# robertknight/ocrs

Hardware: AMD Instinct MI355X
Metric: pages/sec end-to-end (1024x1024) (higher is better)
Workload: dtype f32

## Files before the change

include/ocrs_amd.h:

```cpp
#ifndef OCRS_AMD_H
#define OCRS_AMD_H

#include <stddef.h>
#include <stdint.h>

#if defined(__GNUC__)
#define OCRS_API __attribute__((visibility("default")))
#else
#define OCRS_API
#endif

#ifdef __cplusplus
extern "C" {
#endif

typedef enum ocrs_status {
    OCRS_OK = 0,
    OCRS_ERR_INVALID_ARGUMENT = 1,
    OCRS_ERR_MODEL_NOT_LOADED = 2,
    OCRS_ERR_MODEL_DIMS = 3,
    OCRS_ERR_RUN_FAILED = 4,
    OCRS_ERR_WRONG_OUTPUT = 5,
    OCRS_ERR_IMAGE_SOURCE = 6,
    OCRS_ERR_DEVICE = 7,
    OCRS_ERR_IO = 8,
    OCRS_ERR_CAPACITY = 9
} ocrs_status;

OCRS_API const char* ocrs_last_error(void);

#define OCRS_ABI_VERSION 6u
OCRS_API uint32_t ocrs_abi_version(void);

OCRS_API void ocrs_buffer_free(void* p);

OCRS_API ocrs_status ocrs_device_count(int* n);
OCRS_API ocrs_status ocrs_set_device(int device);
OCRS_API ocrs_status ocrs_get_device(int* device);

OCRS_API ocrs_status ocrs_ctc_beam_search(const float* logp, int t, int c, uint32_t width, int impl, uint32_t** labels,
                                          uint32_t** positions, size_t* n);
OCRS_API ocrs_status ocrs_ctc_beam_search_scored(const float* logp, int t, int c, uint32_t width, int impl, uint32_t** labels,
                                                 uint32_t** positions, size_t* n, double* score, float** step_logp);

OCRS_API ocrs_status ocrs_gru_tile_plan(const int32_t* lengths_desc, size_t n_lines, int hidden, int32_t* n_clusters, int32_t* waves,
                                        int16_t* tiles);

OCRS_API ocrs_status ocrs_coalescer_selftest(int n_threads, int requests_per_thread, int max_active, int max_pages,
                                             long window_us, int fail_every, uint64_t out[5]);

OCRS_API ocrs_status ocrs_stream_plan_selftest(int budget, const int32_t* ops, size_t n_ops, int32_t* out);

OCRS_API ocrs_status ocrs_set_option(const char* name, long value);
OCRS_API ocrs_status ocrs_option_name(int index, const char** name);

OCRS_API ocrs_status ocrs_device_pool_stats(int device, uint64_t out[12]);
OCRS_API ocrs_status ocrs_device_pool_configure(int device, uint64_t device_cached_cap_bytes, uint64_t pinned_cached_cap_bytes);
OCRS_API ocrs_status ocrs_device_pool_trim(int device);

typedef enum { OCRS_ISOLATION_AUTO = 0, OCRS_ISOLATION_NONE = 1 } ocrs_isolation;
OCRS_API ocrs_status ocrs_device_set_isolation(int device, ocrs_isolation policy);
OCRS_API ocrs_status ocrs_device_isolation(int device, int out[3]);

typedef struct ocrs_model ocrs_model;

OCRS_API ocrs_status ocrs_model_load_file(const char* path, ocrs_model** out);
OCRS_API ocrs_status ocrs_model_load_bytes(const void* data, size_t len, ocrs_model** out);
OCRS_API ocrs_status ocrs_model_load_file_on_device(const char* path, int device, ocrs_model** out);
OCRS_API ocrs_status ocrs_model_load_bytes_on_device(const void* data, size_t len, int device, ocrs_model** out);
OCRS_API ocrs_status ocrs_model_device(const ocrs_model* m, int* device);

typedef int (*ocrs_model_run_fn)(void* user, const float* input, const int64_t in_shape[4], float** output,
                                 int64_t out_shape[4], int* out_ndim);
OCRS_API ocrs_status ocrs_model_from_callback(const int64_t input_shape[4],
                                     ocrs_model_run_fn run, void* user, ocrs_model** out);

OCRS_API ocrs_status ocrs_model_input_shape(const ocrs_model* m, int64_t dims[4], uint8_t is_fixed[4]);

typedef struct ocrs_run_options {
    int timing;
} ocrs_run_options;

OCRS_API ocrs_status ocrs_model_run(const ocrs_model* m, const float* input, const int64_t in_shape[4],
                           const ocrs_run_options* opts, float** output, int64_t out_shape[4], int* out_ndim);

OCRS_API ocrs_status ocrs_model_flops(const ocrs_model* m, const int64_t in_shape[4], double* flops);

OCRS_API void ocrs_model_free(ocrs_model* m);

typedef struct ocrs_engine ocrs_engine;
typedef struct ocrs_page ocrs_page;

typedef enum ocrs_numerics { OCRS_NUMERICS_EXACT = 0, OCRS_NUMERICS_RELAXED = 1, OCRS_NUMERICS_REDUCED = 2 } ocrs_numerics;

typedef enum ocrs_decode_method {
    OCRS_DECODE_GREEDY = 0,
    OCRS_DECODE_BEAM_SEARCH = 1
} ocrs_decode_method;

typedef struct ocrs_engine_params {
    const ocrs_model* detection_model;
    const ocrs_model* recognition_model;
    int debug;
    ocrs_decode_method decode_method;
    uint32_t beam_width;
    const char* alphabet;
    const char* allowed_chars;
    ocrs_numerics numerics;
    int coalesce;
    int coalesce_pages;
    int coalesce_window_us;
    int layout_threads;
    int64_t rec_max_pixels;
} ocrs_engine_params;

OCRS_API ocrs_status ocrs_engine_new(const ocrs_engine_params* params, ocrs_engine** out);
OCRS_API void ocrs_engine_free(ocrs_engine* e);
OCRS_API ocrs_status ocrs_engine_device(const ocrs_engine* e, int* device);
OCRS_API ocrs_status ocrs_engine_set_option(ocrs_engine* e, const char* name, long value);
OCRS_API ocrs_status ocrs_engine_get_option(const ocrs_engine* e, const char* name, long* value);

typedef enum ocrs_dim_order { OCRS_HWC = 0, OCRS_CHW = 1 } ocrs_dim_order;
typedef enum ocrs_pixel_type { OCRS_U8 = 0, OCRS_F32 = 1 } ocrs_pixel_type;

OCRS_API ocrs_status ocrs_image_source_check_bytes(size_t len, uint32_t width, uint32_t height, uint32_t* channels);

OCRS_API ocrs_status ocrs_engine_prepare_input(const ocrs_engine* e, const void* pixels, ocrs_pixel_type type,
                                      ocrs_dim_order order, int height, int width, int channels,
                                      ocrs_page** out);
OCRS_API ocrs_status ocrs_engine_prepare_input_batch(const ocrs_engine* e, const void* const* pixels, size_t n,
                                                     ocrs_pixel_type type, ocrs_dim_order order, int height, int width,
                                                     int channels, ocrs_page** out);
OCRS_API ocrs_status ocrs_engine_prepare_input_device(const ocrs_engine* e, const void* d_pixels, ocrs_pixel_type type,
                                             ocrs_dim_order order, int height, int width, int channels,
                                             ocrs_page** out);
OCRS_API void ocrs_page_free(ocrs_page* p);
OCRS_API ocrs_status ocrs_page_dims(const ocrs_page* p, int* height, int* width);
OCRS_API ocrs_status ocrs_page_image(const ocrs_page* p, float* out_hw);
OCRS_API ocrs_status ocrs_engine_page_from_grey(const ocrs_engine* e, const float* grey_hw, int height, int width, ocrs_page** out);

OCRS_API ocrs_status ocrs_engine_detect_words(const ocrs_engine* e, const ocrs_page* page, float** rects, size_t* n);
OCRS_API ocrs_status ocrs_engine_detect_words_batch(const ocrs_engine* e, const ocrs_page* const* pages, size_t n_pages,
                                           float** rects, size_t* offsets);

OCRS_API ocrs_status ocrs_engine_detect_words_scored(const ocrs_engine* e, const ocrs_page* page, float** rects, size_t* n,
                                                     float** score, uint32_t** pixels);
OCRS_API ocrs_status ocrs_engine_detect_words_batch_scored(const ocrs_engine* e, const ocrs_page* const* pages, size_t n_pages,
                                                           float** rects, size_t* offsets, float** score, uint32_t** pixels);

OCRS_API ocrs_status ocrs_engine_detect_text_pixels(const ocrs_engine* e, const ocrs_page* page, float* out_hw);

#define OCRS_TILE_OVERLAP_DEFAULT 100
OCRS_API ocrs_status ocrs_detection_tile_plan(int page_h, int page_w, int model_h, int model_w, int overlap, size_t* ny, size_t* nx,
                                              int32_t** origin_y, int32_t** bound_y, int32_t** origin_x, int32_t** bound_x);
OCRS_API ocrs_status ocrs_engine_detect_words_tiled(const ocrs_engine* e, const ocrs_page* page, int overlap, float** rects, size_t* n,
                                                    float** score, uint32_t** pixels);
OCRS_API ocrs_status ocrs_engine_detect_words_batch_tiled(const ocrs_engine* e, const ocrs_page* const* pages, size_t n_pages, int overlap,
                                                          float** rects, size_t* offsets, float** score, uint32_t** pixels);
OCRS_API ocrs_status ocrs_engine_detect_text_pixels_tiled(const ocrs_engine* e, const ocrs_page* page, int overlap, float* out_hw);

typedef enum ocrs_resample_filter { OCRS_RESAMPLE_AUTO = 0, OCRS_RESAMPLE_BILINEAR = 1, OCRS_RESAMPLE_AREA = 2 } ocrs_resample_filter;
OCRS_API ocrs_status ocrs_engine_resize_page(const ocrs_engine* e, const ocrs_page* page, int out_h, int out_w, int filter, ocrs_page** out);
OCRS_API ocrs_status ocrs_engine_resize_pages(const ocrs_engine* e, const ocrs_page* const* pages, size_t n, const int* out_hw,
                                              const int* filters, ocrs_page** out);
OCRS_API ocrs_status ocrs_work_size(int page_h, int page_w, double scale, int* h, int* w);
OCRS_API ocrs_status ocrs_rescale_rects(float* rects6, size_t n, int from_h, int from_w, int to_h, int to_w);
OCRS_API ocrs_status ocrs_engine_detect_words_at(const ocrs_engine* e, const ocrs_page* page, int work_h, int work_w, int filter, int tiled,
                                                 int overlap, float** rects, size_t* n, float** score, uint32_t** pixels);
OCRS_API ocrs_status ocrs_engine_detect_words_batch_at(const ocrs_engine* e, const ocrs_page* const* pages, size_t n_pages,
                                                       const int* work_hw, int filter, int tiled, int overlap, float** rects,
                                                       size_t* offsets, float** score, uint32_t** pixels);

typedef enum ocrs_polarity { OCRS_POLARITY_AUTO = 0, OCRS_POLARITY_KEEP = 1, OCRS_POLARITY_INVERT = 2 } ocrs_polarity;
typedef struct ocrs_normalize_params {
    int32_t tile;
    int32_t polarity;
    int32_t flatten;
    int32_t levels;
} ocrs_normalize_params;
typedef struct ocrs_normalize_info {
    int32_t dark;
    int32_t white;
    int32_t lo, hi;
    int64_t vote;
    uint64_t counted;
} ocrs_normalize_info;
OCRS_API ocrs_status ocrs_normalize_params_default(ocrs_normalize_params* out);
OCRS_API ocrs_status ocrs_normalize_params_check(const ocrs_normalize_params* params);
OCRS_API ocrs_status ocrs_engine_normalize_page(const ocrs_engine* e, const ocrs_page* page, const ocrs_normalize_params* params,
                                                ocrs_page** out_page, ocrs_normalize_info* out_info);
OCRS_API ocrs_status ocrs_engine_normalize_pages(const ocrs_engine* e, const ocrs_page* const* pages, size_t n,
                                                 const ocrs_normalize_params* params, ocrs_page** out_pages, ocrs_normalize_info* out_info);

typedef struct ocrs_skew_params {
    double max_deg;
    double coarse_step_deg;
    double fine_step_deg;
    int32_t work_max_side;
    int32_t reserved;
} ocrs_skew_params;
typedef struct ocrs_skew_info {
    double angle_deg;
    uint64_t best_score;
    uint64_t second_score;
// ... 235 lines not shown
```

ocrs_amd/_lib.py:

```python
import ctypes as C
import os

_HERE = os.path.dirname(os.path.abspath(__file__))
LIB_PATH = os.environ.get("OCRS_AMD_LIB") or os.path.join(_HERE, "libocrs_amd.so")

OCRS_OK = 0
STATUS_NAMES = {
    0: "OK", 1: "INVALID_ARGUMENT", 2: "MODEL_NOT_LOADED", 3: "MODEL_DIMS", 4: "RUN_FAILED", 5: "WRONG_OUTPUT",
    6: "IMAGE_SOURCE", 7: "DEVICE", 8: "IO", 9: "CAPACITY",
}

RUN_FN = C.CFUNCTYPE(C.c_int, C.c_void_p, C.POINTER(C.c_float), C.POINTER(C.c_int64), C.POINTER(C.POINTER(C.c_float)),
                     C.POINTER(C.c_int64), C.POINTER(C.c_int))


class EngineParams(C.Structure):
    _fields_ = [("detection_model", C.c_void_p), ("recognition_model", C.c_void_p), ("debug", C.c_int),
                ("decode_method", C.c_int), ("beam_width", C.c_uint32), ("alphabet", C.c_char_p),
                ("allowed_chars", C.c_char_p), ("numerics", C.c_int), ("coalesce", C.c_int), ("coalesce_pages", C.c_int),
                ("coalesce_window_us", C.c_int), ("layout_threads", C.c_int), ("rec_max_pixels", C.c_int64)]


class GroupParams(C.Structure):
    _fields_ = [("detection_model", C.c_void_p), ("detection_model_len", C.c_size_t), ("recognition_model", C.c_void_p),
                ("recognition_model_len", C.c_size_t), ("devices", C.POINTER(C.c_int)), ("n_devices", C.c_size_t),
                ("debug", C.c_int), ("decode_method", C.c_int), ("beam_width", C.c_uint32), ("alphabet", C.c_char_p),
                ("allowed_chars", C.c_char_p), ("gather", C.c_int), ("numerics", C.c_int), ("coalesce", C.c_int),
                ("coalesce_pages", C.c_int), ("coalesce_window_us", C.c_int), ("layout_threads", C.c_int), ("rec_max_pixels", C.c_int64),
                ("min_block", C.c_int), ("shared_block", C.c_int)]


class RunOptions(C.Structure):
    _fields_ = [("timing", C.c_int)]


class TextCharC(C.Structure):
    _fields_ = [("ch", C.c_uint32), ("top", C.c_int32), ("left", C.c_int32), ("bottom", C.c_int32),
                ("right", C.c_int32)]


class OcrsError(RuntimeError):
    def __init__(self, status, message):
        super().__init__(message)
        self.status = status
        self.status_name = STATUS_NAMES.get(status, str(status))


DECLARED_SYMBOLS = [
    "ocrs_last_error", "ocrs_buffer_free", "ocrs_device_count", "ocrs_set_device", "ocrs_set_option", "ocrs_ctc_beam_search", "ocrs_model_load_file",
    "ocrs_model_load_bytes", "ocrs_model_from_callback", "ocrs_model_input_shape", "ocrs_model_run",
    "ocrs_model_flops", "ocrs_model_free", "ocrs_engine_new", "ocrs_engine_free", "ocrs_image_source_check_bytes",
    "ocrs_engine_prepare_input", "ocrs_engine_prepare_input_device", "ocrs_page_free", "ocrs_page_dims",
    "ocrs_page_image", "ocrs_engine_detect_words", "ocrs_engine_detect_words_batch",
    "ocrs_engine_detect_text_pixels", "ocrs_engine_detection_threshold", "ocrs_engine_find_text_lines",
    "ocrs_engine_find_text_lines_batch",
    "ocrs_engine_recognize_text", "ocrs_engine_recognize_text_batch", "ocrs_engine_recognize_tokens",
    "ocrs_engine_prepare_recognition_input", "ocrs_text_item_rotated_rect", "ocrs_rotated_rect_corners", "ocrs_engine_get_text", "ocrs_device_malloc", "ocrs_device_free",
    "ocrs_device_upload", "ocrs_device_synchronize", "ocrs_device_measure_peaks", "ocrs_engine_enable_timing", "ocrs_stage_count",
    "ocrs_stage_name", "ocrs_engine_stage_times", "ocrs_kernel_class_count", "ocrs_kernel_class_name",
    "ocrs_engine_kernel_stats", "ocrs_engine_set_kernel_timing_mask", "ocrs_gru_tile_plan", "ocrs_host_malloc", "ocrs_host_free", "ocrs_engine_prepare_input_batch",
    "ocrs_get_device", "ocrs_model_load_file_on_device", "ocrs_model_load_bytes_on_device", "ocrs_model_device", "ocrs_engine_device",
    "ocrs_engine_group_new", "ocrs_engine_group_free", "ocrs_engine_group_size", "ocrs_engine_group_member", "ocrs_group_deal",
    "ocrs_group_prepare_input_batch", "ocrs_group_prepare_input_device_batch", "ocrs_group_detect_words_batch",
    "ocrs_group_recognize_text_batch", "ocrs_group_gather", "ocrs_group_final_gather", "ocrs_group_worker_threads", "ocrs_group_last_gather", "ocrs_device_malloc_on", "ocrs_engine_coalesce_stats", "ocrs_coalescer_selftest", "ocrs_stream_plan_selftest", "ocrs_engine_kernel_mfma_flops", "ocrs_engine_prepare_input_jpeg", "ocrs_jpeg_decode_rgb", "ocrs_jpeg_info", "ocrs_jpeg_coefficients",
    "ocrs_group_member_stats", "ocrs_numa_parse_cpulist", "ocrs_numa_bind_selftest", "ocrs_engine_recognize_logits", "ocrs_engine_set_option", "ocrs_engine_get_option", "ocrs_option_name", "ocrs_device_pool_stats", "ocrs_device_pool_configure", "ocrs_device_pool_trim",
    "ocrs_device_set_isolation", "ocrs_device_isolation", "ocrs_group_set_replay", "ocrs_abi_version",
    "ocrs_engine_recognize_text_scored", "ocrs_engine_recognize_text_batch_scored", "ocrs_ctc_beam_search_scored",
    "ocrs_engine_run_recognition_ops",
    "ocrs_engine_detect_words_scored", "ocrs_engine_detect_words_batch_scored", "ocrs_group_detect_words_batch_scored",
    "ocrs_engine_find_text_lines_indexed", "ocrs_engine_find_text_lines_batch_indexed",
    "ocrs_detection_tile_plan", "ocrs_engine_detect_words_tiled", "ocrs_engine_detect_words_batch_tiled",
    "ocrs_engine_detect_text_pixels_tiled", "ocrs_group_detect_words_batch_tiled",
    "ocrs_line_frame", "ocrs_line_char_boxes", "ocrs_engine_prepare_recognition_input_rectified",
    "ocrs_engine_recognize_text_rectified", "ocrs_engine_recognize_text_batch_rectified",
    "ocrs_group_recognize_text_batch_rectified", "ocrs_engine_recognize_tokens_rectified",
    "ocrs_engine_rotate_page", "ocrs_engine_rotate_pages", "ocrs_unrotate_rects", "ocrs_unrotate_chars",
    "ocrs_orientation_vote", "ocrs_engine_detect_orientation", "ocrs_engine_page_from_grey",
    "ocrs_engine_resize_page", "ocrs_engine_resize_pages", "ocrs_work_size", "ocrs_rescale_rects",
    "ocrs_engine_detect_words_at", "ocrs_engine_detect_words_batch_at",
    "ocrs_normalize_params_default", "ocrs_normalize_params_check", "ocrs_engine_normalize_page", "ocrs_engine_normalize_pages",
    "ocrs_skew_params_default", "ocrs_skew_params_check", "ocrs_skew_table", "ocrs_engine_skew_scores", "ocrs_engine_estimate_skew",
    "ocrs_engine_warp_page", "ocrs_engine_warp_pages", "ocrs_deskew_map", "ocrs_unwarp_rects", "ocrs_unwarp_chars",
    "ocrs_outline_params_default", "ocrs_outline_params_check", "ocrs_engine_edge_peaks", "ocrs_outline_choose", "ocrs_engine_find_outline",
    "ocrs_quad_map", "ocrs_engine_project_page", "ocrs_engine_project_pages", "ocrs_unproject_rects", "ocrs_unproject_chars",
]

ABI_VERSION = 6
TILE_OVERLAP_DEFAULT = 100
RESAMPLE_FILTERS = {"auto": 0, "bilinear": 1, "area": 2}
POLARITIES = {"auto": 0, "keep": 1, "invert": 2}


class NormalizeParams(C.Structure):
    _fields_ = [("tile", C.c_int32), ("polarity", C.c_int32), ("flatten", C.c_int32), ("levels", C.c_int32)]


class NormalizeInfo(C.Structure):
    _fields_ = [("dark", C.c_int32), ("white", C.c_int32), ("lo", C.c_int32), ("hi", C.c_int32), ("vote", C.c_int64),
                ("counted", C.c_uint64)]

    def as_dict(self):
        return {"dark": int(self.dark), "vote": int(self.vote), "white": int(self.white), "lo": int(self.lo), "hi": int(self.hi),
                "counted": int(self.counted)}


class SkewParams(C.Structure):
    _fields_ = [("max_deg", C.c_double), ("coarse_step_deg", C.c_double), ("fine_step_deg", C.c_double), ("work_max_side", C.c_int32),
                ("reserved", C.c_int32)]


class SkewInfo(C.Structure):
    _fields_ = [("angle_deg", C.c_double), ("best_score", C.c_uint64), ("second_score", C.c_uint64), ("fine_score", C.c_uint64),
                ("work_h", C.c_int32), ("work_w", C.c_int32), ("coarse_index", C.c_int32), ("fine_index", C.c_int32)]


class OutlineParams(C.Structure):
    _fields_ = [("max_deg", C.c_double), ("step_deg", C.c_double), ("min_cover", C.c_double), ("min_span", C.c_double), ("min_area", C.c_double),
                ("work_max_side", C.c_int32), ("min_step", C.c_int32)]


class OutlineInfo(C.Structure):
    _fields_ = [("found", C.c_int32), ("polarity", C.c_int32), ("corners", C.c_float * 8), ("counts", C.c_uint32 * 4), ("angles", C.c_int32 * 4),
                ("work_h", C.c_int32), ("work_w", C.c_int32)]


_lib = None


def lib():
    global _lib
    if _lib is None:
        if not os.path.exists(LIB_PATH):
            raise OcrsError(7, "libocrs_amd.so is not built: run `python -m ocrs_amd.build` "
                               "(there is no CPU fallback for the HIP engine)")
        L = C.CDLL(LIB_PATH)
        L.ocrs_abi_version.restype = C.c_uint32
        if L.ocrs_abi_version() != ABI_VERSION:
            raise OcrsError(7, "libocrs_amd.so has ABI version %d, this binding was written for %d: rebuild (python -m ocrs_amd.build)"
                            % (L.ocrs_abi_version(), ABI_VERSION))
        L.ocrs_last_error.restype = C.c_char_p
        L.ocrs_engine_detection_threshold.restype = C.c_float
        L.ocrs_engine_detection_threshold.argtypes = [C.c_void_p]
        L.ocrs_stage_name.restype = C.c_char_p
        L.ocrs_kernel_class_name.restype = C.c_char_p
        L.ocrs_buffer_free.argtypes = [C.c_void_p]
        for name in ("ocrs_model_free", "ocrs_engine_free", "ocrs_page_free", "ocrs_engine_group_free"):
            getattr(L, name).argtypes = [C.c_void_p]
            getattr(L, name).restype = None
        _lib = L
    return _lib


def check(status):
    if status != OCRS_OK:
        msg = lib().ocrs_last_error()
        raise OcrsError(status, msg.decode("utf-8", "replace") if msg else STATUS_NAMES.get(status, "error"))


def device_count():
    n = C.c_int(0)
    check(lib().ocrs_device_count(C.byref(n)))
    return n.value


def measure_peaks():
    a, b = C.c_double(0), C.c_double(0)
    check(lib().ocrs_device_measure_peaks(C.byref(a), C.byref(b)))
    return a.value, b.value


def set_option(name, value):
    check(lib().ocrs_set_option(name.encode(), C.c_long(int(value))))


def option_names():
    out, i = [], 0
    while True:
        n = C.c_char_p()
        check(lib().ocrs_option_name(i, C.byref(n)))
        if not n.value:
            return out
        out.append(n.value.decode())
        i += 1


POOL_FIELDS = ("device_live", "device_cached", "device_cap", "device_peak_live", "device_driver_allocs", "device_driver_frees",
               "pinned_live", "pinned_cached", "pinned_cap", "pinned_peak_live", "pinned_driver_allocs", "pinned_driver_frees")


def pool_stats(device=-1):
    v = (C.c_uint64 * 12)()
    check(lib().ocrs_device_pool_stats(int(device), v))
    return dict(zip(POOL_FIELDS, (int(x) for x in v)))


def pool_trim(device=-1):
    check(lib().ocrs_device_pool_trim(int(device)))


def pool_configure(device=-1, device_cached_cap=0, pinned_cached_cap=0):
    check(lib().ocrs_device_pool_configure(int(device), C.c_uint64(int(device_cached_cap)), C.c_uint64(int(pinned_cached_cap))))


ISOLATION = {"auto": 0, "none": 1}


def set_isolation(policy="auto", device=-1):
    check(lib().ocrs_device_set_isolation(int(device), int(ISOLATION[policy])))


def isolation(device=-1):
    v = (C.c_int * 3)()
    check(lib().ocrs_device_isolation(int(device), v))
    return {"mode": ("free", "serial")[v[0]], "relaxed_engines": int(v[1]), "cus": int(v[2])}


def ctc_beam_search(logp, width, impl=0):
# ... 64 lines not shown
```

ocrs_amd/csrc/abi.cpp:

```cpp
#include <cstdio>
#include <fstream>
#include <thread>

#include <atomic>
#include "abi_util.hpp"
#include "coalesce_selftest.hpp"
#include "engine.hpp"
#include "host_pool.hpp"
#include "jpeg.hpp"
#include "kernels.hpp"
#include "page_ops.hpp"

using namespace ocrs;
using namespace ocrs::geom;

using namespace ocrs::abi;

extern "C" {

const char* ocrs_last_error(void) { return last_error().c_str(); }

void ocrs_buffer_free(void* p) { free(p); }

ocrs_status ocrs_device_count(int* n) {
    return guarded([&] {
        int c = 0;
        hipError_t e = hipGetDeviceCount(&c);
        if (e != hipSuccess) c = 0;
        *n = c;
    });
}

ocrs_status ocrs_set_device(int device) {
    return guarded([&] { select_device(device); });
}

ocrs_status ocrs_get_device(int* device) {
    return guarded([&] {
        if (!device) fail(OCRS_ERR_INVALID_ARGUMENT, "null argument");
        *device = default_device();
    });
}

ocrs_status ocrs_gru_tile_plan(const int32_t* lengths_desc, size_t n_lines, int hidden, int32_t* n_clusters, int32_t* waves,
                               int16_t* tiles) {
    return guarded([&] {
        if (!lengths_desc || !n_clusters || !waves || !tiles || n_lines == 0 || n_lines > (size_t)1 << 20)
            fail(OCRS_ERR_INVALID_ARGUMENT, "bad argument");
        for (size_t i = 0; i < n_lines; i++)
            if (lengths_desc[i] < 1 || (i > 0 && lengths_desc[i] > lengths_desc[i - 1]))
                fail(OCRS_ERR_INVALID_ARGUMENT, "lengths must be positive and descending");
        int ncl = 0;
        if (!k::gru_tile_plan(lengths_desc, (int)n_lines, hidden, &ncl, waves, tiles))
            fail(OCRS_ERR_CAPACITY, "no persistent-kernel plan for this shape (the engine then runs the recurrence as one fused launch per time step)");
        *n_clusters = ncl;
    });
}

ocrs_status ocrs_coalescer_selftest(int n_threads, int requests_per_thread, int max_active, int max_pages, long window_us,
                                    int fail_every, uint64_t out[5]) {
    return guarded([&] {
        if (!out || n_threads < 1 || requests_per_thread < 1 || max_pages < 1) fail(OCRS_ERR_INVALID_ARGUMENT, "bad argument");
        coalescer_selftest(n_threads, requests_per_thread, max_active, max_pages, window_us, fail_every, out);
    });
}

ocrs_status ocrs_stream_plan_selftest(int budget, const int32_t* ops, size_t n_ops, int32_t* out) {
    return guarded([&] {
        if (!out || (n_ops > 0 && !ops) || !LanePlan::valid_budget(budget)) fail(OCRS_ERR_INVALID_ARGUMENT, "bad argument");
        LanePlan plan(budget);
        for (size_t i = 0; i < n_ops; i++) {
            const int32_t op = ops[2 * i], arg = ops[2 * i + 1];
            switch (op) {
                case 0: out[i] = plan.acquire(arg); break;
                case 1: plan.release(arg); out[i] = plan.outstanding(); break;
                case 2: out[i] = plan.set_budget(arg) ? 1 : 0; break;
                case 3: out[i] = plan.load(arg); break;
                case 4: out[i] = plan.budget(); break;
                case 5: out[i] = plan.light_lanes(); break;
                default: fail(OCRS_ERR_INVALID_ARGUMENT, "unknown op %d", (int)op);
            }
        }
    });
}

namespace {

void beam_search_hook(const float* logp, int t, int c, uint32_t width, int impl, std::vector<uint32_t>* l,
                      std::vector<uint32_t>* p, double* score, std::vector<float>* step_logp) {
    if (impl == 2 && t > 0) {
        DeviceScope bind(-1);
        if (!k::ctc_beam_supported(c, (int)width)) fail(OCRS_ERR_CAPACITY, "beam search on the GPU supports up to 128 classes and width 128");
        Workspace ws;
        std::vector<int32_t> meta(1 + t + 1);
        meta[0] = t;
        for (int i = 0; i <= t; i++) meta[1 + i] = i;
        int32_t* d_meta = ws.alloc_n<int32_t>(meta.size());
        float* d_logp = ws.alloc_n<float>((size_t)t * c);
        ws.upload(d_meta, meta.data(), meta.size() * sizeof(int32_t));
        ws.upload(d_logp, logp, (size_t)t * c * sizeof(float));
        const size_t arena = k::ctc_beam_arena_entries(t, (int)width);
        int2* d_nodes = ws.alloc_n<int2>(arena);
        int2* d_posn = ws.alloc_n<int2>(arena);
        uint32_t* d_ol = ws.alloc_n<uint32_t>(t);
        uint32_t* d_op = ws.alloc_n<uint32_t>(t);
        int32_t* d_cnt = ws.alloc_n<int32_t>(1);
        double* d_score = score ? ws.alloc_n<double>(1) : nullptr;
        float* d_slp = score ? ws.alloc_n<float>(t) : nullptr;
        k::ctc_beam_packed(d_logp, d_meta, d_meta + 1, 1, t, c, (int)width, nullptr, d_nodes, d_posn, d_ol, d_op, d_cnt, ws.s(),
                           d_score, d_slp);
        std::vector<uint32_t> hl(t), hp(t);
        std::vector<float> hs(score ? t : 0);
        int32_t cnt = 0;
        ws.download(hl.data(), d_ol, (size_t)t * 4);
        ws.download(hp.data(), d_op, (size_t)t * 4);
        ws.download(&cnt, d_cnt, 4);
        if (score) {
            ws.download(score, d_score, sizeof(double));
            ws.download(hs.data(), d_slp, (size_t)t * sizeof(float));
        }
        ws.sync();
        OCRS_HIP(hipGetLastError());
        l->assign(hl.begin(), hl.begin() + cnt);
        p->assign(hp.begin(), hp.begin() + cnt);
        if (score) step_logp->assign(hs.begin(), hs.begin() + cnt);
    } else {
        double bs = 0.0;
        const std::vector<CtcStep> st = t == 0 ? std::vector<CtcStep>()
                                              : (impl == 1 ? ctc_beam_search_reference(logp, t, c, c, width, &bs)
                                                           : ctc_beam_search(logp, t, c, c, width, &bs));
        l->resize(st.size()); p->resize(st.size());
        for (size_t i = 0; i < st.size(); i++) { (*l)[i] = st[i].label; (*p)[i] = st[i].pos; }
        if (score) score_line(logp, t, c, c, nullptr, st, &bs, step_logp, score);
    }
}

}

ocrs_status ocrs_ctc_beam_search(const float* logp, int t, int c, uint32_t width, int impl, uint32_t** labels,
                                 uint32_t** positions, size_t* n) {
    return guarded([&] {
        if (!logp || !labels || !positions || !n || t < 0 || c < 1) fail(OCRS_ERR_INVALID_ARGUMENT, "bad argument");
        std::vector<uint32_t> l, p;
        beam_search_hook(logp, t, c, width, impl, &l, &p, nullptr, nullptr);
        *labels = dup_buffer(l);
        *positions = dup_buffer(p);
        *n = l.size();
    });
}

ocrs_status ocrs_ctc_beam_search_scored(const float* logp, int t, int c, uint32_t width, int impl, uint32_t** labels,
                                        uint32_t** positions, size_t* n, double* score, float** step_logp) {
    return guarded([&] {
        if (!logp || !labels || !positions || !n || !score || !step_logp || t < 0 || c < 1)
            fail(OCRS_ERR_INVALID_ARGUMENT, "bad argument");
        std::vector<uint32_t> l, p;
        std::vector<float> s;
        double sc = 0.0;
        beam_search_hook(logp, t, c, width, impl, &l, &p, &sc, &s);
        *labels = dup_buffer(l);
        *positions = dup_buffer(p);
        *step_logp = dup_buffer(s);
        *n = l.size();
        *score = sc;
    });
}

uint32_t ocrs_abi_version(void) { return OCRS_ABI_VERSION; }

static void check_option_set(int r, const char* name, long value) {
    if (r == 1) fail(OCRS_ERR_INVALID_ARGUMENT, "unknown option '%s'", name ? name : "(null)");
    if (r == 2) fail(OCRS_ERR_INVALID_ARGUMENT, "option '%s': value %ld is out of range", name, value);
    if (r == 3) fail(OCRS_ERR_INVALID_ARGUMENT, "option '%s' cannot change while a request is in flight on a device", name);
    if (r == 4) fail(OCRS_ERR_INVALID_ARGUMENT, "option '%s' belongs to the devices, not to an engine: set it with ocrs_set_option", name);
}

ocrs_status ocrs_set_option(const char* name, long value) {
    return guarded([&] { check_option_set(set_option(name, value), name, value); });
}

ocrs_status ocrs_engine_set_option(ocrs_engine* e, const char* name, long value) {
    return guarded([&] {
        if (!e) fail(OCRS_ERR_INVALID_ARGUMENT, "null argument");
        check_option_set(set_option(e->tuning, name, value), name, value);
    });
}

ocrs_status ocrs_engine_get_option(const ocrs_engine* e, const char* name, long* value) {
    return guarded([&] {
        if (!e || !value) fail(OCRS_ERR_INVALID_ARGUMENT, "null argument");
        if (!get_option(e->tuning, name, value)) fail(OCRS_ERR_INVALID_ARGUMENT, "unknown option '%s'", name ? name : "(null)");
    });
}

ocrs_status ocrs_option_name(int index, const char** name) {
    return guarded([&] {
        if (!name) fail(OCRS_ERR_INVALID_ARGUMENT, "null argument");
        *name = option_name(index);
    });
}

ocrs_status ocrs_device_pool_stats(int device, uint64_t out[12]) {
    return guarded([&] {
        if (!out) fail(OCRS_ERR_INVALID_ARGUMENT, "null argument");
        DeviceContext& c = device_context(device < 0 ? default_device() : device);
        const PoolStats d = c.pool.stats(), h = c.host_pool.stats();
        const uint64_t v[12] = {d.live, d.cached, d.cap, d.peak_live, d.driver_allocs, d.driver_frees,
                                h.live, h.cached, h.cap, h.peak_live, h.driver_allocs, h.driver_frees};
        for (int i = 0; i < 12; i++) out[i] = v[i];
    });
}

ocrs_status ocrs_device_pool_trim(int device) {
    return guarded([&] {
        DeviceContext& c = device_context(device < 0 ? default_device() : device);
        DeviceScope bind(c.device);
        {
            std::lock_guard<std::mutex> heavy(c.heavy_phase);
            OCRS_HIP(hipStreamSynchronize(c.heavy_stream()));
            c.heavy_arena.clear();
        }
        c.pool.trim();
    });
}

ocrs_status ocrs_device_set_isolation(int device, ocrs_isolation policy) {
    return guarded([&] {
        if (policy != OCRS_ISOLATION_AUTO && policy != OCRS_ISOLATION_NONE) fail(OCRS_ERR_INVALID_ARGUMENT, "unknown isolation policy %d", (int)policy);
        DeviceContext& c = device_context(device < 0 ? default_device() : device);
        DeviceScope bind(c.device);
        c.set_isolation(policy == OCRS_ISOLATION_NONE ? DeviceContext::ISO_NONE : DeviceContext::ISO_AUTO);
    });
}

// ... 878 lines not shown
```

ocrs_amd/csrc/common.cpp:

```cpp
#include "common.hpp"

#include <chrono>
#include <climits>
#include <cstdint>
#include <cstdlib>
#include <cstring>

#include <algorithm>
#include <atomic>
#include <condition_variable>
#include <deque>
#include <system_error>

namespace ocrs {

static thread_local std::string g_last_error;

void set_last_error(const std::string& msg) { g_last_error = msg; }
const std::string& last_error() { return g_last_error; }

namespace {
std::atomic<int> g_default_device{0};
thread_local DeviceContext* t_ctx = nullptr;
constexpr int kMaxDevices = 64;
// ... 323 lines not shown
hipStream_t DeviceContext::recurrent_stream(int mode) {
    if (mode == MODE_SERIAL) return heavy_stream();
    std::lock_guard<std::mutex> g(lazy_mu_);
    create_lanes_locked(planned_light_lanes());
    return recurrent_;
}

hipStream_t DeviceContext::light_lane(int lane) {
    std::lock_guard<std::mutex> g(lazy_mu_);
    create_lanes_locked(std::max(lane + 1, plan.light_lanes()));
    return light_[lane];
}

bool DeviceContext::calls_in_flight() {
    std::lock_guard<std::mutex> lk(iso_mu_);
    return leases_ > 0;
}

static thread_local int t_lease_depth[kMaxDevices] = {0};

template <class F> void DeviceContext::switch_isolation(F&& change) {
    if (t_lease_depth[device] > 0) fail(OCRS_ERR_INVALID_ARGUMENT, "the isolation regime of device %d cannot change from inside one of its requests", device);
    std::unique_lock<std::mutex> lk(iso_mu_);
    iso_cv_.wait(lk, [&] { return !switching_; });
    const Mode before = mode_locked();
    switching_ = true;
    struct Done { DeviceContext* c; ~Done() { c->switching_ = false; c->iso_cv_.notify_all(); } } done{this};
    const Isolation p0 = policy_;
    const int r0 = relaxed_;
    change();
    if (mode_locked() == before) return;
    const Isolation p1 = policy_;
    const int r1 = relaxed_;
    policy_ = p0; relaxed_ = r0;
    iso_cv_.wait(lk, [&] { return leases_ == 0; });
    {
        DeviceScope bind(device);
        if (hipDeviceSynchronize() != hipSuccess) (void)hipGetLastError();
    }
    policy_ = p1; relaxed_ = r1;
}

DeviceContext::Mode DeviceContext::lease_begin() {
    std::unique_lock<std::mutex> lk(iso_mu_);
    if (t_lease_depth[device] == 0) iso_cv_.wait(lk, [&] { return !switching_; });
    t_lease_depth[device]++;
    leases_++;
    return mode_locked();
}

void DeviceContext::lease_end() {
    std::lock_guard<std::mutex> lk(iso_mu_);
    t_lease_depth[device]--;
    if (--leases_ == 0) iso_cv_.notify_all();
}

void DeviceContext::add_relaxed_engine(int delta) {
    switch_isolation([&] { relaxed_ += delta; });
}

void DeviceContext::set_isolation(Isolation policy) {
    switch_isolation([&] { policy_ = policy; });
}

DeviceContext::Mode DeviceContext::current_mode() {
    std::lock_guard<std::mutex> lk(iso_mu_);
    return mode_locked();
}

int DeviceContext::relaxed_engine_count() {
    std::lock_guard<std::mutex> lk(iso_mu_);
    return relaxed_;
}

int DeviceContext::cu_count() {
    std::lock_guard<std::mutex> g(lazy_mu_);
    if (!cus_) {
        hipDeviceProp_t prop;
        OCRS_HIP(hipGetDeviceProperties(&prop, device));
        cus_ = prop.multiProcessorCount;
    }
    return cus_;
}

namespace {
struct OptDef { const char* name; const char* env; long def; };
const OptDef kOptDefs[OPT_COUNT] = {
    {"gru_mode", "OCRS_GRU_MODE", GRU_PERSISTENT},
    {"gru_gates", "OCRS_GRU_GATES", 1},
    {"gru_local", "OCRS_GRU_LOCAL", 1},
    {"det_fuse", "OCRS_DET_FUSE", 1},
    {"det_stream", "OCRS_DET_STREAM", 1},
    {"det_rows", "OCRS_DET_ROWS", 1},
    {"ccl_quad", "OCRS_CCL_QUAD", 1},
    {"conv12_fuse", "OCRS_CONV12_FUSE", 1},
    {"conv_flat", "OCRS_CONV_FLAT", 1},
    {"beam_gpu", "OCRS_BEAM_GPU", 1},
    {"det_tile_batch", "OCRS_DET_TILE_BATCH", 16},
    {"stream_budget", "OCRS_STREAM_BUDGET", LanePlan::kDefaultBudget},
    {"numerics", nullptr, 0},
    {"coalesce", nullptr, 2},
    {"coalesce_pages", nullptr, 16},
    {"coalesce_window_us", nullptr, 300},
    {"layout_threads", nullptr, 0},
    {"rec_max_pixels", nullptr, 0},
};
struct OptRange { long lo, hi; long also[4]; };
const OptRange kOptRanges[OPT_COUNT] = {
    {0, 1, {}}, {0, 1, {}}, {0, 1, {}}, {0, 2, {}}, {0, 1, {8, 14, 32}}, {0, 1, {8, 14, 20, 32}}, {0, 1, {}}, {0, 1, {}}, {0, 1, {}}, {0, 1, {}},
    {1, 1024, {}}, {LanePlan::kMinBudget, LanePlan::kMaxBudget, {}},
    {0, 2, {}}, {0, 64, {}}, {1, 4096, {}}, {0, 10000000, {}}, {0, 4096, {}}, {0, INT64_MAX, {}},
};
bool in_range(int i, long v) {
    const OptRange& r = kOptRanges[i];
    if (i == OPT_STREAM_BUDGET) return LanePlan::valid_budget(v);
    if (v >= r.lo && v <= r.hi) return true;
    for (long a : r.also) if (a && v == a) return true;
    return false;
}
const char* const kRetired[] = {"det_heavy", "det_tail", "gru_waves", "gru_background", "gru_scatter", "gru_gates_pack", "conv_occupancy",
                                "gx_heavy", "gemm_nfast", "conv_a_lds", "gru_heavy", "heavy_priority", "det_mfma"};
std::atomic<long> g_opts[OPT_COUNT];
std::once_flag g_opts_once;
void init_options() {
    for (int i = 0; i < OPT_COUNT; i++) {
        const char* e = kOptDefs[i].env ? getenv(kOptDefs[i].env) : nullptr;
        const long v = e && *e ? strtol(e, nullptr, 10) : kOptDefs[i].def;
        g_opts[i].store(in_range(i, v) ? v : kOptDefs[i].def);
    }
}
int find_option(const char* name, int count = OPT_PUBLIC_COUNT) {
    for (int i = 0; i < count; i++)
        if (name && i != OPT_NUMERICS && strcmp(name, kOptDefs[i].name) == 0) return i;
    return -1;
}
thread_local const Tuning* t_tuning = nullptr;
}

TuningScope::TuningScope(const Tuning* t) : prev_(t_tuning) { t_tuning = t; }
TuningScope::~TuningScope() { t_tuning = prev_; }
const Tuning* current_tuning() { return t_tuning; }

long process_option(Option o) {
    std::call_once(g_opts_once, init_options);
    return g_opts[o].load(std::memory_order_relaxed);
}

long option_long(Option o) {
    if (t_tuning) return __atomic_load_n(&t_tuning->v[o], __ATOMIC_RELAXED);
    std::call_once(g_opts_once, init_options);
    return g_opts[o].load(std::memory_order_relaxed);
}
int option(Option o) { return (int)option_long(o); }

Tuning default_tuning() {
    std::call_once(g_opts_once, init_options);
    Tuning t;
    for (int i = 0; i < OPT_COUNT; i++) t.v[i] = g_opts[i].load(std::memory_order_relaxed);
    return t;
}

const char* option_name(int i) { return i >= 0 && i < OPT_PUBLIC_COUNT ? kOptDefs[i].name : nullptr; }

int set_option(const char* name, long value) {
    std::call_once(g_opts_once, init_options);
    const int i = find_option(name);
    if (i < 0) {
        for (const char* r : kRetired) if (name && strcmp(name, r) == 0) return 0;
        return 1;
    }
    if (!in_range(i, value)) return 2;
    if (i == OPT_STREAM_BUDGET && value != g_opts[i].load() && any_device_has_calls_in_flight()) return 3;
    g_opts[i].store(value);
    return 0;
}

int set_option(Tuning& t, const char* name, long value) {
    const int i = find_option(name, OPT_COUNT);
    if (i < 0) return 1;
    if (i == OPT_STREAM_BUDGET) return 4;
    if (!in_range(i, value)) return 2;
    __atomic_store_n(&t.v[i], value, __ATOMIC_RELAXED);
    return 0;
}

bool get_option(const Tuning& t, const char* name, long* value) {
    const int i = name && strcmp(name, "numerics") == 0 ? (int)OPT_NUMERICS : find_option(name, OPT_COUNT);
    if (i < 0) return false;
    *value = __atomic_load_n(&t.v[i], __ATOMIC_RELAXED);
    return true;
}

static hipEvent_t take_lease_event(DeviceContext* c) {
    {
        std::lock_guard<std::mutex> g(c->stream_mu);
        if (!c->lease_events.empty()) {
            hipEvent_t e = c->lease_events.back();
            c->lease_events.pop_back();
            return e;
        }
    }
    hipEvent_t e = nullptr;
    OCRS_HIP(hipEventCreateWithFlags(&e, hipEventBlockingSync | hipEventDisableTiming));
    return e;
}

StreamLease::StreamLease(bool high_priority, int avoid_lane) : ctx_(&ctx()), high_(high_priority) {
    high_ = true;
    mode_ = ctx_->lease_begin();
    try {
        done_ = take_lease_event(ctx_);
        if (mode_ == DeviceContext::MODE_SERIAL) {
            s_ = ctx_->heavy_stream();
            shared_ = true;
            return;
        }
        (void)ctx_->planned_light_lanes();
        lane_ = ctx_->plan.acquire(avoid_lane);
        counted_ = true;
        if (lane_ >= 0) {
            s_ = ctx_->light_lane(lane_);
            return;
        }
        {
            std::lock_guard<std::mutex> g(ctx_->stream_mu);
            auto& v = ctx_->streams;
            if (!v.empty()) {
                s_ = v.back();
                v.pop_back();
                return;
            }
        }
        int least = 0, greatest = 0;
        OCRS_HIP(hipDeviceGetStreamPriorityRange(&least, &greatest));
        OCRS_HIP(hipStreamCreateWithPriority(&s_, hipStreamNonBlocking, greatest));
    } catch (...) {
        if (counted_) ctx_->plan.release(lane_);
        if (done_) {
            std::lock_guard<std::mutex> g(ctx_->stream_mu);
            ctx_->lease_events.push_back(done_);
        }
        ctx_->lease_end();
        throw;
    }
}

StreamLease::~StreamLease() {
    {
        std::lock_guard<std::mutex> g(ctx_->stream_mu);
        ctx_->lease_events.push_back(done_);
        if (!shared_ && lane_ < 0) ctx_->streams.push_back(s_);
    }
    if (counted_) ctx_->plan.release(lane_);
    ctx_->lease_end();
}

std::vector<StageTimers::Pending>& StageTimers::pending() {
    static thread_local std::vector<Pending> p;
    return p;
}
std::map<int, std::vector<hipEvent_t>>& StageTimers::thread_events() {
    static thread_local std::map<int, std::vector<hipEvent_t>> f;
    return f;
}
std::vector<hipEvent_t>& StageTimers::free_events() { return thread_events()[ctx().device]; }

hipEvent_t StageTimers::get_event() {
    auto& fe = free_events();
    if (!fe.empty()) {
        hipEvent_t e = fe.back();
        fe.pop_back();
        return e;
    }
    hipEvent_t e;
    OCRS_HIP(hipEventCreate(&e));
    return e;
}

int StageTimers::begin(int stage, hipStream_t s, uint64_t n_launches) {
    if (!enabled) return -1;
    Pending p{stage, get_event(), get_event(), n_launches, false, 0.0, 0.0, 0.0};
    OCRS_HIP(hipEventRecord(p.a, s));
    pending().push_back(p);
    return (int)pending().size() - 1;
}

int StageTimers::kbegin(int cls, hipStream_t s, double flops, double bytes, double mfma_flops) {
    if (!enabled || !kernels_enabled || !((kernel_mask >> cls) & 1u)) return -1;
    if (mfma_flops < 0.0) mfma_flops = cls <= KC_GEMM_LINEAR ? flops : 0.0;
    Pending p{cls, get_event(), get_event(), 1, true, flops, bytes, mfma_flops};
    OCRS_HIP(hipEventRecord(p.a, s));
    pending().push_back(p);
    return (int)pending().size() - 1;
}

void StageTimers::end(int token, hipStream_t s) {
    if (token < 0) return;
    auto& pd = pending();
    if ((size_t)token < pd.size()) (void)hipEventRecord(pd[token].b, s);
}

void StageTimers::collect() {
    auto& pd = pending();
    if (pd.empty()) return;
    double lms[ST_COUNT] = {0}, lkms[KC_COUNT] = {0}, lkf[KC_COUNT] = {0}, lkb[KC_COUNT] = {0}, lkm[KC_COUNT] = {0};
    uint64_t ln[ST_COUNT] = {0}, lkn[KC_COUNT] = {0};
    for (auto& p : pd) {
        float t = 0.f;
        if (hipEventSynchronize(p.b) == hipSuccess && hipEventElapsedTime(&t, p.a, p.b) == hipSuccess) {
            if (p.kernel) { lkms[p.stage] += t; lkn[p.stage] += 1; lkf[p.stage] += p.flops; lkb[p.stage] += p.bytes; lkm[p.stage] += p.mfma; }
            else { lms[p.stage] += t; ln[p.stage] += p.n; }
        }
        free_events().push_back(p.a);
        free_events().push_back(p.b);
    }
    pd.clear();
    std::lock_guard<std::mutex> g(mu);
    for (int i = 0; i < ST_COUNT; i++) { ms[i] += lms[i]; launches[i] += ln[i]; }
    for (int i = 0; i < KC_COUNT; i++) { kms[i] += lkms[i]; klaunches[i] += lkn[i]; kflops[i] += lkf[i]; kbytes[i] += lkb[i]; kmfma[i] += lkm[i]; }
}

void StageTimers::release_thread_events() {
    for (auto& p : pending()) { (void)hipEventDestroy(p.a); (void)hipEventDestroy(p.b); }
    pending().clear();
    for (auto& kv : thread_events()) {
        for (hipEvent_t e : kv.second) (void)hipEventDestroy(e);
        kv.second.clear();
    }
}

void StageTimers::reset() {
    std::lock_guard<std::mutex> g(mu);
    for (int i = 0; i < ST_COUNT; i++) { ms[i] = 0; launches[i] = 0; }
    for (int i = 0; i < KC_COUNT; i++) { kms[i] = 0; klaunches[i] = 0; kflops[i] = 0; kbytes[i] = 0; kmfma[i] = 0; }
}

}
```

ocrs_amd/csrc/common.hpp:

```cpp
#pragma once
#include <atomic>
#include <hip/hip_runtime.h>

#include <cstdarg>
#include <cstdint>
#include <cstdio>
#include <cstdlib>
#include <chrono>
#include <condition_variable>
#include <cstring>
#include <map>
#include <mutex>
#include <stdexcept>
#include <string>
#include <thread>
#include <vector>

#include "../../include/ocrs_amd.h"
#include "stream_plan.hpp"

namespace ocrs {

struct Error : std::runtime_error {
    ocrs_status status;
    Error(ocrs_status s, const std::string& msg) : std::runtime_error(msg), status(s) {}
};

[[noreturn]] inline void fail(ocrs_status s, const char* fmt, ...) {
    char buf[512];
    va_list ap;
    va_start(ap, fmt);
    vsnprintf(buf, sizeof buf, fmt, ap);
    va_end(ap);
    throw Error(s, buf);
}

#define OCRS_HIP(expr)                                                                              \
    do {                                                                                            \
        hipError_t _e = (expr);                                                                     \
        if (_e != hipSuccess)                                                                       \
            ::ocrs::fail(OCRS_ERR_DEVICE, "HIP error %s at %s:%d (%s)", hipGetErrorString(_e), __FILE__, \
                         __LINE__, #expr);                                                          \
    } while (0)

void set_last_error(const std::string& msg);


struct PoolStats { uint64_t live = 0, cached = 0, cap = 0, peak_live = 0, driver_allocs = 0, driver_frees = 0; };
class DevicePool {
  public:
    explicit DevicePool(int device) : device_(device) {}
    ~DevicePool();
    void* alloc(size_t bytes);
    void release(void* p);
    void trim();
    void set_cap(uint64_t bytes);
    PoolStats stats();
    int device() const { return device_; }

  private:
    uint64_t cap_locked();
    const int device_;
    std::mutex mu_;
    std::multimap<size_t, void*> free_;
    std::map<void*, size_t> live_;
    uint64_t cached_ = 0, live_bytes_ = 0, peak_live_ = 0, cap_ = 0, allocs_ = 0;
    std::atomic<uint64_t> frees_{0};
};

class HostPool {
  public:
    void* alloc(size_t bytes);
    void release(void* p);
    void set_cap(uint64_t bytes);
    PoolStats stats();

  private:
    std::mutex mu_;
    std::multimap<size_t, void*> free_;
    std::map<void*, size_t> live_;
    uint64_t cached_ = 0, live_bytes_ = 0, peak_live_ = 0, cap_ = uint64_t(1) << 30, allocs_ = 0;
    std::atomic<uint64_t> frees_{0};
};

struct DeviceContext {
    const int device;
    DevicePool pool;
    HostPool host_pool;
    std::mutex heavy_phase, rec_phase;
    hipStream_t heavy_stream();
    hipStream_t recurrent_stream(int mode = 0);
    enum Isolation { ISO_AUTO = 0, ISO_NONE = 1 };
    enum Mode { MODE_FREE = 0, MODE_SERIAL = 1 };
    Mode lease_begin();
    void lease_end();
    void add_relaxed_engine(int delta);
    void set_isolation(Isolation policy);
    Mode current_mode();
    int relaxed_engine_count();
    int cu_count();
    std::vector<struct DevBuf> heavy_arena;
    std::mutex stream_mu;
    LanePlan plan;
    std::vector<hipStream_t> streams;
    std::vector<hipEvent_t> lease_events;
    hipStream_t light_lane(int lane);
    int planned_light_lanes();
    bool calls_in_flight();

    explicit DeviceContext(int d) : device(d), pool(d) {}

  private:
    Mode mode_locked() const { return policy_ == ISO_NONE || relaxed_ <= 0 ? MODE_FREE : MODE_SERIAL; }
    template <class F> void switch_isolation(F&& change);
    std::mutex lazy_mu_;
    hipStream_t heavy_ = nullptr, recurrent_ = nullptr;
    std::vector<hipStream_t> light_;
    void create_lanes_locked(int n_light);
    int cus_ = 0;
    std::mutex iso_mu_;
    std::condition_variable iso_cv_;
    int leases_ = 0, relaxed_ = 0;
    bool switching_ = false;
    Isolation policy_ = ISO_AUTO;
    friend class StreamLease;
};

DeviceContext& device_context(int device);
int default_device();
void select_device(int device);
DeviceContext& ctx();

class DeviceScope {
  public:
    explicit DeviceScope(int device);
    ~DeviceScope();
    DeviceScope(const DeviceScope&) = delete;
    DeviceScope& operator=(const DeviceScope&) = delete;

  private:
    DeviceContext* prev_;
    int restore_ = -1;
};

inline DevicePool& pool() { return ctx().pool; }
inline HostPool& host_pool() { return ctx().host_pool; }
inline hipStream_t heavy_stream() { return ctx().heavy_stream(); }

enum Option { OPT_GRU_MODE = 0, OPT_GRU_GATES, OPT_GRU_LOCAL, OPT_DET_FUSE, OPT_DET_STREAM, OPT_DET_ROWS, OPT_CCL_QUAD,
              OPT_CONV12_FUSE, OPT_CONV_FLAT, OPT_BEAM_GPU, OPT_DET_TILE_BATCH, OPT_STREAM_BUDGET, OPT_PUBLIC_COUNT,
              OPT_NUMERICS = OPT_PUBLIC_COUNT,
              OPT_COALESCE, OPT_COALESCE_PAGES, OPT_COALESCE_WINDOW_US,
              OPT_LAYOUT_THREADS, OPT_REC_MAX_PIXELS,
              OPT_COUNT };
struct Tuning { long v[OPT_COUNT]; };
Tuning default_tuning();
int set_option(const char* name, long value);
int set_option(Tuning& t, const char* name, long value);
bool get_option(const Tuning& t, const char* name, long* value);
const char* option_name(int i);
class TuningScope {
  public:
    explicit TuningScope(const Tuning* t);
    ~TuningScope();
    TuningScope(const TuningScope&) = delete;
    TuningScope& operator=(const TuningScope&) = delete;
  private:
    const Tuning* prev_;
};
const Tuning* current_tuning();
enum { GRU_PERSISTENT = 0, GRU_STEP = 1 };
int option(Option o);
long process_option(Option o);

inline void allow_dynamic_lds(const void* kernel, std::atomic<uint64_t>& done) {
    int dev = 0;
    (void)hipGetDevice(&dev);
    const uint64_t bit = 1ull << (dev & 63);
    if (done.load(std::memory_order_relaxed) & bit) return;
    (void)hipFuncSetAttribute(kernel, hipFuncAttributeMaxDynamicSharedMemorySize, 160 * 1024);
    done.fetch_or(bit, std::memory_order_relaxed);
}
long option_long(Option o);
inline int gru_mode() { return option(OPT_GRU_MODE); }

struct DevBuf {
    void* p = nullptr;
    size_t bytes = 0;
    DevicePool* owner = nullptr;
    DevBuf() = default;
    explicit DevBuf(size_t n) : bytes(n), owner(n ? &pool() : nullptr) { p = n ? owner->alloc(n) : nullptr; }
    DevBuf(const DevBuf&) = delete;
    DevBuf& operator=(const DevBuf&) = delete;
    DevBuf(DevBuf&& o) noexcept : p(o.p), bytes(o.bytes), owner(o.owner) { o.p = nullptr; o.bytes = 0; o.owner = nullptr; }
    DevBuf& operator=(DevBuf&& o) noexcept {
        if (this != &o) { reset(); p = o.p; bytes = o.bytes; owner = o.owner; o.p = nullptr; o.bytes = 0; o.owner = nullptr; }
        return *this;
    }
    ~DevBuf() { reset(); }
    void reset() { if (p && owner) owner->release(p); p = nullptr; bytes = 0; owner = nullptr; }
    int device() const { return owner ? owner->device() : -1; }
    template <class T> T* as() const { return static_cast<T*>(p); }
};

struct PinnedBuf {
    void* p = nullptr;
    size_t bytes = 0;
    PinnedBuf() = default;
    explicit PinnedBuf(size_t n) : bytes(n) { if (n) OCRS_HIP(hipHostMalloc(&p, n, hipHostMallocPortable)); }
    PinnedBuf(const PinnedBuf&) = delete;
    PinnedBuf& operator=(const PinnedBuf&) = delete;
    ~PinnedBuf() { if (p) (void)hipHostFree(p); }
    template <class T> T* as() const { return static_cast<T*>(p); }
};

inline hipError_t wait_event(hipEvent_t ev) noexcept {
    for (int i = 0;; i++) {
        const hipError_t e = hipEventQuery(ev);
        if (e != hipErrorNotReady) return e;
        if (i < 64) std::this_thread::yield();
        else std::this_thread::sleep_for(std::chrono::microseconds(i < 256 ? 20 : 100));
    }
}

class StreamLease {
  public:
    explicit StreamLease(bool high_priority = false, int avoid_lane = LanePlan::kPrivate);
    ~StreamLease();
    hipStream_t get() const { return s_; }
    int lane() const { return lane_; }
    bool may_park_waits() const { return lane_ < 0 || ctx_->plan.outstanding() <= 1; }
    hipError_t wait_done() const noexcept {
        const hipError_t e = hipEventRecord(done_, s_);
        return e != hipSuccess ? e : wait_event(done_);
    }
    void sync() const { OCRS_HIP(wait_done()); }
    hipError_t sync_noexcept() const noexcept { return wait_done(); }
    DeviceContext::Mode mode() const { return mode_; }
    bool serial() const { return mode_ == DeviceContext::MODE_SERIAL; }
    hipStream_t conv_stream() const { return ctx_->heavy_stream(); }
    hipStream_t recurrent_stream() const { return ctx_->recurrent_stream((int)mode_); }

  private:
    DeviceContext* ctx_;
    DeviceContext::Mode mode_ = DeviceContext::MODE_FREE;
    bool shared_ = false;
    bool counted_ = false;
    int lane_ = LanePlan::kPrivate;
    hipStream_t s_ = nullptr;
    hipEvent_t done_ = nullptr;
    bool high_;
};

enum Stage {
    ST_PREPARE = 0,
    ST_RESIZE_IN,
    ST_DET_CNN,
    ST_RESIZE_THRESH,
    ST_CCL,
    ST_CONTOUR_RECTS,
    ST_LINE_CROP,
    ST_REC_CONV,
    ST_REC_GRU,
    ST_REC_HEAD,
    ST_CTC,
    ST_COUNT
};
extern const char* const kStageNames[ST_COUNT];

enum KernelClass {
    KC_GEMM_CONV3X3 = 0, KC_GEMM_POINTWISE, KC_GEMM_CONVT, KC_GEMM_GRU_INPUT, KC_GEMM_GRU_HIDDEN, KC_GEMM_LINEAR,
    KC_DWCONV3X3, KC_CONV_DIRECT, KC_POOL, KC_PADCAT, KC_CONV1X1_SIGMOID, KC_GRU_GATES, KC_LOGSOFTMAX_ARGMAX,
    KC_OTHER, KC_DET_BLOCK, KC_DET_STREAM_WAVE, KC_DET_STREAM_ROWS, KC_COUNT
};
extern const char* const kKernelClassNames[KC_COUNT];

struct StageTimers {
    bool enabled = false;
    bool kernels_enabled = false;
    uint32_t kernel_mask = 0xffffffffu;
    std::mutex mu;
    double ms[ST_COUNT] = {0};
    uint64_t launches[ST_COUNT] = {0};
    double kms[KC_COUNT] = {0};
    uint64_t klaunches[KC_COUNT] = {0};
    double kflops[KC_COUNT] = {0};
    double kbytes[KC_COUNT] = {0};
    double kmfma[KC_COUNT] = {0};
    struct Pending { int stage; hipEvent_t a, b; uint64_t n; bool kernel; double flops, bytes, mfma; };
    static std::vector<Pending>& pending();
    int begin(int stage, hipStream_t s, uint64_t n_launches);
    int kbegin(int cls, hipStream_t s, double flops, double bytes, double mfma_flops = -1.0);
    void end(int token, hipStream_t s);
    void collect();
    void reset();
    static void release_thread_events();
  private:
    static std::vector<hipEvent_t>& free_events();
    static std::map<int, std::vector<hipEvent_t>>& thread_events();
    hipEvent_t get_event();
};

inline int ceil_div(int64_t a, int64_t b) { return (int)((a + b - 1) / b); }

struct StageScope {
    StageTimers* t; int token; hipStream_t s;
    StageScope(StageTimers* timers, int stage, hipStream_t stream, uint64_t n_launches = 1)
        : t(timers), token(timers ? timers->begin(stage, stream, n_launches) : -1), s(stream) {}
// ... 66 lines not shown
```

ocrs_amd/csrc/kernels.hpp:

```cpp
#pragma once
#include <vector>
#include <hip/hip_runtime.h>

#include <cstdint>

namespace ocrs {
namespace jpeg { struct Coefficients; }
namespace k {

void prepare_image(const void* d_pixels, bool is_u8, bool chans_last, int h, int w, int chans, float* d_out,
                   hipStream_t s);
struct PrepareTable {
    enum { kPages = 32 };
    const void* src[kPages];
    float* dst[kPages];
};
void prepare_image_batch(const void* const* d_pixels, float* const* d_out, int n, bool is_u8, bool chans_last, int h, int w,
                         int chans, hipStream_t s);
void resize_pages_to_model(const float* const* d_src_ptrs, int n, int sh, int sw, int vh, int vw, float* d_dst,
                           int dh, int dw, hipStream_t s);
bool resize_threshold(const float* d_prob, int n, int mh, int mw, int sh, int sw, float thr, uint8_t* d_mask,
                      float* d_map, int h, int w, hipStream_t s, int32_t* d_labels = nullptr, int32_t* d_zero_a = nullptr,
                      int32_t* d_zero_b = nullptr);
void threshold_only(const float* d_prob, float thr, uint8_t* d_mask, int64_t count, hipStream_t s);

struct CclBuffers {
    int32_t* labels;
    int32_t* row_counts;
    int32_t* row_offsets;
    int32_t* n_roots;
    int32_t* roots;
    int32_t* lengths;
    int32_t* offsets;
    int32_t* overflow;
    uint32_t* pts;
    uint32_t* tmp;
    uint8_t* keep;
    float* rects;
    uint8_t* valid;
    uint32_t* score_pixels;
    unsigned long long* score_sums;
};
void ccl_label(const uint8_t* d_mask, int n, int h, int w, const CclBuffers& b, int max_comp, hipStream_t s, bool prepared = false);
void contour_rects(const uint8_t* d_mask, int n, int h, int w, const CclBuffers& b, int max_comp, int64_t arena,
                   float expand, float min_area, float eps, hipStream_t s, bool prepared = false);

void component_scores(const uint8_t* d_mask, const float* d_map, int n, int h, int w, const CclBuffers& b, int max_comp,
                      hipStream_t s);

struct TileDesc {
    const float* page;
    uint8_t* mask;
    float* map;
    int32_t h, w;
    int32_t oy, ox;
    int32_t y0, y1, x0, x1;
};
void gather_tiles(const TileDesc* d_tiles, int n_tiles, float* d_dst, int mh, int mw, hipStream_t s);
void stitch_threshold(const TileDesc* d_tiles, int n_tiles, const float* d_prob, int mh, int mw, float thr, hipStream_t s);

struct GemmDesc {
    const float* A; int lda;
    const float* B; int ldb;
    const float* bias;
    float* C; int ldc;
    int M, N, K;
    int relu;
    int im2col; int H, W, Cin;
    int convt; int Cout;
    int batch; int64_t strideA, strideB, strideBias, strideC;
    int nfast = 0, nx = 0, ny = 0;
    const uint16_t* Bsplit = nullptr; int64_t strideBsplit = 0;
};
void gemm(const GemmDesc& d, hipStream_t s);
void conv_direct(const float* x, int n, int h, int w, int cin, const float* wt, const float* bias, int kh, int kw,
                 int cout, int relu, float* y, hipStream_t s);
void dwconv3x3(const float* x, int n, int h, int w, int c, const float* wt, const float* bias, int relu, float* y,
               hipStream_t s);
bool dwpw_fused_supported(int cin, int cout);
void dwpw_fused(const float* x, int n, int h, int w, int cin, const float* wdw, const float* bdw, int relu_dw, int cout,
                const float* wpw, const float* bpw, int relu_pw, float* y, hipStream_t s);
bool dwconv3x3_cat(const float* skip, int n, int h, int w, int cs, const float* up, int uh, int uw, int cu, const float* wt,
                   const float* bias, int relu, float* y, hipStream_t s);
struct DoubleConvArgs {
    const float* skip;
    const float* x1;
    const float *wt, *bt;
    const float *wd1, *bd1;
    const float *wp1, *bp1;
    const float *wd2, *bd2;
    const float *wp2, *bp2;
    const float *wf, *bf;
    float* y;
    float* ypool;
    int n, h, w, h1, w1;
    int relu_d1, relu_p1, relu_d2, relu_p2, sigmoid;
    int tiles_x, tiles_y;
    const float* tape = nullptr;
    int tape_len = 0;
    const float* rtape = nullptr;
    int rtape_len = 0;
};
struct StreamWeights {
    const float *wt, *bt, *wd1, *bd1, *wp1, *bp1, *wd2, *bd2, *wp2, *bp2, *wf, *bf;
};
bool double_conv_fused(const DoubleConvArgs& a, int cs, int cx, int cmid, int cout, bool pool, bool final_conv,
                       bool launch, hipStream_t s, bool* on_mfma = nullptr, int* path = nullptr);
bool double_conv_stream(const DoubleConvArgs& a, int cs, int cx, int cmid, int cout, bool pool, bool final_conv, bool launch, hipStream_t s,
                        const StreamWeights* hw = nullptr, std::vector<float>* tape_out = nullptr, int* tape_len = nullptr);
bool double_conv_rows(const DoubleConvArgs& a, int cs, int cx, int cmid, int cout, bool pool, bool final_conv, bool launch, hipStream_t s,
                      const StreamWeights* hw = nullptr, std::vector<float>* tape_out = nullptr, int* tape_len = nullptr);
bool double_conv_rows_takes(const DoubleConvArgs& a, int cx);
void maxpool(const float* x, int n, int h, int w, int c, int kh, int kw, float* y, hipStream_t s);
void avgpool(const float* x, int n, int h, int w, int c, int kh, int kw, float* y, hipStream_t s);
void padcat(const float* skip, int n, int sh, int sw, int cs, const float* x, int h, int w, int cx, float* y,
            hipStream_t s);
void sigmoid(const float* x, float* y, int64_t count, hipStream_t s);
void conv1x1_cout1(const float* x, int64_t pixels, int cin, const float* wt, const float* bias, int relu, int do_sigmoid,
                   float* y, hipStream_t s);
void to_seq(const float* x, int n, int w, int c, float* y, hipStream_t s);
void gru_gates(const float* gx, const float* gh, float* h, float* y, int T, int N, int H, int step, hipStream_t s);
bool log_softmax_argmax(const float* logits, int64_t rows, int c, const uint8_t* d_excluded ,
                        float* logp, int32_t* labels, hipStream_t s, float* maxlp = nullptr);
void to_seq_packed(const float* x, int n, int T, int c, const int32_t* d_pos, const int32_t* d_off, float* y,
                   hipStream_t s);
void gru_gates_packed(const float* gx, const float* gh, float* h, float* y, const int32_t* d_Tm, const int32_t* d_off,
                      int64_t R, int Mcap, int active, int H, int step, hipStream_t s);
bool gru_step_fused(const float* gx, const float* wh, const float* bh, const float* hT_in, float* hT_out, float* y,
                    const int32_t* d_Tm, const int32_t* d_off, int64_t R, int Mcap, int active, int H, int step,
                    hipStream_t s);
size_t gru_persistent_sync_words(int M);
size_t gru_persistent_exchange_bytes(const int32_t* h_Tm, int M, int H);
bool gru_persistent_supported(const int32_t* h_Tm, int M, int Tmax, int64_t R, int H);
bool gru_tile_plan(const int32_t* h_Tm, int M, int H, int* ncl, int* waves, int16_t* tiles );
hipError_t gru_persistent_prepare(float* hx, const int32_t* h_Tm, int M, int H, hipStream_t s);
bool gru_persistent(const float* gx, const float* wh, const float* bh, float* y, float* hx, const int32_t* d_Tm, const int32_t* d_off,
                    const int32_t* h_Tm, int64_t R, int M, int Tmax, int H, uint32_t* d_sync, hipStream_t s);
bool gru_general_tile_plan(const int32_t* h_Tm, int M, int Tmax, int H, int cap, int* ncl, int16_t* tiles , int kernel );
size_t gru_split_exchange_bytes(const int32_t* h_Tm, int M, int H, int np);
bool gru_split_supported(const int32_t* h_Tm, int M, int Tmax, int64_t R, int H, int np);
hipError_t gru_split_prepare(uint16_t* hx, const int32_t* h_Tm, int M, int H, int np, hipStream_t s);
bool gru_persistent_split(const float* gx, const float* wh, const float* bh, float* y, uint16_t* hx, const int32_t* d_Tm, const int32_t* d_off,
                          const int32_t* h_Tm, int64_t R, int M, int Tmax, int H, int np, uint32_t* d_sync, hipStream_t s);
void ctc_collapse_packed(const int32_t* labels, const int32_t* d_Tm, const int32_t* d_off, int M, int Tmax,
                         uint32_t* out_labels, uint32_t* out_pos, int32_t* out_count, hipStream_t s);
void ctc_collapse_scored_packed(const int32_t* labels, const float* maxlp, const int32_t* d_Tm, const int32_t* d_off, int M,
                                int Tmax, uint32_t* out_labels, uint32_t* out_pos, float* out_logp, int32_t* out_count,
                                double* out_score, hipStream_t s);
void argmax_rows(const float* x, int64_t rows, int c, const uint8_t* d_excluded, int32_t* labels, hipStream_t s);
bool ctc_beam_supported(int C, int width);
size_t ctc_beam_arena_entries(int Tmax, int width);
bool ctc_beam_packed(const float* logp, const int32_t* d_Tm, const int32_t* d_off, int M, int Tmax, int C, int width,
                     const uint8_t* d_excluded, int2* d_nodes, int2* d_posn, uint32_t* out_labels, uint32_t* out_pos,
                     int32_t* out_count, hipStream_t s, double* out_score = nullptr, float* out_logp = nullptr);
void ctc_collapse(const int32_t* labels, int T, int N, uint32_t* out_labels, uint32_t* out_pos, int32_t* out_count,
                  hipStream_t s);

struct RaggedView {
    int G;
    int H;
    const int32_t* W;
    const int32_t* n;
    const int64_t* poff;
    const int32_t* toff256;
    const int32_t* loff;
    int ntiles256;
    const int32_t* toff2d;
    int ntiles2d, tw;
    const int32_t* toff2d_flat;
    const int32_t* toff2d_flat2;
    int ntiles2d_flat, ntiles2d_flat2;
    const int32_t* toff2d_gap;
    int ntiles2d_gap;
    int64_t max_tile_px_;
    int min_w;
    int64_t pixels;
    int max_w;
};
void conv1_relu_pool_ragged(const float* x, const RaggedView& in, const float* wt, const float* bias, int cout,
                            float* y, const RaggedView& out, hipStream_t s);
void pool_ragged(const float* x, const RaggedView& in, int c, int kh, int kw, bool avg, float* y, const RaggedView& out,
                 hipStream_t s);
void to_seq_packed_ragged(const float* x, const RaggedView& in, int c, const int32_t* d_pos, const int32_t* d_off,
                          float* y, hipStream_t s);
void avgpool_to_seq_ragged(const float* x, const RaggedView& in, const RaggedView& seq, int c, const int32_t* d_pos,
                           const int32_t* d_off, float* y, hipStream_t s);
bool conv12_fused_ragged(const float* x, const RaggedView& in0, const RaggedView& mid, const float* w1, const float* b1,
                         int c1, const float* w2, const float* b2, int c2, float* y, const RaggedView& out, hipStream_t s,
                         const uint16_t* w2split = nullptr);
void conv12_split_weights(const float* w2_host , std::vector<uint16_t>* out);
bool conv3x3_ragged(const float* x, const RaggedView& rv, int cin, const float* wt, const float* bias, int cout, int relu,
                    int ph, int pw, float* y, const RaggedView& out, hipStream_t s, const uint16_t* wsplit = nullptr);
void split_weights(const float* w_host, int K, int N, int ldw, std::vector<uint16_t>* out);

struct LineDesc {
    int32_t page;
    int32_t poly_off;
    int32_t poly_n;
    int32_t top, left, bh, bw;
    int32_t resized_w;
    int32_t out_w;
    int64_t out_off;
};
void crop_lines(const float* const* d_pages, const int32_t* d_page_hw , const LineDesc* d_lines,
                const int32_t* d_poly , int n_lines, int out_h, float* d_out, hipStream_t s);

struct RectLineDesc {
    int32_t page;
    int32_t mode;
    int32_t range_off;
    int32_t range_n;
    int32_t resized_w;
    int32_t out_w;
    int64_t out_off;
    float x0, ax, bx, y0, ay, by;
};
void rectify_lines(const float* const* d_pages, const int32_t* d_page_hw , const RectLineDesc* d_lines,
                   const int32_t* d_ranges, int n_lines, int max_out_w, int out_h, float* d_out, hipStream_t s);

struct RotateDesc {
    const uint32_t* src;
    uint32_t* dst;
    int32_t h, w;
    int32_t k;
    int32_t block0;
    int32_t vec;
    int32_t pad_;
};
int64_t rotate_tiles(int h, int w);
void rotate_pages(const RotateDesc* d_descs, int n_pages, int total_tiles, hipStream_t s);

struct ResampleDesc {
    const float* src;
    float* dst;
    int32_t sh, sw, dh, dw;
    int32_t area;
    int32_t block0;
    uint32_t py, qy;
    uint32_t px, qx;
};
int64_t resample_blocks(int dh, int dw);
void resample_pages(const ResampleDesc* d_descs, int n_pages, int total_blocks, hipStream_t s);

struct NormInfo {
    int32_t dark;
    int32_t white;
    int32_t lo, hi;
    int64_t vote;
    uint64_t counted;
};
struct NormState {
    unsigned long long hist_v[256];
    unsigned long long hist_u[256];
    long long vote;
    NormInfo info;
};
struct NormDesc {
    const float* src;
    float* dst;
    NormState* state;
    uint32_t* tiles;
    uint8_t* grid;
    int32_t h, w;
    int32_t tshift;
    int32_t th, tw;
    int32_t block0;
    int32_t polarity;
    int32_t flatten, levels;
    int32_t vec;
};
void normalize_pages(const NormDesc* d_descs, int n_pages, int total_blocks, NormInfo* d_info, hipStream_t s);

struct SkewDesc {
    const float* src;
    uint32_t* prof;
    int32_t h, w;
    int32_t nb;
    int32_t block0;
};
int64_t skew_tiles(int h, int w);
void skew_scores(const SkewDesc* d_descs, int n_pages, int total_tiles, const int32_t* d_sc_table, int n_angles,
                 unsigned long long* d_scores, hipStream_t s);
struct WarpDesc {
    const float* src;
    float* dst;
    int32_t sh, sw, dh, dw;
    int32_t block0;
    int32_t vec;
    float m[6];
    float fill;
    int32_t pad_;
};
int64_t warp_blocks(int dh, int dw);
void warp_pages(const WarpDesc* d_descs, int n_pages, int total_blocks, hipStream_t s);

struct EdgeDesc {
    const float* src;
    uint32_t* prof;
    unsigned long long* peaks;
    int32_t h, w;
    int32_t nb;
    int32_t block0;
};
int64_t edge_tiles(int h, int w);
void edge_peaks(const EdgeDesc* d_descs, int n_pages, int total_tiles, const int32_t* d_sc_table, int n_angles, int min_step, hipStream_t s);
struct ProjDesc {
    const float* src;
    float* dst;
    int32_t sh, sw, dh, dw;
    int32_t block0;
    int32_t vec;
    float m[8];
    float fill;
    int32_t pad_;
};
int64_t project_blocks(int dh, int dw);
void project_pages(const ProjDesc* d_descs, int n_pages, int total_blocks, hipStream_t s);

void measure_peaks(double* mfma_tflops, double* copy_gbps);


size_t jpeg_sample_bytes(const jpeg::Coefficients& c);
void jpeg_decode(const jpeg::Coefficients& c, const uint64_t* d_mask, const uint32_t* d_offset, const int16_t* d_values,
                 const uint16_t* d_quant, uint8_t* d_samples, uint8_t* d_rgb, hipStream_t s);

}
}
```

ocrs_amd/csrc/kernels_rec.hip:

```cpp
#include <algorithm>

#include "common.hpp"
#include "kernels.hpp"
#include "split_mfma.hpp"

namespace ocrs {
namespace k {

typedef float f32x16 __attribute__((ext_vector_type(16)));
typedef unsigned u32x4 __attribute__((ext_vector_type(4)));
typedef float f32x4 __attribute__((ext_vector_type(4)));
typedef float f32x2 __attribute__((ext_vector_type(2)));
typedef unsigned u32x2 __attribute__((ext_vector_type(2)));
typedef __bf16 bf16x8 __attribute__((ext_vector_type(8)));
typedef __bf16 bf16x2 __attribute__((ext_vector_type(2)));

__device__ __forceinline__ int xcd_remap(int b, int nwg) {
    const int xcd = b & 7, q = nwg >> 3, r = nwg & 7;
    return (xcd < r ? xcd * (q + 1) : r * (q + 1) + (xcd - r) * q) + (b >> 3);
}

__device__ __forceinline__ int find_group(const int32_t* __restrict__ toff, int G, int tile) {
    int lo = 0, hi = G;
    while (hi - lo > 1) {
        int mid = (lo + hi) >> 1;
        if (toff[mid] <= tile) lo = mid; else hi = mid;
    }
    return lo;
}

__global__ void __launch_bounds__(256)
conv1_relu_pool_ragged_kernel(const float* __restrict__ x, RaggedView in, const float* __restrict__ wt,
                              const float* __restrict__ bias, int cout, float* __restrict__ y, RaggedView out) {
    __shared__ float sw[9 * 64 + 64];
    for (int i = threadIdx.x; i < 9 * cout; i += 256) sw[i] = wt[i];
    for (int i = threadIdx.x; i < cout; i += 256) sw[9 * 64 + i] = bias[i];
    __syncthreads();
    const int g = find_group(out.toff256, out.G, blockIdx.x);
    const int tile = blockIdx.x - out.toff256[g];
    const int ow = out.W[g], oh = out.H, iw = in.W[g], ih = in.H;
    const int64_t rows = (int64_t)out.n[g] * oh * ow;
    const float* __restrict__ xg = x + in.poff[g];
    float* __restrict__ yg = y + out.poff[g] * cout;
    const int cq = cout >> 2;
    const int step_px = 256 / cq;
    const int q = threadIdx.x % cq;
    int64_t r = (int64_t)tile * 256 + threadIdx.x / cq;
    int ox = (int)(r % ow);
    int64_t t0 = r / ow;
    int oy = (int)(t0 % oh);
    int64_t img = t0 / oh;
    float wq[9][4], bq[4];
#pragma unroll
    for (int t = 0; t < 9; t++)
#pragma unroll
        for (int c = 0; c < 4; c++) wq[t][c] = sw[t * cout + 4 * q + c];
#pragma unroll
    for (int c = 0; c < 4; c++) bq[c] = sw[9 * 64 + 4 * q + c];
    for (int it = 0; it < cq; it++, r += step_px) {
        if (r >= rows) break;
        if (it > 0) {
            ox += step_px;
            while (ox >= ow) { ox -= ow; if (++oy == oh) { oy = 0; img++; } }
        }
        const float* xi = xg + img * ih * iw;
        float p[4][4];
        const int iy0 = 2 * oy - 1, ix0 = 2 * ox - 1;
        if (iy0 >= 0 && iy0 + 3 < ih && ix0 >= 0 && ix0 + 3 < iw) {
            const float* pp = xi + (int64_t)iy0 * iw + ix0;
#pragma unroll
            for (int a = 0; a < 4; a++)
#pragma unroll
                for (int b = 0; b < 4; b++) p[a][b] = pp[a * iw + b];
        } else {
#pragma unroll
            for (int a = 0; a < 4; a++)
#pragma unroll
                for (int b = 0; b < 4; b++) {
                    const int iy = iy0 + a, ix = ix0 + b;
                    p[a][b] = ((unsigned)iy < (unsigned)ih && (unsigned)ix < (unsigned)iw) ? xi[(int64_t)iy * iw + ix] : 0.0f;
                }
        }
        float m[4];
#pragma unroll
        for (int py = 0; py < 2; py++)
#pragma unroll
            for (int px = 0; px < 2; px++) {
                float acc[4];
#pragma unroll
                for (int c = 0; c < 4; c++) acc[c] = bq[c];
#pragma unroll
                for (int ky = 0; ky < 3; ky++)
#pragma unroll
                    for (int kx = 0; kx < 3; kx++) {
                        const float xv = p[py + ky][px + kx];
#pragma unroll
                        for (int c = 0; c < 4; c++) acc[c] = fmaf(xv, wq[ky * 3 + kx][c], acc[c]);
                    }
#pragma unroll
                for (int c = 0; c < 4; c++) {
                    float v = acc[c] > 0.0f ? acc[c] : 0.0f;
                    if (py == 0 && px == 0) m[c] = v;
                    else m[c] = v > m[c] ? v : m[c];
                }
            }
        *reinterpret_cast<float4*>(yg + r * cout + 4 * q) = make_float4(m[0], m[1], m[2], m[3]);
    }
}

void conv1_relu_pool_ragged(const float* x, const RaggedView& in, const float* wt, const float* bias, int cout,
                            float* y, const RaggedView& out, hipStream_t s) {
    if (out.ntiles256 <= 0) return;
    hipLaunchKernelGGL(conv1_relu_pool_ragged_kernel, dim3(out.ntiles256), dim3(256), 0, s, x, in, wt, bias, cout, y, out);
}

template <bool AVG>
__global__ void __launch_bounds__(256)
pool_ragged_kernel(const float* __restrict__ x, RaggedView in, int c, int kh, int kw, float* __restrict__ y,
                   RaggedView out) {
    const int g = find_group(out.toff256, out.G, blockIdx.x);
    const int tile = blockIdx.x - out.toff256[g];
    const int ow = out.W[g], oh = out.H, iw = in.W[g], ih = in.H;
    const int64_t rows = (int64_t)out.n[g] * oh * ow;
    const float* __restrict__ xg = x + in.poff[g] * c;
    float* __restrict__ yg = y + out.poff[g] * c;
    const int cq = c >> 2;
    const float inv = 1.0f / (float)(kh * kw);
    for (int i = threadIdx.x; i < 256 * cq; i += 256) {
        const int64_t r = (int64_t)tile * 256 + i / cq;
        if (r >= rows) break;
        const int q = i % cq;
        const int ox = (int)(r % ow);
        const int oy = (int)((r / ow) % oh);
        const int64_t img = r / ((int64_t)ow * oh);
        const float* xp = xg + ((img * ih + (int64_t)oy * kh) * iw + (int64_t)ox * kw) * c + 4 * q;
        float4 acc = AVG ? make_float4(0.f, 0.f, 0.f, 0.f) : *reinterpret_cast<const float4*>(xp);
        for (int ky = 0; ky < kh; ky++)
            for (int kx = 0; kx < kw; kx++) {
                const float4 v = *reinterpret_cast<const float4*>(xp + ((int64_t)ky * iw + kx) * c);
                if (AVG) { acc.x = acc.x + v.x; acc.y = acc.y + v.y; acc.z = acc.z + v.z; acc.w = acc.w + v.w; }
                else {
                    acc.x = v.x > acc.x ? v.x : acc.x; acc.y = v.y > acc.y ? v.y : acc.y;
                    acc.z = v.z > acc.z ? v.z : acc.z; acc.w = v.w > acc.w ? v.w : acc.w;
                }
            }
        if (AVG) { acc.x = acc.x * inv; acc.y = acc.y * inv; acc.z = acc.z * inv; acc.w = acc.w * inv; }
        *reinterpret_cast<float4*>(yg + r * c + 4 * q) = acc;
    }
}

void pool_ragged(const float* x, const RaggedView& in, int c, int kh, int kw, bool avg, float* y, const RaggedView& out,
                 hipStream_t s) {
    if (out.ntiles256 <= 0) return;
    if (avg) hipLaunchKernelGGL((pool_ragged_kernel<true>), dim3(out.ntiles256), dim3(256), 0, s, x, in, c, kh, kw, y, out);
    else hipLaunchKernelGGL((pool_ragged_kernel<false>), dim3(out.ntiles256), dim3(256), 0, s, x, in, c, kh, kw, y, out);
}

__global__ void __launch_bounds__(256)
to_seq_packed_ragged_kernel(const float* __restrict__ x, RaggedView in, int c, const int32_t* __restrict__ pos,
                            const int32_t* __restrict__ off, float* __restrict__ y) {
    const int g = find_group(in.toff256, in.G, blockIdx.x);
    const int tile = blockIdx.x - in.toff256[g];
    const int T = in.W[g];
    const int64_t rows = (int64_t)in.n[g] * T;
    const float* __restrict__ xg = x + in.poff[g] * c;
    const int32_t* __restrict__ posg = pos + in.loff[g];
    const int cq = c >> 2;
    for (int i = threadIdx.x; i < 256 * cq; i += 256) {
        const int64_t r = (int64_t)tile * 256 + i / cq;
        if (r >= rows) break;
        const int q = i % cq;
        const int t = (int)(r % T);
        const int line = (int)(r / T);
        const float4 v = *reinterpret_cast<const float4*>(xg + r * c + 4 * q);
        *reinterpret_cast<float4*>(y + ((int64_t)off[t] + posg[line]) * c + 4 * q) = v;
    }
}

__global__ void __launch_bounds__(256)
avgpool_to_seq_ragged_kernel(const float* __restrict__ x, RaggedView in, RaggedView seq, int c,
                             const int32_t* __restrict__ pos, const int32_t* __restrict__ off, float* __restrict__ y) {
    const int g = find_group(seq.toff256, seq.G, blockIdx.x);
    const int tile = blockIdx.x - seq.toff256[g];
    const int T = seq.W[g], ih = in.H;
    const int64_t rows = (int64_t)seq.n[g] * T;
    const float* __restrict__ xg = x + in.poff[g] * c;
    const int32_t* __restrict__ posg = pos + seq.loff[g];
    const int cq = c >> 2;
    const float inv = 1.0f / (float)ih;
    for (int i = threadIdx.x; i < 256 * cq; i += 256) {
        const int64_t r = (int64_t)tile * 256 + i / cq;
        if (r >= rows) break;
        const int q = i % cq;
        const int t = (int)(r % T);
        const int64_t line = r / T;
        const float* xp = xg + (line * ih * T + t) * c + 4 * q;
        float4 acc = make_float4(0.f, 0.f, 0.f, 0.f);
        for (int ky = 0; ky < ih; ky++) {
            const float4 v = *reinterpret_cast<const float4*>(xp + (int64_t)ky * T * c);
            acc.x = acc.x + v.x; acc.y = acc.y + v.y; acc.z = acc.z + v.z; acc.w = acc.w + v.w;
        }
        acc.x = acc.x * inv; acc.y = acc.y * inv; acc.z = acc.z * inv; acc.w = acc.w * inv;
        *reinterpret_cast<float4*>(y + ((int64_t)off[t] + posg[line]) * c + 4 * q) = acc;
    }
}

void avgpool_to_seq_ragged(const float* x, const RaggedView& in, const RaggedView& seq, int c, const int32_t* d_pos,
                           const int32_t* d_off, float* y, hipStream_t s) {
    if (seq.ntiles256 <= 0) return;
    hipLaunchKernelGGL(avgpool_to_seq_ragged_kernel, dim3(seq.ntiles256), dim3(256), 0, s, x, in, seq, c, d_pos, d_off, y);
}

void to_seq_packed_ragged(const float* x, const RaggedView& in, int c, const int32_t* d_pos, const int32_t* d_off,
                          float* y, hipStream_t s) {
    if (in.ntiles256 <= 0) return;
    hipLaunchKernelGGL(to_seq_packed_ragged_kernel, dim3(in.ntiles256), dim3(256), 0, s, x, in, c, d_pos, d_off, y);
}

constexpr int RG_BM = 128, RG_BK = 16, RG_LDA = RG_BM + 1;
constexpr int CONV_WAVES = 4;
template <int BN, int TW, int PH, int PW, bool FLAT, int SPLIT = 0>
__global__ void __launch_bounds__(256, SPLIT == 3 ? 2 : SPLIT == 2 ? 3 : CONV_WAVES)
conv3x3_ragged_kernel(const float* __restrict__ X, RaggedView rv, int cin, const float* __restrict__ Bw,
                      const float* __restrict__ bias, int cout, int relu, float* __restrict__ Y,
                      const int64_t* __restrict__ out_poff) {
    extern __shared__ __attribute__((aligned(16))) float lds[];
    constexpr int NTW = BN / 64;
    constexpr int TH = RG_BM / TW;
    static_assert(TW == 32 || TW == 16, "patch width");
    static_assert(!SPLIT || (BN == 128 && RG_BK == 16), "split mode: 128-column blocks, 16-deep chunks");
    constexpr int NP = SPLIT ? SPLIT : 1;
    constexpr int SP_PLANE = split::PLANE;
    float* As = lds;
    float* Bs = lds + (SPLIT ? 2 * NP * SP_PLANE : 2 * RG_BK * RG_LDA);
    const int tid = threadIdx.x, lane = tid & 63, wave = tid >> 6;
    const int half = lane >> 5, l31 = lane & 31;
    const int wm = wave >> 1, wn = wave & 1;
    const int gtile = xcd_remap(blockIdx.x, gridDim.x);
    const int32_t* __restrict__ toff = FLAT ? (PW == 2 ? rv.toff2d_flat2 : rv.toff2d_flat) : rv.toff2d;
    const int g = find_group(toff, rv.G, gtile);
    const int tile = gtile - toff[g];
    const int H = rv.H, W = rv.W[g];
    const int tiles_h = H / TH;
    const int Wp = FLAT ? (PW == 2 ? (W + 1) & ~1 : W) : W;
    const int nimg = FLAT ? rv.n[g] : 1;
    int rb, img, x0, span = 1;
    if (FLAT) {
        rb = tile % tiles_h;
        const int c0 = (tile / tiles_h) * TW;
        img = c0 / Wp;
        x0 = c0 - img * Wp;
        span = min(nimg - img, (x0 + TW - 1) / Wp + 1);
    } else {
        const int tiles_w = (W + TW - 1) / TW;
        const int cb = tile % tiles_w;
        const int t2 = tile / tiles_w;
        rb = t2 % tiles_h;
        img = t2 / tiles_h;
        x0 = cb * TW;
    }
    const int y0 = rb * TH;
    const int n0 = blockIdx.y * BN;
    const float* __restrict__ A = X + (rv.poff[g] + (int64_t)img * H * W) * cin;
    const int K = 9 * cin;

    constexpr int AQ = RG_BK / 4;
    constexpr int AROWS = 256 / AQ;
    constexpr int AV = RG_BM / AROWS;
    const int ar = tid / AQ, akq = tid % AQ;
    int aoff[AV];
    unsigned amask[AV];
#pragma unroll
    for (int j = 0; j < AV; j++) {
        const int m = ar + AROWS * j;
        const int py = y0 + m / TW;
        int px = x0 + m % TW, ir = 0;
        if (FLAT) {
#pragma unroll
            for (int q = 0; q < 3; q++) { const bool nx = px >= Wp; px -= nx ? Wp : 0; ir += nx; }
        }
        unsigned mk = 0;
        if (px < W && ir < span) {
#pragma unroll
            for (int t9 = 0; t9 < 9; t9++) {
                const int iy = py + t9 / 3 - 1, ix = px + t9 % 3 - 1;
                if ((unsigned)iy < (unsigned)H && (unsigned)ix < (unsigned)W) mk |= 1u << t9;
            }
        }
        amask[j] = mk;
        aoff[j] = ((min(ir, span - 1) * H + py) * W + min(px, W - 1)) * cin + akq * 4;
    }
    constexpr int BV = RG_BK * BN / 4 / 256;
    f32x4 pa0[AV], pa1[AV];
    const uint64_t a_addr = reinterpret_cast<uint64_t>(A);
    const float* a_uniform = reinterpret_cast<const float*>(((uint64_t)(uint32_t)__builtin_amdgcn_readfirstlane((int)(a_addr >> 32)) << 32) |
                                                            (uint32_t)__builtin_amdgcn_readfirstlane((int)a_addr));
    const __amdgpu_buffer_rsrc_t a_rsrc = __builtin_amdgcn_make_buffer_rsrc(
        const_cast<float*>(a_uniform),  0,
        __builtin_amdgcn_readfirstlane((int)((int64_t)span * H * W * cin * sizeof(float))), 0x00020000);
    constexpr int OOB = 0x40000000;
    auto load_a_into = [&](int k0, f32x4 (&d0)[AV], f32x4 (&d1)[AV]) {
        const int tap = k0 / cin;
        const int ci0 = k0 - tap * cin;
        const int ky = tap / 3, kx = tap - ky * 3;
        const int delta = ((ky - 1) * W + (kx - 1)) * cin + ci0;
#pragma unroll
        for (int j = 0; j < AV; j++) {
            const int voff = ((amask[j] >> tap) & 1u) ? (aoff[j] + delta) * 4 : OOB;
            const u32x4 v0 = __builtin_amdgcn_raw_buffer_load_b128(a_rsrc, voff, 0, 0);
            const u32x4 v1 = __builtin_amdgcn_raw_buffer_load_b128(a_rsrc, voff + RG_BK * 4, 0, 0);
            d0[j] = __builtin_bit_cast(f32x4, v0);
            d1[j] = __builtin_bit_cast(f32x4, v1);
        }
    };
    auto load_a_pair = [&](int k0) { load_a_into(k0, pa0, pa1); };
    int boff[BV];
#pragma unroll
    for (int j = 0; j < BV; j++) {
        const int idx = tid + 256 * j;
        const int kk = idx / (BN / 4), nn = (idx % (BN / 4)) * 4;
        boff[j] = kk * cout + min(n0 + nn, cout - 4);
    }
    auto load_b = [&](int k0, int buf) {
        if constexpr (SPLIT != 0) {
            split::load_weights<NP>(Bw + ((int64_t)blockIdx.y * (K / RG_BK) + k0 / RG_BK) * split::image_floats,
                                    Bs + buf * NP * SP_PLANE, wave, lane);
            return;
        }
        const float* __restrict__ bk = Bw + (int64_t)k0 * cout;
        float* bdst = Bs + buf * RG_BK * BN + wave * 256;
#pragma unroll
        for (int j = 0; j < BV; j++)
            __builtin_amdgcn_global_load_lds((const __attribute__((address_space(1))) void*)(bk + boff[j]),
                                             (__attribute__((address_space(3))) void*)(bdst + 1024 * j), 16, 0, 0);
    };
    auto commit = [&](int buf, const f32x4 (&pa)[AV]) {
        if constexpr (SPLIT != 0) {
            char* base = reinterpret_cast<char*>(As + buf * NP * SP_PLANE);
#pragma unroll
            for (int j = 0; j < AV; j++) split::commit4<NP>(base, ar + AROWS * j, akq, pa[j][0], pa[j][1], pa[j][2], pa[j][3]);
            return;
        }
        float* a = As + buf * RG_BK * RG_LDA;
#pragma unroll
        for (int j = 0; j < AV; j++) {
            const int r = ar + AROWS * j;
            a[(akq * 4 + 0) * RG_LDA + r] = pa[j].x;
            a[(akq * 4 + 1) * RG_LDA + r] = pa[j].y;
            a[(akq * 4 + 2) * RG_LDA + r] = pa[j].z;
            a[(akq * 4 + 3) * RG_LDA + r] = pa[j].w;
        }
    };

    f32x16 acc[2][NTW];
#pragma unroll
    for (int t = 0; t < NTW; t++) {
        const int col = n0 + wn * (BN / 2) + t * 32 + l31;
        const float bv = col < cout ? bias[col] : 0.0f;
#pragma unroll
        for (int r = 0; r < 16; r++) { acc[0][t][r] = bv; acc[1][t][r] = bv; }
    }
    auto compute = [&](int buf, int bbuf = -1) {
        if constexpr (SPLIT != 0) {
            split::mma_chunk<NP>(reinterpret_cast<const char*>(As + buf * NP * SP_PLANE),
                                 reinterpret_cast<const char*>(Bs + (bbuf < 0 ? buf : bbuf) * NP * SP_PLANE), wm, wn, l31, half, acc);
            return;
        }
        const float* a = As + buf * RG_BK * RG_LDA + wm * 64 + l31;
        const float* b = Bs + buf * RG_BK * BN + wn * (BN / 2) + l31;
#pragma unroll
        for (int kp = 0; kp < RG_BK / 2; kp++) {
            const int kr = 2 * kp + half;
            const float a0 = a[kr * RG_LDA], a1 = a[kr * RG_LDA + 32];
#pragma unroll
            for (int t = 0; t < NTW; t++) {
                const float bt = b[kr * BN + t * 32];
                acc[0][t] = __builtin_amdgcn_mfma_f32_32x32x2f32(a0, bt, acc[0][t], 0, 0, 0);
                acc[1][t] = __builtin_amdgcn_mfma_f32_32x32x2f32(a1, bt, acc[1][t], 0, 0, 0);
            }
        }
    };
    const int nchunks = K / RG_BK;
    if constexpr (SPLIT != 0) {
        static_assert(AV == 2, "split::pipeline counts four activation loads per chunk pair");
        split::pipeline<NP>(nchunks,
                            [&](int k0, f32x4 (&d0)[AV], f32x4 (&d1)[AV]) { load_a_into(k0, d0, d1); },
                            [&](int k0, int ring) { load_b(k0, ring); },
                            [&](int abuf, const f32x4 (&d)[AV]) { commit(abuf, d); },
                            [&](int abuf, int ring) { compute(abuf, ring); });
    } else {
    load_a_pair(0);
    load_b(0, 0);
    commit(0, pa0);
    __syncthreads();
    for (int c = 0; c < nchunks; c += 2) {
        load_b((c + 1) * RG_BK, 1);
        compute(0);
        commit(1, pa1);
        __syncthreads();
        const bool more = c + 2 < nchunks;
        if (more) {
            load_a_pair((c + 2) * RG_BK);
            load_b((c + 2) * RG_BK, 0);
        }
        compute(1);
        if (more) commit(0, pa0);
        __syncthreads();
    }
    }

    const int Ho = H / PH, Wo = W / PW;
    float* __restrict__ C = Y + (out_poff[g] + (int64_t)img * Ho * Wo) * cout;
    auto act = [&](float v) { return relu ? (v > 0.0f ? v : 0.0f) : v; };
    if (PH == 1 && PW == 1 && n0 + BN <= cout && (cout & 3) == 0 && (((uintptr_t)Y) & 15) == 0) {
        constexpr int WN = BN / 2, LPR = WN / 4, RPI = 64 / LPR, NIT = 32 / RPI;
        static_assert(SPLIT != 0 || 4 * 32 * WN <= 2 * RG_BK * RG_LDA + 2 * RG_BK * BN, "staging must fit the operand tiles");
        float* stage = lds + wave * (32 * WN);
        const int srow = lane / LPR, sc4 = (lane % LPR) * 4;
        int soff[NIT];
#pragma unroll
        for (int it = 0; it < NIT; it++) {
            const int q = it * RPI + srow;
            int x = x0 + (TW == 32 ? q : (q & 15)), ir = 0;
            if (FLAT) {
#pragma unroll
                for (int k = 0; k < 3; k++) { const bool nx = x >= Wp; x -= nx ? Wp : 0; ir += nx; }
            }
            soff[it] = (x < W && (!FLAT || ir < span)) ? ((FLAT ? ir * Ho * Wo : 0) + x) * cout + n0 + wn * WN + sc4 : -1;
        }
#pragma unroll
        for (int i = 0; i < 2; i++) {
#pragma unroll
            for (int t = 0; t < NTW; t++)
#pragma unroll
                for (int r = 0; r < 16; r++)
                    stage[((r & 3) + 8 * (r >> 2) + 4 * half) * WN + t * 32 + l31] = act(acc[i][t][r]);
            asm volatile("s_waitcnt lgkmcnt(0)" ::: "memory");
#pragma unroll
            for (int it = 0; it < NIT; it++) {
                const int q = it * RPI + srow;
                if (soff[it] < 0) continue;
                const int ty = TW == 32 ? 2 * wm + i : 4 * wm + 2 * i + (q >> 4);
                *reinterpret_cast<f32x4*>(&C[soff[it] + (y0 + ty) * Wo * cout]) = *reinterpret_cast<const f32x4*>(&stage[q * WN + sc4]);
            }
            asm volatile("s_waitcnt lgkmcnt(0)" ::: "memory");
        }
        return;
    }
    constexpr int NX = TW == 16 ? 8 : 16;
    int xo_off[FLAT ? NX : 1];
    if (FLAT) {
#pragma unroll
        for (int jx = 0; jx < NX; jx++) {
            if (PW == 2 && (jx & 1)) { xo_off[jx] = -1; continue; }
            const int q = (jx & 3) + 8 * (jx >> 2) + 4 * half;
            int x = x0 + (TW == 32 ? q : (q & 15)), ir = 0;
#pragma unroll
            for (int k = 0; k < 3; k++) { const bool nx = x >= Wp; x -= nx ? Wp : 0; ir += nx; }
            xo_off[jx] = (x + (PW - 1) < W && ir < span) ? (ir * Ho * Wo + x / PW) * cout : -1;
        }
    }
#pragma unroll
    for (int t = 0; t < NTW; t++) {
        const int col = n0 + wn * (BN / 2) + t * 32 + l31;
        if (col >= cout) continue;
#pragma unroll
        for (int i = 0; i < 2; i++) {
            if (PH == 2 && TW == 32 && i == 1) continue;
#pragma unroll
            for (int r = 0; r < 16; r++) {
                if (PH == 2 && TW == 16 && (r & 8)) continue;
                if (PW == 2 && (r & 1)) continue;
                const int q = (r & 3) + 8 * (r >> 2) + 4 * half;
                const int ty = TW == 32 ? 2 * wm + i : 4 * wm + 2 * i + (r >> 3);
                const int tx = TW == 32 ? q : (q & 15);
                const int x = x0 + tx;
                if (FLAT ? xo_off[TW == 16 ? (r & 7) : r] < 0 : x + (PW - 1) >= W) continue;
                constexpr int VI = (PH == 2 && TW == 32) ? 1 : 0;
                constexpr int VR = (PH == 2 && TW == 16) ? 8 : 0;
                float m = act(acc[i][t][r]);
                if (PW == 2) { const float v = act(acc[i][t][(r + 1) & 15]); m = v > m ? v : m; }
                if (PH == 2) {
                    { const float v = act(acc[(i + VI) & 1][t][(r + VR) & 15]); m = v > m ? v : m; }
                    if (PW == 2) { const float v = act(acc[(i + VI) & 1][t][(r + VR + 1) & 15]); m = v > m ? v : m; }
                }
                const int yo = (y0 + ty) / PH;
                if (FLAT) C[xo_off[TW == 16 ? (r & 7) : r] + yo * Wo * cout + col] = m;
                else C[((int64_t)yo * Wo + x / PW) * cout + col] = m;
            }
        }
    }
}

constexpr int F12_MID = 32, F12_COUT = 64, F12_TW = 16, F12_TH = 8, F12_HW = F12_TW + 2, F12_HH = F12_TH + 2;
constexpr int F12_NPOS = F12_HH * F12_HW;
constexpr int F12_LD = F12_MID + 1;
constexpr int F12_BK = 16;
constexpr size_t F12_LDS = (size_t)(F12_NPOS * F12_LD + 2 * F12_BK * F12_COUT) * sizeof(float);

__global__ void __launch_bounds__(256, CONV_WAVES)
conv12_fused_kernel(const float* __restrict__ X0, RaggedView in0, RaggedView mid, const float* __restrict__ w1,
                    const float* __restrict__ b1, const float* __restrict__ Bw, const float* __restrict__ bias,
                    float* __restrict__ Y, const int64_t* __restrict__ out_poff) {
    extern __shared__ __attribute__((aligned(16))) float lds[];
    constexpr int BN = F12_COUT, TW = F12_TW, TH = F12_TH, LD = F12_LD;
    float* T = lds;
    float* Bs = lds + F12_NPOS * LD;
    const int tid = threadIdx.x, lane = tid & 63, wave = tid >> 6;
    const int half = lane >> 5, l31 = lane & 31;
    const int wm = wave >> 1, wn = wave & 1;
    const int gtile = xcd_remap(blockIdx.x, gridDim.x);
    const int g = find_group(mid.toff2d_gap, mid.G, gtile);
    const int tile = gtile - mid.toff2d_gap[g];
    const int H = mid.H, W = mid.W[g];
    const int H0 = in0.H, W0 = in0.W[g];
    const int tiles_h = H / TH;
    const int Wg = (W + 2) & ~1;
    const int nimg = mid.n[g];
    const int rb = tile % tiles_h;
    const int c0 = (tile / tiles_h) * TW;
    const int img = c0 / Wg;
    const int x0 = c0 - img * Wg;
    const int span = min(nimg - img, (x0 + TW - 1) / Wg + 1);
    const int y0 = rb * TH;

    constexpr int BV = F12_BK * BN / 4 / 256;
    const int boff = (tid / (BN / 4)) * BN + (tid % (BN / 4)) * 4;
    auto load_b = [&](int k0, int buf) {
#pragma unroll
        for (int j = 0; j < BV; j++)
            __builtin_amdgcn_global_load_lds((const __attribute__((address_space(1))) void*)(Bw + (int64_t)(k0 + 16 * j) * BN + boff),
                                             (__attribute__((address_space(3))) void*)(Bs + buf * F12_BK * BN + wave * 256 + 1024 * j), 16, 0, 0);
    };
    load_b(0, 0);

    {
        const int q = tid & 7;
        f32x2 wq[9][2], bq[2];
#pragma unroll
        for (int t = 0; t < 9; t++)
#pragma unroll
            for (int c = 0; c < 2; c++) wq[t][c] = f32x2{w1[t * F12_MID + 4 * q + 2 * c], w1[t * F12_MID + 4 * q + 2 * c + 1]};
#pragma unroll
        for (int c = 0; c < 2; c++) bq[c] = f32x2{b1[4 * q + 2 * c], b1[4 * q + 2 * c + 1]};
        const float* __restrict__ xg = X0 + in0.poff[g];
        for (int p = tid >> 3; p < F12_NPOS; p += 32) {
            const int hy = p / F12_HW, hx = p - hy * F12_HW;
            const int y = y0 - 1 + hy;
            int x = x0 - 1 + hx, ir = 0;
#pragma unroll
            for (int k = 0; k < 3; k++) { const bool nx = x >= Wg; x -= nx ? Wg : 0; ir += nx; }
            f32x2 m[2] = {f32x2{0.0f, 0.0f}, f32x2{0.0f, 0.0f}};
            if ((unsigned)y < (unsigned)H && x >= 0 && x < W && ir < span) {
                const float* xi = xg + (int64_t)(img + ir) * H0 * W0;
                float pt[4][4];
                const int iy0 = 2 * y - 1, ix0 = 2 * x - 1;
                if (iy0 >= 0 && iy0 + 3 < H0 && ix0 >= 0 && ix0 + 3 < W0) {
                    const float* pp = xi + (int64_t)iy0 * W0 + ix0;
#pragma unroll
                    for (int a = 0; a < 4; a++)
#pragma unroll
                        for (int b = 0; b < 4; b++) pt[a][b] = pp[a * W0 + b];
                } else {
#pragma unroll
                    for (int a = 0; a < 4; a++)
#pragma unroll
                        for (int b = 0; b < 4; b++) {
                            const int iy = iy0 + a, ix = ix0 + b;
                            pt[a][b] = ((unsigned)iy < (unsigned)H0 && (unsigned)ix < (unsigned)W0) ? xi[(int64_t)iy * W0 + ix] : 0.0f;
                        }
                }
#pragma unroll
                for (int py = 0; py < 2; py++)
#pragma unroll
                    for (int px = 0; px < 2; px++) {
                        f32x2 acc[2] = {bq[0], bq[1]};
#pragma unroll
                        for (int ky = 0; ky < 3; ky++)
#pragma unroll
                            for (int kx = 0; kx < 3; kx++) {
                                const float xs = pt[py + ky][px + kx];
                                const f32x2 xv = f32x2{xs, xs};
#pragma unroll
                                for (int c = 0; c < 2; c++) acc[c] = __builtin_elementwise_fma(xv, wq[ky * 3 + kx][c], acc[c]);
                            }
#pragma unroll
                        for (int c = 0; c < 2; c++) m[c] = (py == 0 && px == 0) ? acc[c] : __builtin_elementwise_max(acc[c], m[c]);
                    }
#pragma unroll
                for (int c = 0; c < 2; c++) {
                    m[c].x = m[c].x > 0.0f ? m[c].x : 0.0f;
                    m[c].y = m[c].y > 0.0f ? m[c].y : 0.0f;
                }
            }
            float* t = T + p * LD + 4 * q;
            t[0] = m[0].x; t[1] = m[0].y; t[2] = m[1].x; t[3] = m[1].y;
        }
    }

    f32x16 acc[2];
    {
        const int col = wn * 32 + l31;
        const float bv = bias[col];
#pragma unroll
        for (int r = 0; r < 16; r++) { acc[0][r] = bv; acc[1][r] = bv; }
    }
    int abase[2];
#pragma unroll
    for (int i = 0; i < 2; i++) {
        const int m = wm * 64 + i * 32 + l31;
        abase[i] = ((m / TW) * F12_HW + (m % TW)) * LD + half;
    }
    __syncthreads();
// ... 151 lines not shown
            *reinterpret_cast<u32x2*>(T + off) = ph;
            *reinterpret_cast<u32x2*>(T + F12S_TILE + off) = pm;
            if (NP == 3) {
                u32x2 pl = {cut(r0 - lo_f(pm[0]), r1 - hi_f(pm[0])), cut(r2 - lo_f(pm[1]), r3 - hi_f(pm[1]))};
                *reinterpret_cast<u32x2*>(T + 2 * F12S_TILE + off) = pl;
            }
        }
    }

    f32x16 acc[2];
    {
        const float bv = bias[wn * 32 + l31];
#pragma unroll
        for (int r = 0; r < 16; r++) { acc[0][r] = bv; acc[1][r] = bv; }
    }
    const int mx = l31 & 15;
    int pos0[2];
#pragma unroll
    for (int i = 0; i < 2; i++) {
        const int m = wm * 64 + i * 32 + l31;
        pos0[i] = (m / TW) * F12S_RS + mx;
    }
    const int nb = wn * 32 + l31;
    const int boff = nb * 64, bsw = (nb >> 2) & 3;
    asm volatile("" ::: "memory");
    __builtin_amdgcn_s_waitcnt(0x0070);
    __builtin_amdgcn_s_barrier();
    asm volatile("" ::: "memory");
#pragma unroll
    for (int tap = 0; tap < 9; tap++) {
        if (tap + 2 < 9) load_b(tap + 2);
        const int ky = tap / 3, kx = tap % 3;
        const int asw = ((mx + kx) >> 2) & 3;
        const char* bb = Bs + (tap % 3) * NP * F12S_BTAP + boff;
#pragma unroll
        for (int s2 = 0; s2 < 2; s2++) {
            const int qa = (((2 * s2 + half) ^ asw) & 3) << 4, qb = (((2 * s2 + half) ^ bsw) & 3) << 4;
            bf16x8 af[2][3], bfr[3];
#pragma unroll
            for (int i = 0; i < 2; i++)
#pragma unroll
                for (int p = 0; p < NP; p++) af[i][p] = *reinterpret_cast<const bf16x8*>(T + p * F12S_TILE + (pos0[i] + ky * F12S_RS + kx) * 64 + qa);
#pragma unroll
            for (int p = 0; p < NP; p++) bfr[p] = *reinterpret_cast<const bf16x8*>(bb + p * F12S_BTAP + qb);
#define OCRS_TERM12(PA, PB)                                                                                   \
            OCRS_SPLIT_MMA(af[0][PA], bfr[PB], acc[0]);                                                       \
            OCRS_SPLIT_MMA(af[1][PA], bfr[PB], acc[1]);
            if (NP == 3) { OCRS_TERM12(NP - 1, 0) OCRS_TERM12(0, NP - 1) OCRS_TERM12(1, 1) }
            OCRS_TERM12(1, 0) OCRS_TERM12(0, 1) OCRS_TERM12(0, 0)
#undef OCRS_TERM12
        }
        asm volatile("" ::: "memory");
        if (tap + 2 < 9) __builtin_amdgcn_s_waitcnt(0x0070 | NP);
        else __builtin_amdgcn_s_waitcnt(0x0070);
        __builtin_amdgcn_s_barrier();
        asm volatile("" ::: "memory");
    }

    const int Ho = H / 2, Wo = W / 2;
    float* __restrict__ C = Y + (out_poff[g] + (int64_t)img * Ho * Wo) * BN;
    auto act = [&](float v) { return v > 0.0f ? v : 0.0f; };
    const int col = wn * 32 + l31;
    int xo_off[8];
#pragma unroll
    for (int jx = 0; jx < 8; jx++) {
        if (jx & 1) { xo_off[jx] = -1; continue; }
        int x = x0 + (jx & 3) + 8 * (jx >> 2) + 4 * half, ir = 0;
#pragma unroll
        for (int k = 0; k < 3; k++) { const bool nx = x >= Wg; x -= nx ? Wg : 0; ir += nx; }
        xo_off[jx] = (x + 1 < W && ir < span) ? (ir * Ho * Wo + x / 2) * BN : -1;
    }
#pragma unroll
    for (int i = 0; i < 2; i++)
#pragma unroll
        for (int r = 0; r < 8; r += 2) {
            if (xo_off[r & 7] < 0) continue;
            const float m = act(__builtin_fmaxf(__builtin_fmaxf(acc[i][r], acc[i][r + 1]), __builtin_fmaxf(acc[i][r + 8], acc[i][r + 9])));
            const int yo = (y0 + 4 * wm + 2 * i) / 2;
            C[xo_off[r & 7] + yo * Wo * BN + col] = m;
        }
}

void conv12_split_weights(const float* w, std::vector<uint16_t>* out) {
    out->assign((size_t)9 * 3 * F12_COUT * 32, 0);
    auto bits = [](float f) { uint32_t u; memcpy(&u, &f, 4); return u; };
    auto from = [](uint32_t u) { float f; memcpy(&f, &u, 4); return f; };
    auto rne = [&](float f) { const uint32_t u = bits(f); return (u + 0x7FFFu + ((u >> 16) & 1u)) >> 16; };
    for (int tap = 0; tap < 9; tap++)
        for (int n = 0; n < F12_COUT; n++)
            for (int k = 0; k < 32; k++) {
                const float x = w[(size_t)(tap * 32 + k) * F12_COUT + n];
                const uint32_t hb = rne(x);
                const float r1 = x - from(hb << 16);
                const uint32_t mb = rne(r1);
                const uint32_t lb = rne(r1 - from(mb << 16));
                const size_t e = (size_t)n * 32 + (size_t)((((k >> 3) ^ (n >> 2)) & 3) * 8) + (k & 7);
                uint16_t* img = out->data() + (size_t)tap * 3 * F12_COUT * 32;
                img[e] = (uint16_t)hb;
                img[F12_COUT * 32 + e] = (uint16_t)mb;
                img[2 * F12_COUT * 32 + e] = (uint16_t)lb;
            }
}

bool conv12_fused_ragged(const float* x, const RaggedView& in0, const RaggedView& mid, const float* w1, const float* b1,
                         int c1, const float* w2, const float* b2, int c2, float* y, const RaggedView& out, hipStream_t s,
                         const uint16_t* w2split) {
    if (option(OPT_CONV12_FUSE) == 0) return false;
    if (c1 != F12_MID || c2 != F12_COUT || mid.H % F12_TH != 0 || in0.H != 2 * mid.H || out.H * 2 != mid.H) return false;
    if (mid.min_w < 11 || mid.ntiles2d_gap <= 0) return false;
    if (mid.max_tile_px_ * 4 * (int64_t)sizeof(float) >= (int64_t)1 << 30 ||
        mid.max_tile_px_ * F12_COUT * (int64_t)sizeof(float) >= (int64_t)1 << 30) return false;
    if (!x) return true;
    const int numerics = option(OPT_NUMERICS);
    if (numerics != 0 && w2split) {
        static std::atomic<uint64_t> ok3{0}, ok2{0};
        if (numerics == 2) {
            allow_dynamic_lds(reinterpret_cast<const void*>(&conv12_fused_split_kernel<2>), ok2);
            hipLaunchKernelGGL((conv12_fused_split_kernel<2>), dim3(mid.ntiles2d_gap), dim3(256), f12s_lds(2), s, x, in0, mid, w1, b1, w2split, b2, y, out.poff);
        } else {
            allow_dynamic_lds(reinterpret_cast<const void*>(&conv12_fused_split_kernel<3>), ok3);
            hipLaunchKernelGGL((conv12_fused_split_kernel<3>), dim3(mid.ntiles2d_gap), dim3(256), f12s_lds(3), s, x, in0, mid, w1, b1, w2split, b2, y, out.poff);
        }
        return true;
    }
    hipLaunchKernelGGL(conv12_fused_kernel, dim3(mid.ntiles2d_gap), dim3(256), F12_LDS, s, x, in0, mid, w1, b1, w2, b2, y, out.poff);
    return true;
}

void split_weights(const float* w, int K, int N, int ldw, std::vector<uint16_t>* out) {
    const int nblk = N / 128, nch = K / 16;
    out->assign((size_t)nblk * nch * 3 * 128 * 16, 0);
    auto bits = [](float f) { uint32_t u; memcpy(&u, &f, 4); return u; };
    auto from = [](uint32_t u) { float f; memcpy(&f, &u, 4); return f; };
    auto rne = [&](float f) { const uint32_t u = bits(f); return (u + 0x7FFFu + ((u >> 16) & 1u)) >> 16; };
    for (int nb = 0; nb < nblk; nb++)
        for (int c = 0; c < nch; c++) {
            uint16_t* img = out->data() + ((size_t)nb * nch + c) * 3 * 128 * 16;
            for (int n = 0; n < 128; n++)
                for (int kl = 0; kl < 16; kl++) {
                    const float x = w[(size_t)(c * 16 + kl) * ldw + nb * 128 + n];
                    const uint32_t hb = rne(x);
                    const float r1 = x - from(hb << 16);
                    const uint32_t mb = rne(r1);
                    const uint32_t lb = rne(r1 - from(mb << 16));
                    const int half = kl >> 3, j = kl & 7;
                    const size_t e = (size_t)n * 16 + (size_t)(((half ^ (n >> 3)) & 1) * 8) + j;
                    img[e] = (uint16_t)hb;
                    img[128 * 16 + e] = (uint16_t)mb;
                    img[2 * 128 * 16 + e] = (uint16_t)lb;
                }
        }
}

bool conv3x3_ragged(const float* x, const RaggedView& rv, int cin, const float* wt, const float* bias, int cout, int relu,
                    int ph, int pw, float* y, const RaggedView& out, hipStream_t s, const uint16_t* wsplit) {
    if ((cin % (2 * RG_BK)) != 0 || (cout % 4) != 0 || cout < 64) return false;
    if (!((ph == 1 && pw == 1) || (ph == 2 && (pw == 1 || pw == 2)))) return false;
    if ((ph == 2 || pw == 2) && !relu) return false;
    if (rv.tw != 32 && rv.tw != 16) return false;
    if (rv.H % (RG_BM / rv.tw) != 0) return false;
    const bool flat = option(OPT_CONV_FLAT) != 0 && rv.min_w >= 11 &&
                      rv.max_tile_px_ * std::max(cin, cout) * (int64_t)sizeof(float) < (int64_t)1 << 30;
    if (!flat && (int64_t)rv.H * rv.max_w * cin * (int64_t)sizeof(float) >= (int64_t)1 << 30) return false;
    const int ntiles = flat ? (pw == 2 ? rv.ntiles2d_flat2 : rv.ntiles2d_flat) : rv.ntiles2d;
    if (ntiles <= 0) return true;
    const bool n64 = cout <= 64;
    const int numerics = option(OPT_NUMERICS);
    const bool split = wsplit && !n64 && (cout % 128) == 0 && (cin % 64) == 0 && numerics != 0;
    const size_t lds = split ? split::lds_bytes(numerics == 2 ? 2 : 3)
                             : (size_t)(2 * RG_BK * RG_LDA + 2 * RG_BK * (n64 ? 64 : 128)) * sizeof(float);
    const dim3 grid(ntiles, (cout + (n64 ? 63 : 127)) / (n64 ? 64 : 128));
#define OCRS_LAUNCH_SPLIT(TW_, PH_, PW_, FLAT_, NP_, SLOT_)                                                              \
    if (flat == FLAT_ && (numerics == 2 ? 2 : 3) == NP_) {                                                              \
        allow_dynamic_lds(reinterpret_cast<const void*>(&conv3x3_ragged_kernel<128, TW_, PH_, PW_, FLAT_, NP_>), ok_[SLOT_]);   \
        hipLaunchKernelGGL((conv3x3_ragged_kernel<128, TW_, PH_, PW_, FLAT_, NP_>), grid, dim3(256), lds, s, x, rv, cin, ws_, bias, \
                           cout, relu, y, out.poff);                                                                    \
    }
#define OCRS_LAUNCH_CONV(BN_, TW_, PH_, PW_)                                                                            \
    do {                                                                                                                \
        if (split && BN_ == 128) {                                                                                      \
            const float* ws_ = reinterpret_cast<const float*>(wsplit);                                                  \
            static std::atomic<uint64_t> ok_[4] = {};                                                                    \
            OCRS_LAUNCH_SPLIT(TW_, PH_, PW_, true, 3, 0) OCRS_LAUNCH_SPLIT(TW_, PH_, PW_, false, 3, 1)                     \
            OCRS_LAUNCH_SPLIT(TW_, PH_, PW_, true, 2, 2) OCRS_LAUNCH_SPLIT(TW_, PH_, PW_, false, 2, 3)                     \
        } else if (flat) hipLaunchKernelGGL((conv3x3_ragged_kernel<BN_, TW_, PH_, PW_, true>), grid, dim3(256), lds, s, x, rv, \
                                     cin, wt, bias, cout, relu, y, out.poff);                                           \
        else hipLaunchKernelGGL((conv3x3_ragged_kernel<BN_, TW_, PH_, PW_, false>), grid, dim3(256), lds, s, x, rv,     \
                                cin, wt, bias, cout, relu, y, out.poff);                                                \
    } while (0)
#define OCRS_DISPATCH_POOL(BN_, TW_)                              \
    do {                                                          \
        if (ph == 1) OCRS_LAUNCH_CONV(BN_, TW_, 1, 1);            \
        else if (pw == 1) OCRS_LAUNCH_CONV(BN_, TW_, 2, 1);       \
        else OCRS_LAUNCH_CONV(BN_, TW_, 2, 2);                    \
    } while (0)
    if (n64) {
        if (rv.tw == 32) OCRS_DISPATCH_POOL(64, 32); else OCRS_DISPATCH_POOL(64, 16);
    } else {
        if (rv.tw == 32) OCRS_DISPATCH_POOL(128, 32); else OCRS_DISPATCH_POOL(128, 16);
    }
#undef OCRS_DISPATCH_POOL
#undef OCRS_LAUNCH_CONV
#undef OCRS_LAUNCH_SPLIT
    return true;
}

}
}
```

ocrs_amd/csrc/model.hpp:

```cpp
#pragma once
#include <functional>
#include <memory>
#include <string>
#include <vector>

#include "common.hpp"

namespace ocrs {

enum OpType : uint32_t {
    OP_CONV = 0, OP_DWCONV3, OP_MAXPOOL, OP_AVGPOOL, OP_CONVT2, OP_PADCAT, OP_SIGMOID, OP_TOSEQ, OP_GRU, OP_LINEAR,
    OP_LOGSOFTMAX, OP_COUNT
};

struct GraphOp {
    uint32_t type;
    int32_t in0, in1, out;
    int32_t relu, kh, kw, cin, cout, hidden;
    const float* w[8] = {nullptr};
    size_t wcount[8] = {0};
    const float* aux0 = nullptr;
    const float* aux1 = nullptr;
    const float* aux2 = nullptr;
    const float* aux3 = nullptr;
    const uint16_t* wsplit = nullptr;
    bool fused_into_prev = false;
    bool fuse_next_pw = false;
    bool done_by_prev = false;
    bool cat_into_next = false;
    bool reads_cat = false;
    int dc_block = -1;
};

struct DcBlock {
    int first = -1, last = -1;
    int convt = -1, cat = -1, dw1 = -1, pw1 = -1, dw2 = -1, pw2 = -1, pool = -1, fin = -1, sig = -1;
    int cs = 0, cx = 0, cmid = 0, cout = 0;
    const float* tape = nullptr;
    int tape_len = 0;
    const float* rtape = nullptr;
    int rtape_len = 0;
};

struct TensorShape {
    int n = 0, h = 0, w = 0, c = 0;
    bool seq = false;
    int64_t count() const { return (int64_t)n * h * w * c; }
};

struct ModelBase {
    virtual ~ModelBase() = default;
    int device = -1;
    int64_t input_shape[4] = {-1, -1, -1, -1};
    virtual bool is_callback() const = 0;
};

struct CallbackModel : ModelBase {
    ocrs_model_run_fn fn = nullptr;
    void* user = nullptr;
    bool is_callback() const override { return true; }
    void run(const float* input, const int64_t in_shape[4], std::vector<float>& out, int64_t out_shape[4],
             int* out_ndim) const;
};

struct HipModel : ModelBase {
    uint32_t kind = 0;
    std::vector<GraphOp> ops;
    std::vector<DcBlock> dc_blocks;
    uint32_t n_slots = 0, out_slot = 0;
    DevBuf weights;
    std::vector<DevBuf> tapes;
    bool is_callback() const override { return false; }

    static std::unique_ptr<HipModel> load(const void* data, size_t len, int device = -1);

    TensorShape infer(int n, int h, int w, std::vector<TensorShape>* slots = nullptr) const;
    double flops(int n, int h, int w) const;

    float* run_device(Workspace& ws, const float* d_in, int n, int h, int w, TensorShape* out_shape,
                      StageTimers* timers, const uint8_t* d_excluded = nullptr, int32_t* d_labels = nullptr,
                      bool want_logp = true, bool print_timing = false, int stop_before = -1,
                      hipStream_t exec = nullptr ) const;

    int packed_split() const;
    struct PackedGroup {
        const float* d_batch;
        int n, w;
        const int32_t* d_pos;
    };
    struct PackedPlan {
        int M = 0, Tmax = 0;
        int64_t R = 0;
        const int32_t* d_Tm = nullptr;
        const int32_t* d_off = nullptr;
        std::vector<int> active;
        std::vector<int32_t> h_Tm;
        std::vector<int32_t> h_off;
        uint32_t* h_status = nullptr;
    };
    struct OpRange {
        int first = 0, last = 0;
        bool gx_only = false;
        const float* seq_in = nullptr;
        int in_c = 0;
        const float* out = nullptr;
        int out_c = 0;
    };
    static const int32_t* make_packed_plan(Workspace& ws, const std::vector<int32_t>& T, PackedPlan* plan, std::vector<size_t>* order);
    int run_recognition_packed(Workspace& ws, const std::vector<PackedGroup>& groups, const PackedPlan& plan, int h,
                               StageTimers* timers, const uint8_t* d_excluded, int32_t* d_labels,
                               float** d_logp = nullptr, float* d_maxlp = nullptr, OpRange* range = nullptr) const;
    float* run_prefix_ragged(Workspace& ws, hipStream_t exec, const std::vector<PackedGroup>& groups,
                             const PackedPlan& plan, int h, int ts, StageTimers* timers, int* feat_c,
                             const std::function<void()>& before_launch = nullptr, const OpRange* range = nullptr,
                             hipEvent_t* stack_done = nullptr) const;
};

}

struct ocrs_model {
    std::unique_ptr<ocrs::ModelBase> impl;
};
```

ocrs_amd/csrc/model_load.cpp:

```cpp
#include "model_exec.hpp"

namespace ocrs {

namespace {
#pragma pack(push, 1)
struct FileHeader {
    char magic[8];
    uint32_t version, kind;
    int64_t input_shape[4];
    uint32_t n_ops, n_slots, out_slot, reserved;
    uint64_t blob_floats;
};
struct FileOp {
    uint32_t type;
    int32_t in0, in1, out, relu, kh, kw, cin, cout, hidden;
    uint32_t n_w, reserved;
    struct { uint64_t off, cnt; } w[8];
};
#pragma pack(pop)
static_assert(sizeof(FileHeader) == 72, "header layout");
static_assert(sizeof(FileOp) == 176, "op layout");

struct ParsedFile {
    FileHeader hd;
    std::vector<FileOp> fops;
    const float* blob = nullptr;
    std::vector<float> slab;
};
struct Fix { size_t op; int which; size_t off; };

void pad16(std::vector<float>& slab) { while (slab.size() % 4) slab.push_back(0.f); }

void check_op_record(const FileHeader& hd, const FileOp& f, uint32_t i) {
    if (f.type >= OP_COUNT || f.n_w > 8) fail(OCRS_ERR_IO, "bad op record %u", i);
    for (uint32_t j = 0; j < f.n_w; j++)
        if (f.w[j].off > hd.blob_floats || f.w[j].cnt > hd.blob_floats - f.w[j].off)
            fail(OCRS_ERR_IO, "weight reference out of range in op %u", i);
    const int64_t ns = hd.n_slots;
    const bool two_in = f.type == OP_PADCAT;
    if (f.in0 < 0 || f.in0 >= ns || f.out <= 0 || f.out >= ns || (two_in ? (f.in1 < 0 || f.in1 >= ns) : false) ||
        (!two_in && f.in1 >= ns))
        fail(OCRS_ERR_IO, "slot index out of range in op %u", i);
    auto want = [&](uint32_t j, int64_t cnt) {
        if (j >= f.n_w || cnt < 0 || (int64_t)f.w[j].cnt != cnt)
            fail(OCRS_ERR_IO, "op %u (%s): weight tensor %u has %llu floats, the op's shape needs %lld", i,
                 kOpNames[f.type], j, j < f.n_w ? (unsigned long long)f.w[j].cnt : 0ull, (long long)cnt);
    };
    auto pos = [&](int64_t v, const char* what) {
        if (v <= 0 || v > (1 << 20)) fail(OCRS_ERR_IO, "op %u (%s): bad %s %lld", i, kOpNames[f.type], what, (long long)v);
    };
    switch (f.type) {
        case OP_CONV: pos(f.kh, "kh"); pos(f.kw, "kw"); pos(f.cin, "cin"); pos(f.cout, "cout");
            want(0, (int64_t)f.kh * f.kw * f.cin * f.cout); want(1, f.cout); break;
        case OP_DWCONV3: pos(f.cin, "channels"); want(0, 9LL * f.cin); want(1, f.cin); break;
        case OP_MAXPOOL: case OP_AVGPOOL: pos(f.kh, "kh"); pos(f.kw, "kw"); break;
        case OP_CONVT2: pos(f.cin, "cin"); pos(f.cout, "cout"); want(0, 4LL * f.cin * f.cout); want(1, f.cout); break;
        case OP_GRU: pos(f.cin, "input size"); pos(f.hidden, "hidden size");
            if (f.n_w != 8) fail(OCRS_ERR_IO, "GRU op %u needs 8 weight tensors", i);
            for (uint32_t d = 0; d < 2; d++) {
                want(4 * d + 0, 3LL * f.cin * f.hidden); want(4 * d + 1, 3LL * f.hidden);
                want(4 * d + 2, 3LL * f.hidden * f.hidden); want(4 * d + 3, 3LL * f.hidden);
            }
            break;
        case OP_LINEAR: pos(f.cin, "cin"); pos(f.cout, "cout"); want(0, (int64_t)f.cin * f.cout); want(1, f.cout); break;
        default: break;
    }
}

void check_channels(const FileHeader& hd, const std::vector<FileOp>& fops) {
    std::vector<int64_t> chans(hd.n_slots, -1);
    chans[0] = 1;
    for (uint32_t i = 0; i < hd.n_ops; i++) {
        const FileOp& f = fops[i];
        auto in = [&](int32_t sl) {
            if (chans[sl] < 0)
                fail(OCRS_ERR_IO, "op %u (%s): input slot %d is not written by an earlier op", i, kOpNames[f.type], sl);
            return chans[sl];
        };
        const int64_t c0 = in(f.in0);
        auto need = [&](int64_t want, const char* what) {
            if (c0 != want)
                fail(OCRS_ERR_IO, "op %u (%s): %s is %lld but input slot %d carries %lld channels", i, kOpNames[f.type], what,
                     (long long)want, f.in0, (long long)c0);
        };
        int64_t co = c0;
        switch (f.type) {
            case OP_CONV: case OP_CONVT2: case OP_LINEAR: need(f.cin, "cin"); co = f.cout; break;
            case OP_DWCONV3: need(f.cin, "channels"); break;
            case OP_GRU: need(f.cin, "input size"); co = 2LL * f.hidden; break;
            case OP_PADCAT: co = c0 + in(f.in1); break;
            default: break;
        }
        if (co > (1 << 24)) fail(OCRS_ERR_IO, "op %u (%s): %lld output channels", i, kOpNames[f.type], (long long)co);
        chans[f.out] = co;
    }
    if (chans[hd.out_slot] < 0) fail(OCRS_ERR_IO, "the output slot %u is not written by any op", hd.out_slot);
}

ParsedFile parse_and_validate(const void* data, size_t len) {
    ParsedFile pf;
    FileHeader& hd = pf.hd;
    if (len < sizeof(FileHeader)) fail(OCRS_ERR_IO, "model file too short");
    memcpy(&hd, data, sizeof hd);
    if (memcmp(hd.magic, "OCRSMDL1", 8) != 0 || hd.version != 1) fail(OCRS_ERR_IO, "not an OCRSMDL1 model file");
    if (hd.n_ops > (1u << 20) || hd.n_slots == 0 || hd.n_slots > (1u << 20) || hd.out_slot >= hd.n_slots)
        fail(OCRS_ERR_IO, "model file header out of range (%u ops, %u slots, output slot %u)", hd.n_ops, hd.n_slots, hd.out_slot);
    const size_t table = sizeof(FileHeader) + (size_t)hd.n_ops * sizeof(FileOp);
    if (len < table || hd.blob_floats > (len - table) / sizeof(float)) fail(OCRS_ERR_IO, "model file truncated");
    pf.blob = reinterpret_cast<const float*>(static_cast<const char*>(data) + table);
    pf.fops.resize(hd.n_ops);
    for (uint32_t i = 0; i < hd.n_ops; i++) {
        memcpy(&pf.fops[i], static_cast<const char*>(data) + sizeof(FileHeader) + (size_t)i * sizeof(FileOp), sizeof(FileOp));
        check_op_record(hd, pf.fops[i], i);
    }
    check_channels(hd, pf.fops);
    pf.slab.assign(pf.blob, pf.blob + hd.blob_floats);
    pad16(pf.slab);
    return pf;
}

GraphOp graph_op(const FileOp& f) {
    GraphOp op{};
    op.type = f.type; op.in0 = f.in0; op.in1 = f.in1; op.out = f.out;
    op.relu = f.relu; op.kh = f.kh; op.kw = f.kw; op.cin = f.cin; op.cout = f.cout; op.hidden = f.hidden;
    for (uint32_t j = 0; j < f.n_w; j++) op.wcount[j] = f.w[j].cnt;
    return op;
}

std::vector<Fix> append_derived(ParsedFile& pf) {
    std::vector<Fix> fixes;
    std::vector<float>& slab = pf.slab;
    for (size_t i = 0; i < pf.fops.size(); i++) {
        const FileOp& f = pf.fops[i];
        if (f.type == OP_CONVT2) {
            const float* w = pf.blob + f.w[0].off;
            const float* b = pf.blob + f.w[1].off;
            fixes.push_back({i, 0, slab.size()});
            for (int ci = 0; ci < f.cin; ci++)
                for (int q = 0; q < 4; q++)
                    for (int co = 0; co < f.cout; co++) slab.push_back(w[((size_t)q * f.cin + ci) * f.cout + co]);
            pad16(slab);
            fixes.push_back({i, 1, slab.size()});
            for (int q = 0; q < 4; q++)
                for (int co = 0; co < f.cout; co++) slab.push_back(b[co]);
            pad16(slab);
        } else if (f.type == OP_GRU) {
            for (int part = 0; part < 4; part++) {
                fixes.push_back({i, part, slab.size()});
                for (int d = 0; d < 2; d++) {
                    const float* src = pf.blob + f.w[4 * d + part].off;
                    slab.insert(slab.end(), src, src + f.w[4 * d + part].cnt);
                }
                pad16(slab);
            }
        }
    }
    return fixes;
}

template <class T>
const T* upload_tape(HipModel& m, const std::vector<T>& host) {
    m.tapes.emplace_back(host.size() * sizeof(T));
    OCRS_HIP(hipMemcpy(m.tapes.back().p, host.data(), host.size() * sizeof(T), hipMemcpyHostToDevice));
    return m.tapes.back().as<T>();
}

void upload_slab(HipModel& m, const ParsedFile& pf, const std::vector<Fix>& fixes) {
    m.weights = DevBuf(pf.slab.size() * sizeof(float));
    OCRS_HIP(hipMemcpy(m.weights.p, pf.slab.data(), pf.slab.size() * sizeof(float), hipMemcpyHostToDevice));
    const float* base = m.weights.as<float>();
    for (size_t i = 0; i < m.ops.size(); i++)
        for (uint32_t j = 0; j < pf.fops[i].n_w; j++) m.ops[i].w[j] = base + pf.fops[i].w[j].off;
    for (const Fix& fx : fixes) {
        GraphOp& op = m.ops[fx.op];
        const float** aux[4] = {&op.aux0, &op.aux1, &op.aux2, &op.aux3};
        *aux[fx.which] = base + fx.off;
    }
}

void upload_split_images(HipModel& m, const ParsedFile& pf, const std::vector<Fix>& fixes) {
    const float* slab = pf.slab.data();
    for (size_t i = 0; i < m.ops.size(); i++) {
        GraphOp& op = m.ops[i];
        if (m.kind != 1 || op.type != OP_CONV || op.kh != 3 || op.kw != 3) continue;
        std::vector<uint16_t> img;
        if ((op.cin % 32) == 0 && (op.cout % 128) == 0)
            k::split_weights(slab + pf.fops[i].w[0].off, 9 * op.cin, op.cout, op.cout, &img);
        else if (op.cin == 32 && op.cout == 64)
            k::conv12_split_weights(slab + pf.fops[i].w[0].off, &img);
        else
            continue;
        op.wsplit = upload_tape(m, img);
    }
    for (const Fix& fx : fixes) {
        GraphOp& op = m.ops[fx.op];
        if (fx.which != 0 || op.type != OP_GRU || (op.cin % 64) != 0 || ((3 * op.hidden) % 128) != 0) continue;
        std::vector<uint16_t> both;
        for (int dir = 0; dir < 2; dir++) {
            std::vector<uint16_t> img;
            k::split_weights(slab + fx.off + (size_t)dir * op.cin * 3 * op.hidden, op.cin, 3 * op.hidden, 3 * op.hidden, &img);
            both.insert(both.end(), img.begin(), img.end());
        }
        op.wsplit = upload_tape(m, both);
    }
}

void mark_fusions(HipModel& m) {
    std::vector<GraphOp>& ops = m.ops;
    auto only_reader_is_next = [&](size_t i) {
        const int slot = ops[i].out;
        if ((uint32_t)slot == m.out_slot) return false;
        for (size_t j = i + 2; j < ops.size(); j++)
            if (ops[j].in0 == slot || ops[j].in1 == slot) return false;
        return true;
    };
    for (size_t i = 0; i + 1 < ops.size(); i++) {
        GraphOp& a = ops[i];
        GraphOp& b = ops[i + 1];
        if (b.in0 != a.out) continue;
        const bool pw11 = b.type == OP_CONV && b.kh == 1 && b.kw == 1;
        if (a.type == OP_CONV && a.cout == 1 && a.kh == 1 && a.kw == 1 && b.type == OP_SIGMOID && only_reader_is_next(i))
            b.fused_into_prev = true;
        if (a.type == OP_DWCONV3 && pw11 && b.cin == a.cin && k::dwpw_fused_supported(a.cin, b.cout) && only_reader_is_next(i)) {
            a.fuse_next_pw = true; b.done_by_prev = true;
        }
        if (a.type == OP_PADCAT && b.type == OP_DWCONV3 && only_reader_is_next(i)) {
            a.cat_into_next = true; b.reads_cat = true;
        }
    }
}

void upload_block_tapes(HipModel& m, const ParsedFile& pf, DcBlock& b) {
    auto host = [&](int op, int j) -> const float* { return op >= 0 ? pf.slab.data() + pf.fops[op].w[j].off : nullptr; };
    k::StreamWeights hw{host(b.convt, 0), host(b.convt, 1), host(b.dw1, 0), host(b.dw1, 1), host(b.pw1, 0), host(b.pw1, 1),
                        host(b.dw2, 0), host(b.dw2, 1), host(b.pw2, 0), host(b.pw2, 1), host(b.fin, 0), host(b.fin, 1)};
    k::DoubleConvArgs none{};
    std::vector<float> tape;
    int tape_len = 0;
    if (k::double_conv_stream(none, b.cs, b.cx, b.cmid, b.cout, b.pool >= 0, b.fin >= 0, false, nullptr, &hw, &tape, &tape_len)) {
        b.tape = upload_tape(m, tape);
        b.tape_len = tape_len;
    }
    if (k::double_conv_rows(none, b.cs, b.cx, b.cmid, b.cout, b.pool >= 0, b.fin >= 0, false, nullptr, &hw, &tape, &tape_len)) {
        b.rtape = upload_tape(m, tape);
        b.rtape_len = tape_len;
    }
}

void find_double_conv_blocks(HipModel& m, const ParsedFile& pf) {
    auto& ops = m.ops;
    const int n = (int)ops.size();
    auto uses = [&](int slot) {
        int u = 0;
        for (const GraphOp& o : ops) u += (o.in0 == slot) + (o.in1 == slot);
        return u + ((uint32_t)slot == m.out_slot ? 1 : 0);
    };
    auto pw11 = [](const GraphOp& o) { return o.type == OP_CONV && o.kh == 1 && o.kw == 1; };
    for (int i = 0; i + 3 < n; i++) {
        DcBlock b;
        int j = i;
        if (ops[j].type == OP_CONVT2 && j + 1 < n && ops[j + 1].type == OP_PADCAT && ops[j + 1].in1 == ops[j].out &&
            uses(ops[j].out) == 1 && uses(ops[j + 1].out) == 1) {
            b.convt = j; b.cat = j + 1;
            j += 2;
        }
        if (j + 3 >= n) continue;
        const GraphOp &d1 = ops[j], &p1 = ops[j + 1], &d2 = ops[j + 2], &p2 = ops[j + 3];
        if (d1.type != OP_DWCONV3 || !pw11(p1) || d2.type != OP_DWCONV3 || !pw11(p2)) continue;
        if (b.cat >= 0 && d1.in0 != ops[b.cat].out) continue;
        if (p1.in0 != d1.out || d2.in0 != p1.out || p2.in0 != d2.out) continue;
        if (uses(d1.out) != 1 || uses(p1.out) != 1 || uses(d2.out) != 1) continue;
        if (p1.cin != d1.cin || d2.cin != p1.cout || p2.cin != d2.cin) continue;
        b.dw1 = j; b.pw1 = j + 1; b.dw2 = j + 2; b.pw2 = j + 3;
        b.first = i; b.last = j + 3;
        b.cmid = p1.cout; b.cout = p2.cout;
        if (b.convt >= 0) {
            b.cx = ops[b.convt].cin;
            b.cs = d1.cin - ops[b.convt].cout;
            if (b.cs != ops[b.convt].cout) continue;
        } else {
            b.cs = d1.cin;
        }
        const int k = j + 4;
        if (k < n && ops[k].type == OP_MAXPOOL && ops[k].kh == 2 && ops[k].kw == 2 && ops[k].in0 == p2.out && b.convt < 0) {
            b.pool = k; b.last = k;
        } else if (k < n && pw11(ops[k]) && ops[k].cout == 1 && !ops[k].relu && ops[k].in0 == p2.out && uses(p2.out) == 1 && b.convt >= 0) {
            b.fin = k; b.last = k;
            if (k + 1 < n && ops[k + 1].type == OP_SIGMOID && ops[k + 1].fused_into_prev) { b.sig = k + 1; b.last = k + 1; }
            else if (uses(ops[k].out) == 0) continue;
        }
        k::DoubleConvArgs none{};
        if (!k::double_conv_fused(none, b.cs, b.cx, b.cmid, b.cout, b.pool >= 0, b.fin >= 0, false, nullptr)) continue;
        upload_block_tapes(m, pf, b);
        ops[i].dc_block = (int)m.dc_blocks.size();
        m.dc_blocks.push_back(b);
        i = b.last;
    }
}
}

void CallbackModel::run(const float* input, const int64_t in_shape[4], std::vector<float>& out,
                        int64_t out_shape[4], int* out_ndim) const {
    float* o = nullptr;
    int64_t os[4] = {0, 0, 0, 0};
    int nd = 0;
    int rc = fn(user, input, in_shape, &o, os, &nd);
    if (rc != 0 || !o || nd < 1 || nd > 4) {
        if (o) free(o);
        fail(OCRS_ERR_RUN_FAILED, "model run failed: callback returned %d", rc);
    }
    int64_t cnt = 1;
    for (int i = 0; i < nd; i++) cnt *= os[i];
    out.assign(o, o + cnt);
    free(o);
    for (int i = 0; i < 4; i++) out_shape[i] = i < nd ? os[i] : 1;
    *out_ndim = nd;
}

std::unique_ptr<HipModel> HipModel::load(const void* data, size_t len, int device) {
    ParsedFile pf = parse_and_validate(data, len);
    const std::vector<Fix> fixes = append_derived(pf);
    auto m = std::make_unique<HipModel>();
    m->kind = pf.hd.kind;
    for (int i = 0; i < 4; i++) m->input_shape[i] = pf.hd.input_shape[i];
    m->n_slots = pf.hd.n_slots;
    m->out_slot = pf.hd.out_slot;
    for (const FileOp& f : pf.fops) m->ops.push_back(graph_op(f));
    DeviceScope bind(device);
    m->device = ctx().device;
    upload_slab(*m, pf, fixes);
    upload_split_images(*m, pf, fixes);
    mark_fusions(*m);
    find_double_conv_blocks(*m, pf);
    return m;
}

TensorShape HipModel::infer(int n, int h, int w, std::vector<TensorShape>* slots_out) const {
    std::vector<TensorShape> s(n_slots);
    s[0] = TensorShape{n, h, w, 1, false};
    for (const GraphOp& op : ops) {
        const TensorShape a = s[op.in0];
        TensorShape o = a;
        switch (op.type) {
            case OP_CONV: o.c = op.cout; break;
            case OP_MAXPOOL:
            case OP_AVGPOOL: o.h = a.h / op.kh; o.w = a.w / op.kw; break;
            case OP_CONVT2: o.h = 2 * a.h; o.w = 2 * a.w; o.c = op.cout; break;
            case OP_PADCAT: o.c = a.c + s[op.in1].c; break;
            case OP_DWCONV3: case OP_SIGMOID: case OP_LOGSOFTMAX: break;
            case OP_TOSEQ: o = TensorShape{a.w, a.n, 1, a.c, true}; break;
            case OP_GRU: o.c = 2 * op.hidden; break;
            case OP_LINEAR: o.c = op.cout; break;
            default: fail(OCRS_ERR_IO, "bad op type %u", op.type);
        }
        s[op.out] = o;
    }
    TensorShape out = s[out_slot];
    if (slots_out) *slots_out = std::move(s);
    return out;
}

double HipModel::flops(int n, int h, int w) const {
    std::vector<TensorShape> s;
    infer(n, h, w, &s);
    double total = 0;
    for (const GraphOp& op : ops) {
        const TensorShape a = s[op.in0];
        const double px = (double)a.n * a.h * a.w;
        switch (op.type) {
            case OP_CONV: total += 2.0 * px * op.cout * op.cin * op.kh * op.kw; break;
            case OP_DWCONV3: total += 2.0 * px * a.c * 9; break;
            case OP_CONVT2: total += 2.0 * px * op.cin * op.cout * 4; break;
            case OP_GRU: total += 2.0 * 2.0 * px * 3 * op.hidden * (op.cin + op.hidden); break;
            case OP_LINEAR: total += 2.0 * px * op.cin * op.cout; break;
            default: break;
        }
    }
    return total;
}

}
```

ocrs_amd/csrc/model_packed.cpp:

```cpp
#include <functional>
#include <mutex>

#include "model_exec.hpp"
#include "ragged_plan.hpp"

namespace ocrs {

namespace {
bool ragged_stack_supported(const std::vector<GraphOp>& ops, int ts, int h) {
    for (int i = 0; i < ts; i++) {
        const GraphOp& op = ops[i];
        if (op.in0 != (i == 0 ? 0 : ops[i - 1].out)) return false;
        if (op.type == OP_CONV) {
            if (op.kh != 3 || op.kw != 3 || !op.relu) return false;
            if (op.cin == 1) {
                if (i + 1 >= ts || ops[i + 1].type != OP_MAXPOOL || ops[i + 1].kh != 2 || ops[i + 1].kw != 2) return false;
                if (op.cout > 64 || op.cout < 4 || (op.cout & (op.cout - 1)) != 0) return false;
            } else if ((op.cin % 32) != 0 || op.cout < 64 || (op.cout % 4) != 0) {
                return false;
            }
        } else if (op.type != OP_MAXPOOL && op.type != OP_AVGPOOL) {
            return false;
        }
    }
    for (int i = 0; i < ts; i++) {
        if (ops[i].type == OP_CONV && ops[i].cin != 1 && (h % 4) != 0) return false;
        if (ops[i].type == OP_MAXPOOL || ops[i].type == OP_AVGPOOL) h /= ops[i].kh;
    }
    return true;
}

struct StackBuffers {
    Workspace& ws;
    const bool shared_arena;
    std::vector<std::pair<float*, size_t>> spare;
    std::vector<char> arena_taken;
    float* held = nullptr;
    size_t held_bytes = 0;

    float* get(size_t floats) {
        const size_t bytes = floats * sizeof(float);
        for (size_t i = 0; i < spare.size(); i++)
            if (spare[i].second >= bytes) { float* p = spare[i].first; spare.erase(spare.begin() + i); return p; }
        if (!shared_arena) return static_cast<float*>(ws.alloc(bytes));
        auto& arena = ctx().heavy_arena;
        arena_taken.resize(arena.size(), 0);
        size_t best = arena.size();
        for (size_t i = 0; i < arena.size(); i++)
            if (!arena_taken[i] && arena[i].bytes >= bytes && (best == arena.size() || arena[i].bytes < arena[best].bytes)) best = i;
        if (best == arena.size()) {
            arena.emplace_back(bytes + bytes / 8);
            arena_taken.push_back(0);
        }
        arena_taken[best] = 1;
        return arena[best].as<float>();
    }
    void rotate(float* y, size_t floats) {
        if (held) spare.emplace_back(held, held_bytes);
        held = y; held_bytes = floats * sizeof(float);
    }
};

struct RaggedStack {
    const HipModel& m;
    const RaggedPlan& geo;
    StageTimers* timers;
    hipStream_t st;
    const int ts, first, last;
    StackBuffers bufs;
    const float* cur;
    int curC = 1;

    template <class Launch>
    void timed(int cls, double flops, double bytes, Launch&& launch) { timed_launch(timers, st, cls, flops, bytes, launch); }
    bool launches(int i, int j) const {
        if (i < first && j >= first)
            fail(OCRS_ERR_INVALID_ARGUMENT, "op range: op %d lies inside the fused launch of ops %d..%d (a range starts at %d)", first, i, j, i);
        if (i <= last && j > last)
            fail(OCRS_ERR_INVALID_ARGUMENT, "op range: op %d lies inside the fused launch of ops %d..%d (a range ends at %d)", last, i, j, j);
        return i >= first;
    }
    float* output(const k::RaggedView& vout, int c) { return bufs.get((size_t)vout.pixels * c); }
    void produced(float* y, const k::RaggedView& vout, int c) {
        bufs.rotate(y, (size_t)vout.pixels * c);
        cur = y;
    }

    int step(int i) {
        const auto& ops = m.ops;
        const GraphOp& op = ops[i];
        const k::RaggedView vin = geo.view(i);
        if (op.type == OP_CONV && op.cin == 1) {
            if (i + 3 < ts && ops[i + 2].type == OP_CONV && ops[i + 2].cin == op.cout && ops[i + 2].relu &&
                ops[i + 3].type == OP_MAXPOOL && ops[i + 3].kh == 2 && ops[i + 3].kw == 2) {
                const GraphOp& op2 = ops[i + 2];
                const k::RaggedView vmid = geo.view(i + 2), vout = geo.view(i + 4);
                if (k::conv12_fused_ragged(nullptr, vin, vmid, nullptr, nullptr, op.cout, nullptr, nullptr, op2.cout, nullptr, vout, st)) {
                    if (launches(i, i + 3)) {
                        float* y = output(vout, op2.cout);
                        timed(KC_GEMM_CONV3X3, 2.0 * vmid.pixels * 9.0 * op2.cin * op2.cout,
                              4.0 * (vin.pixels + vout.pixels * op2.cout) + 4.0 * op2.wcount[0],
                              [&] { k::conv12_fused_ragged(cur, vin, vmid, op.w[0], op.w[1], op.cout, op2.w[0], op2.w[1], op2.cout, y, vout, st, op2.wsplit); });
                        produced(y, vout, op2.cout);
                    }
                    curC = op2.cout;
                    return i + 3;
                }
            }
            const k::RaggedView vout = geo.view(i + 2);
            if (launches(i, i + 1)) {
                float* y = output(vout, op.cout);
                timed(KC_CONV_DIRECT, 2.0 * vin.pixels * 9 * op.cout, 4.0 * vin.pixels + 4.0 * vout.pixels * op.cout,
                      [&] { k::conv1_relu_pool_ragged(cur, vin, op.w[0], op.w[1], op.cout, y, vout, st); });
                produced(y, vout, op.cout);
            }
            curC = op.cout;
            return i + 1;
        }
        if (op.type == OP_CONV) {
            const bool fuse = i + 1 < ts && ops[i + 1].type == OP_MAXPOOL && ops[i + 1].kh == 2 &&
                              (ops[i + 1].kw == 1 || ops[i + 1].kw == 2) && vin.H % 2 == 0;
            const int ph = fuse ? 2 : 1, pw = fuse ? ops[i + 1].kw : 1;
            const k::RaggedView vout = geo.view(fuse ? i + 2 : i + 1);
            if (launches(i, fuse ? i + 1 : i)) {
                float* y = output(vout, op.cout);
                bool ok = false;
                timed(KC_GEMM_CONV3X3, 2.0 * vin.pixels * 9.0 * op.cin * op.cout,
                      4.0 * (vin.pixels * op.cin + vout.pixels * op.cout) + 4.0 * op.wcount[0],
                      [&] { ok = k::conv3x3_ragged(cur, vin, op.cin, op.w[0], op.w[1], op.cout, op.relu, ph, pw, y, vout, st, op.wsplit); });
                if (!ok) fail(OCRS_ERR_RUN_FAILED, "model run failed: ragged conv %d->%d at height %d not supported", op.cin, op.cout, vin.H);
                produced(y, vout, op.cout);
            }
            curC = op.cout;
            return fuse ? i + 1 : i;
        }
        if (op.type == OP_AVGPOOL && i + 1 == ts && op.kw == 1 && op.kh == vin.H && (curC & 3) == 0) {
            launches(i, ts);
            return ts;
        }
        if (launches(i, i)) {
            const k::RaggedView vout = geo.view(i + 1);
            float* y = output(vout, curC);
            timed(KC_POOL, 0, 4.0 * curC * (vin.pixels + vout.pixels),
                  [&] { k::pool_ragged(cur, vin, curC, op.kh, op.kw, op.type == OP_AVGPOOL, y, vout, st); });
            produced(y, vout, curC);
        }
        return i;
    }

    float* finish(int at, Workspace& ws, const HipModel::PackedPlan& plan, const int32_t* d_pos) {
        if (at < ts) {
            float* X = ws.alloc_n<float>(bufs.held_bytes / sizeof(float));
            OCRS_HIP(hipMemcpyAsync(X, bufs.held, bufs.held_bytes, hipMemcpyDeviceToDevice, st));
            return X;
        }
        const auto& ops = m.ops;
        const k::RaggedView vf = geo.view(ts);
        if (vf.H != 1) fail(OCRS_ERR_RUN_FAILED, "model run failed: TOSEQ expects height 1, got %d", vf.H);
        float* X = ws.alloc_n<float>((size_t)plan.R * curC);
        const bool pool_here = ts >= 1 && ops[ts - 1].type == OP_AVGPOOL && ops[ts - 1].kw == 1 && (curC & 3) == 0 &&
                               ops[ts - 1].kh == geo.view(ts - 1).H;
        if (pool_here) {
            const k::RaggedView vp = geo.view(ts - 1);
            timed(KC_POOL, 0, 4.0 * curC * (vp.pixels + vf.pixels),
                  [&] { k::avgpool_to_seq_ragged(cur, vp, vf, curC, d_pos, plan.d_off, X, st); });
        } else {
            launches(ts, ts);
            timed(KC_OTHER, 0, 8.0 * vf.pixels * curC, [&] { k::to_seq_packed_ragged(cur, vf, curC, d_pos, plan.d_off, X, st); });
        }
        return X;
    }
};
}

float* HipModel::run_prefix_ragged(Workspace& ws, hipStream_t exec, const std::vector<PackedGroup>& groups,
                                   const PackedPlan& plan, int h, int ts, StageTimers* timers, int* feat_c,
                                   const std::function<void()>& before_launch, const OpRange* range,
                                   hipEvent_t* stack_done) const {
    const int G = (int)groups.size();
    if (G == 0 || ts <= 0 || !ragged_stack_supported(ops, ts, h)) return nullptr;
    for (int g = 0; g + 1 < G && !(range && range->first > 0); g++)
        if (groups[g].d_batch + (size_t)groups[g].n * h * groups[g].w != groups[g + 1].d_batch) return nullptr;

    RaggedPlan geo(ops, ts, h, groups);
    int64_t* d64 = ws.alloc_n<int64_t>(geo.meta64.size());
    int32_t* d32 = ws.alloc_n<int32_t>(geo.meta32.size());
    ws.upload(d64, geo.meta64.data(), geo.meta64.size() * sizeof(int64_t));
    ws.upload(d32, geo.meta32.data(), geo.meta32.size() * sizeof(int32_t));
    geo.d64 = d64;
    geo.d32 = d32;
    if (before_launch) before_launch();
    if (exec != ws.s()) {
        hipEvent_t ready = ws.make_event();
        OCRS_HIP(hipEventRecord(ready, ws.s()));
        OCRS_HIP(hipStreamWaitEvent(exec, ready, 0));
    }

    int tok = timers ? timers->begin(ST_REC_CONV, exec, 0) : -1;
    const bool shared_arena = exec != ws.s() || (ws.stream.serial() && before_launch);
    RaggedStack stack{*this, geo, timers, exec, ts, range ? range->first : 0, range ? range->last : ts,
                      StackBuffers{ws, shared_arena}, groups[0].d_batch};
    int at = ts;
    for (int i = 0; i < ts; i++) {
        i = stack.step(i);
        if (i >= stack.last) { at = i; break; }
    }
    float* X = stack.finish(at, ws, plan, groups[0].d_pos);
    if (tok >= 0) timers->end(tok, exec);
    if (exec != ws.s()) {
        hipEvent_t done = ws.make_event();
        OCRS_HIP(hipEventRecord(done, exec));
        if (stack_done && !ws.stream.may_park_waits()) *stack_done = done;
        else OCRS_HIP(hipStreamWaitEvent(ws.s(), done, 0));
    }
    *feat_c = stack.curC;
    return X;
}

const int32_t* HipModel::make_packed_plan(Workspace& ws, const std::vector<int32_t>& T, PackedPlan* plan,
                                          std::vector<size_t>* order) {
    order->clear();
    for (size_t i = 0; i < T.size(); i++)
        if (T[i] > 0) order->push_back(i);
    std::stable_sort(order->begin(), order->end(), [&](size_t a, size_t b) { return T[a] > T[b]; });
    const int M = (int)order->size();
    if (M == 0) return nullptr;
    plan->M = M;
    plan->Tmax = T[(*order)[0]];
    plan->active.assign(plan->Tmax, 0);
    std::vector<int32_t> hTm(M), hoff(plan->Tmax + 1, 0), hpos(T.size(), 0);
    for (int m = 0; m < M; m++) {
        hTm[m] = T[(*order)[m]];
        hpos[(*order)[m]] = m;
        for (int t = 0; t < hTm[m]; t++) plan->active[t]++;
    }
    for (int t = 0; t < plan->Tmax; t++) hoff[t + 1] = hoff[t] + plan->active[t];
    plan->R = hoff[plan->Tmax];
    std::vector<int32_t> meta(hTm);
    meta.insert(meta.end(), hoff.begin(), hoff.end());
    meta.insert(meta.end(), hpos.begin(), hpos.end());
    int32_t* d_meta = ws.alloc_n<int32_t>(meta.size());
    ws.upload(d_meta, meta.data(), meta.size() * sizeof(int32_t));
    plan->d_Tm = d_meta;
    plan->d_off = d_meta + M;
    plan->h_Tm = std::move(hTm);
    plan->h_off = std::move(hoff);
    return d_meta + M + plan->Tmax + 1;
}

int HipModel::packed_split() const {
    int ts = -1;
    for (size_t i = 0; i < ops.size(); i++)
        if (ops[i].type == OP_TOSEQ) { ts = (int)i; break; }
    if (ts < 0 || (size_t)ts + 3 > ops.size()) return -1;
    int prev_out = ops[ts].out;
    for (size_t i = ts + 1; i < ops.size(); i++) {
        const GraphOp& op = ops[i];
        const bool last = i + 1 == ops.size(), second_last = i + 2 == ops.size();
        if (op.in0 != prev_out) return -1;
        if (last) { if (op.type != OP_LOGSOFTMAX || (uint32_t)op.out != out_slot) return -1; }
        else if (second_last) { if (op.type != OP_LINEAR) return -1; }
        else if (op.type != OP_GRU) return -1;
        prev_out = op.out;
    }
    for (int i = 0; i < ts; i++)
        if (ops[i].type == OP_GRU || ops[i].type == OP_LINEAR || ops[i].type == OP_LOGSOFTMAX || ops[i].type == OP_TOSEQ)
            return -1;
    return ts;
}

namespace {
struct PackedRun {
    const HipModel& m;
    Workspace& ws;
    const HipModel::PackedPlan& plan;
    StageTimers* timers;
    HipModel::OpRange* range;
    hipStream_t st;
    const float* cur = nullptr;
    int curC = 0;
    int gru_layer = 0;
    float* gx_buf = nullptr; size_t gx_cap = 0;
// ... 213 lines not shown
```

ocrs_amd/csrc/ragged_plan.hpp:

```cpp
#pragma once
#include <algorithm>

#include "kernels.hpp"
#include "model.hpp"

namespace ocrs {

struct RaggedPlan {
    struct Table { size_t off = 0; int32_t total = 0; };
    struct Layer {
        int H = 0;
        std::vector<int32_t> W;
        size_t w = 0, p = 0;
        Table t256;
        Table t32, t16;
        Table f32[2], f16[2];
        Table gap;
        int64_t pixels = 0;
    };
    int G = 0;
    std::vector<int32_t> n;
    std::vector<Layer> layers;
    std::vector<int32_t> meta32;
    std::vector<int64_t> meta64;
    size_t loff_at = 0;
    const int32_t* d32 = nullptr;
    const int64_t* d64 = nullptr;

    RaggedPlan(const std::vector<GraphOp>& ops, int ts, int h, const std::vector<HipModel::PackedGroup>& groups)
        : G((int)groups.size()) {
        Layer in;
        in.H = h;
        for (const HipModel::PackedGroup& g : groups) { n.push_back(g.n); in.W.push_back(g.w); }
        layers.push_back(std::move(in));
        for (int i = 0; i < ts; i++) {
            Layer o = layers.back();
            if (ops[i].type == OP_MAXPOOL || ops[i].type == OP_AVGPOOL) {
                o.H /= ops[i].kh;
                for (auto& w : o.W) w /= ops[i].kw;
            }
            layers.push_back(std::move(o));
        }
        meta32 = n;
        loff_at = prefix([&](int g) { return n[g]; }).off;
        for (Layer& l : layers) tabulate(l);
    }

    k::RaggedView view(size_t li) const {
        const Layer& l = layers[li];
        k::RaggedView v{};
        v.G = G; v.H = l.H;
        v.W = d32 + l.w; v.n = d32; v.poff = d64 + l.p;
        v.toff256 = d32 + l.t256.off; v.loff = d32 + loff_at;
        v.ntiles256 = l.t256.total; v.pixels = l.pixels;
        const bool use16 = l.H % 8 == 0 && (l.H % 4 != 0 || l.t16.total < l.t32.total);
        const Table &t2d = use16 ? l.t16 : l.t32, *flat = use16 ? l.f16 : l.f32;
        v.tw = use16 ? 16 : 32;
        v.toff2d = d32 + t2d.off; v.ntiles2d = t2d.total;
        v.toff2d_flat = d32 + flat[0].off; v.ntiles2d_flat = flat[0].total;
        v.toff2d_flat2 = d32 + flat[1].off; v.ntiles2d_flat2 = flat[1].total;
        v.toff2d_gap = d32 + l.gap.off;
        v.ntiles2d_gap = l.H % 8 == 0 ? l.gap.total : 0;
        v.max_w = 0;
        v.max_tile_px_ = 0;
        v.min_w = INT32_MAX;
        for (int g = 0; g < G; g++) {
            const int64_t w = l.W[g], span = std::min<int64_t>(n[g], (v.tw - 1 + w - 1) / w + 1);
            v.max_tile_px_ = std::max(v.max_tile_px_, span * l.H * w);
            v.min_w = std::min(v.min_w, (int)w);
            v.max_w = std::max(v.max_w, (int)w);
        }
        return v;
    }

private:
    template <class Count>
    Table prefix(Count count) {
        Table t{meta32.size(), 0};
        meta32.push_back(0);
        for (int g = 0; g < G; g++) { t.total += (int32_t)count(g); meta32.push_back(t.total); }
        return t;
    }
    void tabulate(Layer& l) {
        const int H = l.H;
        const std::vector<int32_t>& W = l.W;
        l.w = meta32.size();
        meta32.insert(meta32.end(), W.begin(), W.end());
        l.t256 = prefix([&](int g) { return ((int64_t)n[g] * H * W[g] + 255) / 256; });
        l.t32 = prefix([&](int g) { return n[g] * (H / 4) * ((W[g] + 31) / 32); });
        l.t16 = prefix([&](int g) { return n[g] * (H / 8) * ((W[g] + 15) / 16); });
        l.gap = prefix([&](int g) { return (H / 8) * (((int64_t)n[g] * ((W[g] + 2) & ~1) + 15) / 16); });
        for (int e = 0; e < 2; e++) {
            auto cols = [&, e](int g) { return (int64_t)n[g] * (e ? (W[g] + 1) & ~1 : W[g]); };
            l.f32[e] = prefix([&](int g) { return (H / 4) * ((cols(g) + 31) / 32); });
            l.f16[e] = prefix([&](int g) { return (H / 8) * ((cols(g) + 15) / 16); });
        }
        l.p = meta64.size();
        meta64.push_back(0);
        for (int g = 0; g < G; g++) { l.pixels += (int64_t)n[g] * H * W[g]; meta64.push_back(l.pixels); }
    }
};

}
```

Measured before the change: 277.2.

## Add row-owning wave variant of ragged conv3x3 that skips zero-padding taps

Adds a ROWS template variant of the ragged 3x3 conv kernel in which each wave owns a 32-column slice across all four patch rows. This lets the K loop skip the MFMAs for the top or bottom row when those rows read only zero padding at image edges. The skip is enabled only when the weights are all finite and the result is exact (relu, or no -0 bias), which is checked at model load. It also rotates row-block order by column index and adds a new epilogue, and is on by default (conv_rows=2). The cost is a different wave-to-output mapping with more MFMA issue per wave and new code paths for pooled outputs.

```diff
diff --git a/include/ocrs_amd.h b/include/ocrs_amd.h
--- a/include/ocrs_amd.h
+++ b/include/ocrs_amd.h
@@ -50,6 +50,9 @@
                                              long window_us, int fail_every, uint64_t out[5]);
 
 OCRS_API ocrs_status ocrs_stream_plan_selftest(int budget, const int32_t* ops, size_t n_ops, int32_t* out);
+
+OCRS_API ocrs_status ocrs_conv_rows_selftest(const float* w, size_t n_w, const float* bias, size_t n_bias, int relu, int y0, int h,
+                                             int cin, int32_t out[6]);
 
 OCRS_API ocrs_status ocrs_set_option(const char* name, long value);
 OCRS_API ocrs_status ocrs_option_name(int index, const char** name);
diff --git a/ocrs_amd/_lib.py b/ocrs_amd/_lib.py
--- a/ocrs_amd/_lib.py
+++ b/ocrs_amd/_lib.py
@@ -62,7 +62,7 @@
     "ocrs_get_device", "ocrs_model_load_file_on_device", "ocrs_model_load_bytes_on_device", "ocrs_model_device", "ocrs_engine_device",
     "ocrs_engine_group_new", "ocrs_engine_group_free", "ocrs_engine_group_size", "ocrs_engine_group_member", "ocrs_group_deal",
     "ocrs_group_prepare_input_batch", "ocrs_group_prepare_input_device_batch", "ocrs_group_detect_words_batch",
-    "ocrs_group_recognize_text_batch", "ocrs_group_gather", "ocrs_group_final_gather", "ocrs_group_worker_threads", "ocrs_group_last_gather", "ocrs_device_malloc_on", "ocrs_engine_coalesce_stats", "ocrs_coalescer_selftest", "ocrs_stream_plan_selftest", "ocrs_engine_kernel_mfma_flops", "ocrs_engine_prepare_input_jpeg", "ocrs_jpeg_decode_rgb", "ocrs_jpeg_info", "ocrs_jpeg_coefficients",
+    "ocrs_group_recognize_text_batch", "ocrs_group_gather", "ocrs_group_final_gather", "ocrs_group_worker_threads", "ocrs_group_last_gather", "ocrs_device_malloc_on", "ocrs_engine_coalesce_stats", "ocrs_coalescer_selftest", "ocrs_stream_plan_selftest", "ocrs_conv_rows_selftest", "ocrs_engine_kernel_mfma_flops", "ocrs_engine_prepare_input_jpeg", "ocrs_jpeg_decode_rgb", "ocrs_jpeg_info", "ocrs_jpeg_coefficients",
     "ocrs_group_member_stats", "ocrs_numa_parse_cpulist", "ocrs_numa_bind_selftest", "ocrs_engine_recognize_logits", "ocrs_engine_set_option", "ocrs_engine_get_option", "ocrs_option_name", "ocrs_device_pool_stats", "ocrs_device_pool_configure", "ocrs_device_pool_trim",
     "ocrs_device_set_isolation", "ocrs_device_isolation", "ocrs_group_set_replay", "ocrs_abi_version",
     "ocrs_engine_recognize_text_scored", "ocrs_engine_recognize_text_batch_scored", "ocrs_ctc_beam_search_scored",
diff --git a/ocrs_amd/csrc/abi.cpp b/ocrs_amd/csrc/abi.cpp
--- a/ocrs_amd/csrc/abi.cpp
+++ b/ocrs_amd/csrc/abi.cpp
@@ -5,6 +5,7 @@
 #include <atomic>
 #include "abi_util.hpp"
 #include "coalesce_selftest.hpp"
+#include "conv_rows.hpp"
 #include "engine.hpp"
 #include "host_pool.hpp"
 #include "jpeg.hpp"
@@ -80,6 +81,23 @@
                 case 5: out[i] = plan.light_lanes(); break;
                 default: fail(OCRS_ERR_INVALID_ARGUMENT, "unknown op %d", (int)op);
             }
+        }
+    });
+}
+
+ocrs_status ocrs_conv_rows_selftest(const float* w, size_t n_w, const float* bias, size_t n_bias, int relu, int y0, int h, int cin,
+                                    int32_t out[6]) {
+    return guarded([&] {
+        if (!out || (n_w > 0 && !w) || (n_bias > 0 && !bias) || h < kConvRowsPatchH || h % kConvRowsPatchH != 0 || y0 < 0 || y0 >= h ||
+            y0 % kConvRowsPatchH != 0 || cin < 2 * kConvRowsChunk || cin % (2 * kConvRowsChunk) != 0)
+            fail(OCRS_ERR_INVALID_ARGUMENT, "bad argument");
+        out[0] = conv_rows_skip_exact(w, n_w, bias, n_bias, relu != 0) ? 1 : 0;
+        const RowPhases ph = conv_row_phases(y0, h, cin, out[0] != 0);
+        out[1] = ph.c_top;
+        out[2] = ph.c_bot;
+        for (int phase = 0; phase < 3; phase++) {
+            const int c = 3 * phase * (cin / kConvRowsChunk);
+            out[3 + phase] = c < ph.c_top ? 0 : c >= ph.c_bot ? kConvRowsPatchH - 1 : -1;
         }
     });
 }
diff --git a/ocrs_amd/csrc/common.cpp b/ocrs_amd/csrc/common.cpp
--- a/ocrs_amd/csrc/common.cpp
+++ b/ocrs_amd/csrc/common.cpp
@@ -499,11 +499,13 @@
     return g_opts[o].load(std::memory_order_relaxed);
 }
 int option(Option o) { return (int)option_long(o); }
+int conv_rows_setting() { return t_tuning ? (int)__atomic_load_n(&t_tuning->conv_rows, __ATOMIC_RELAXED) : (int)kConvRowsDefault; }
 
 Tuning default_tuning() {
     std::call_once(g_opts_once, init_options);
     Tuning t;
     for (int i = 0; i < OPT_COUNT; i++) t.v[i] = g_opts[i].load(std::memory_order_relaxed);
+    t.conv_rows = kConvRowsDefault;
     return t;
 }
 
@@ -523,6 +525,11 @@
 }
 
 int set_option(Tuning& t, const char* name, long value) {
+    if (name && strcmp(name, "conv_rows") == 0) {
+        if (value < 0 || value > 2) return 2;
+        __atomic_store_n(&t.conv_rows, value, __ATOMIC_RELAXED);
+        return 0;
+    }
     const int i = find_option(name, OPT_COUNT);
     if (i < 0) return 1;
     if (i == OPT_STREAM_BUDGET) return 4;
@@ -532,6 +539,10 @@
 }
 
 bool get_option(const Tuning& t, const char* name, long* value) {
+    if (name && strcmp(name, "conv_rows") == 0) {
+        *value = __atomic_load_n(&t.conv_rows, __ATOMIC_RELAXED);
+        return true;
+    }
     const int i = name && strcmp(name, "numerics") == 0 ? (int)OPT_NUMERICS : find_option(name, OPT_COUNT);
     if (i < 0) return false;
     *value = __atomic_load_n(&t.v[i], __ATOMIC_RELAXED);
diff --git a/ocrs_amd/csrc/common.hpp b/ocrs_amd/csrc/common.hpp
--- a/ocrs_amd/csrc/common.hpp
+++ b/ocrs_amd/csrc/common.hpp
@@ -153,7 +153,9 @@
               OPT_COALESCE, OPT_COALESCE_PAGES, OPT_COALESCE_WINDOW_US,
               OPT_LAYOUT_THREADS, OPT_REC_MAX_PIXELS,
               OPT_COUNT };
-struct Tuning { long v[OPT_COUNT]; };
+constexpr long kConvRowsDefault = 2;
+struct Tuning { long v[OPT_COUNT]; long conv_rows; };
+int conv_rows_setting();
 Tuning default_tuning();
 int set_option(const char* name, long value);
 int set_option(Tuning& t, const char* name, long value);
diff --git a/ocrs_amd/csrc/conv_rows.hpp b/ocrs_amd/csrc/conv_rows.hpp
--- /dev/null
+++ b/ocrs_amd/csrc/conv_rows.hpp
@@ -0,0 +1,29 @@
+#pragma once
+#include <cmath>
+#include <cstddef>
+#include <cstring>
+
+namespace ocrs {
+
+constexpr int kConvRowsChunk = 16;
+constexpr int kConvRowsPatchH = 4;
+
+inline bool conv_rows_skip_exact(const float* w, size_t n_w, const float* bias, size_t n_bias, bool relu) {
+    for (size_t i = 0; i < n_w; i++)
+        if (!std::isfinite(w[i])) return false;
+    if (relu) return true;
+    for (size_t i = 0; i < n_bias; i++) {
+        unsigned u;
+        memcpy(&u, &bias[i], 4);
+        if (u == 0x80000000u) return false;
+    }
+    return true;
+}
+
+struct RowPhases { int c_top, c_bot; };
+constexpr RowPhases conv_row_phases(int y0, int H, int cin, bool skip) {
+    const int per_tap = cin / kConvRowsChunk;
+    return RowPhases{skip && y0 == 0 ? 3 * per_tap : 0, skip && y0 + kConvRowsPatchH == H ? 6 * per_tap : 9 * per_tap};
+}
+
+}
diff --git a/ocrs_amd/csrc/kernels.hpp b/ocrs_amd/csrc/kernels.hpp
--- a/ocrs_amd/csrc/kernels.hpp
+++ b/ocrs_amd/csrc/kernels.hpp
@@ -170,6 +170,11 @@
     const int32_t* toff2d_flat;
     const int32_t* toff2d_flat2;
     int ntiles2d_flat, ntiles2d_flat2;
+    const int32_t* toff2d_32;
+    const int32_t* toff2d_flat_32;
+    const int32_t* toff2d_flat2_32;
+    int ntiles2d_32, ntiles2d_flat_32, ntiles2d_flat2_32;
+    int64_t max_tile_px32_;
     const int32_t* toff2d_gap;
     int ntiles2d_gap;
     int64_t max_tile_px_;
@@ -190,7 +195,8 @@
                          const uint16_t* w2split = nullptr);
 void conv12_split_weights(const float* w2_host , std::vector<uint16_t>* out);
 bool conv3x3_ragged(const float* x, const RaggedView& rv, int cin, const float* wt, const float* bias, int cout, int relu,
-                    int ph, int pw, float* y, const RaggedView& out, hipStream_t s, const uint16_t* wsplit = nullptr);
+                    int ph, int pw, float* y, const RaggedView& out, hipStream_t s, const uint16_t* wsplit = nullptr,
+                    bool skip_exact = false);
 void split_weights(const float* w_host, int K, int N, int ldw, std::vector<uint16_t>* out);
 
 struct LineDesc {
diff --git a/ocrs_amd/csrc/kernels_rec.hip b/ocrs_amd/csrc/kernels_rec.hip
--- a/ocrs_amd/csrc/kernels_rec.hip
+++ b/ocrs_amd/csrc/kernels_rec.hip
@@ -1,6 +1,8 @@
 #include <algorithm>
+#include <type_traits>
 
 #include "common.hpp"
+#include "conv_rows.hpp"
 #include "kernels.hpp"
 #include "split_mfma.hpp"
 
@@ -219,15 +221,17 @@
 
 constexpr int RG_BM = 128, RG_BK = 16, RG_LDA = RG_BM + 1;
 constexpr int CONV_WAVES = 4;
-template <int BN, int TW, int PH, int PW, bool FLAT, int SPLIT = 0>
+static_assert(RG_BK == kConvRowsChunk && RG_BM / 32 == kConvRowsPatchH, "conv_rows.hpp describes this kernel's K loop");
+template <int BN, int TW, int PH, int PW, int ROWS, bool FLAT, int SPLIT = 0>
 __global__ void __launch_bounds__(256, SPLIT == 3 ? 2 : SPLIT == 2 ? 3 : CONV_WAVES)
 conv3x3_ragged_kernel(const float* __restrict__ X, RaggedView rv, int cin, const float* __restrict__ Bw,
                       const float* __restrict__ bias, int cout, int relu, float* __restrict__ Y,
-                      const int64_t* __restrict__ out_poff) {
+                      const int64_t* __restrict__ out_poff, int skip) {
     extern __shared__ __attribute__((aligned(16))) float lds[];
     constexpr int NTW = BN / 64;
     constexpr int TH = RG_BM / TW;
     static_assert(TW == 32 || TW == 16, "patch width");
+    static_assert(!ROWS || (SPLIT == 0 && BN == 128 && TW == 32), "row-owning waves: exact, 128 columns, 4 x 32 patches");
     static_assert(!SPLIT || (BN == 128 && RG_BK == 16), "split mode: 128-column blocks, 16-deep chunks");
     constexpr int NP = SPLIT ? SPLIT : 1;
     constexpr int SP_PLANE = split::PLANE;
@@ -244,10 +248,11 @@
     const int tiles_h = H / TH;
     const int Wp = FLAT ? (PW == 2 ? (W + 1) & ~1 : W) : W;
     const int nimg = FLAT ? rv.n[g] : 1;
-    int rb, img, x0, span = 1;
+    int rb, img, x0, span = 1, cidx;
     if (FLAT) {
         rb = tile % tiles_h;
-        const int c0 = (tile / tiles_h) * TW;
+        cidx = tile / tiles_h;
+        const int c0 = cidx * TW;
         img = c0 / Wp;
         x0 = c0 - img * Wp;
         span = min(nimg - img, (x0 + TW - 1) / Wp + 1);
@@ -258,6 +263,14 @@
         rb = t2 % tiles_h;
         img = t2 / tiles_h;
         x0 = cb * TW;
+        cidx = cb;
+    }
+    if constexpr (ROWS != 0) {
+        rb = (rb + cidx) % tiles_h;
+        rb = __builtin_amdgcn_readfirstlane(rb);
+        img = __builtin_amdgcn_readfirstlane(img);
+        x0 = __builtin_amdgcn_readfirstlane(x0);
+        span = __builtin_amdgcn_readfirstlane(span);
     }
     const int y0 = rb * TH;
     const int n0 = blockIdx.y * BN;
@@ -355,7 +368,7 @@
     f32x16 acc[2][NTW];
 #pragma unroll
     for (int t = 0; t < NTW; t++) {
-        const int col = n0 + wn * (BN / 2) + t * 32 + l31;
+        const int col = ROWS ? n0 + wave * 32 + l31 : n0 + wn * (BN / 2) + t * 32 + l31;
         const float bv = col < cout ? bias[col] : 0.0f;
 #pragma unroll
         for (int r = 0; r < 16; r++) { acc[0][t][r] = bv; acc[1][t][r] = bv; }
@@ -380,8 +393,49 @@
             }
         }
     };
+    auto compute_rows = [&](int buf, auto without) {
+        constexpr int WO = decltype(without)::value;
+        const float* a = As + buf * RG_BK * RG_LDA + l31;
+        const float* b = Bs + buf * RG_BK * BN + wave * 32 + l31;
+#pragma unroll
+        for (int kp = 0; kp < RG_BK / 2; kp++) {
+            const int kr = 2 * kp + half;
+            const float bt = b[kr * BN];
+#pragma unroll
+            for (int j = 0; j < 4; j++) {
+                if (j == WO) continue;
+                acc[j >> 1][j & 1] = __builtin_amdgcn_mfma_f32_32x32x2f32(a[kr * RG_LDA + 32 * j], bt, acc[j >> 1][j & 1], 0, 0, 0);
+            }
+        }
+    };
     const int nchunks = K / RG_BK;
-    if constexpr (SPLIT != 0) {
+    if constexpr (ROWS != 0) {
+        const RowPhases ph = conv_row_phases(y0, H, cin, skip != 0);
+        const int c_top = __builtin_amdgcn_readfirstlane(ph.c_top), c_bot = __builtin_amdgcn_readfirstlane(ph.c_bot);
+        auto chunk_pairs = [&](int cb, int ce, auto without) {
+            for (int c = cb; c < ce; c += 2) {
+                load_b((c + 1) * RG_BK, 1);
+                compute_rows(0, without);
+                commit(1, pa1);
+                __syncthreads();
+                const bool more = c + 2 < nchunks;
+                if (more) {
+                    load_a_pair((c + 2) * RG_BK);
+                    load_b((c + 2) * RG_BK, 0);
+                }
+                compute_rows(1, without);
+                if (more) commit(0, pa0);
+                __syncthreads();
+            }
+        };
+        load_a_pair(0);
+        load_b(0, 0);
+        commit(0, pa0);
+        __syncthreads();
+        chunk_pairs(0, c_top, std::integral_constant<int, 0>{});
+        chunk_pairs(c_top, c_bot, std::integral_constant<int, -1>{});
+        chunk_pairs(c_bot, nchunks, std::integral_constant<int, 3>{});
+    } else if constexpr (SPLIT != 0) {
         static_assert(AV == 2, "split::pipeline counts four activation loads per chunk pair");
         split::pipeline<NP>(nchunks,
                             [&](int k0, f32x4 (&d0)[AV], f32x4 (&d1)[AV]) { load_a_into(k0, d0, d1); },
@@ -412,7 +466,41 @@
     const int Ho = H / PH, Wo = W / PW;
     float* __restrict__ C = Y + (out_poff[g] + (int64_t)img * Ho * Wo) * cout;
     auto act = [&](float v) { return relu ? (v > 0.0f ? v : 0.0f) : v; };
-    if (PH == 1 && PW == 1 && n0 + BN <= cout && (cout & 3) == 0 && (((uintptr_t)Y) & 15) == 0) {
+    const int wave_e = ROWS ? __builtin_amdgcn_readfirstlane(wave) : wave;
+    const int lane_e = ROWS ? (int)__builtin_amdgcn_mbcnt_hi(~0u, __builtin_amdgcn_mbcnt_lo(~0u, 0u)) : lane;
+    const int half_e = ROWS ? lane_e >> 5 : half, l31_e = ROWS ? lane_e & 31 : l31;
+    if constexpr (ROWS != 0) {
+        if (PH == 1 && PW == 1 && (((uintptr_t)Y) & 15) == 0) {
+            constexpr int WN = 32, LPR = WN / 4, RPI = 64 / LPR, NIT = 32 / RPI;
+            float* stage = lds + wave_e * (32 * WN);
+            const int srow = lane_e / LPR, sc4 = (lane_e % LPR) * 4;
+            int soff[NIT];
+#pragma unroll
+            for (int it = 0; it < NIT; it++) {
+                int x = x0 + it * RPI + srow, ir = 0;
+                if (FLAT) {
+#pragma unroll
+                    for (int k = 0; k < 3; k++) { const bool nx = x >= Wp; x -= nx ? Wp : 0; ir += nx; }
+                }
+                soff[it] = (x < W && (!FLAT || ir < span)) ? ((FLAT ? ir * Ho * Wo : 0) + x) * cout + n0 + wave_e * WN + sc4 : -1;
+            }
+#pragma unroll
+            for (int j = 0; j < 4; j++) {
+#pragma unroll
+                for (int r = 0; r < 16; r++) stage[((r & 3) + 8 * (r >> 2) + 4 * half_e) * WN + l31_e] = act(acc[j >> 1][j & 1][r]);
+                asm volatile("s_waitcnt lgkmcnt(0)" ::: "memory");
+#pragma unroll
+                for (int it = 0; it < NIT; it++) {
+                    if (soff[it] < 0) continue;
+                    *reinterpret_cast<f32x4*>(&C[soff[it] + (y0 + j) * Wo * cout]) =
+                        *reinterpret_cast<const f32x4*>(&stage[(it * RPI + srow) * WN + sc4]);
+                }
+                asm volatile("s_waitcnt lgkmcnt(0)" ::: "memory");
+            }
+            return;
+        }
+    }
+    if (!ROWS && PH == 1 && PW == 1 && n0 + BN <= cout && (cout & 3) == 0 && (((uintptr_t)Y) & 15) == 0) {
         constexpr int WN = BN / 2, LPR = WN / 4, RPI = 64 / LPR, NIT = 32 / RPI;
         static_assert(SPLIT != 0 || 4 * 32 * WN <= 2 * RG_BK * RG_LDA + 2 * RG_BK * BN, "staging must fit the operand tiles");
         float* stage = lds + wave * (32 * WN);
@@ -453,12 +541,37 @@
 #pragma unroll
         for (int jx = 0; jx < NX; jx++) {
             if (PW == 2 && (jx & 1)) { xo_off[jx] = -1; continue; }
-            const int q = (jx & 3) + 8 * (jx >> 2) + 4 * half;
+            const int q = (jx & 3) + 8 * (jx >> 2) + 4 * half_e;
             int x = x0 + (TW == 32 ? q : (q & 15)), ir = 0;
 #pragma unroll
             for (int k = 0; k < 3; k++) { const bool nx = x >= Wp; x -= nx ? Wp : 0; ir += nx; }
             xo_off[jx] = (x + (PW - 1) < W && ir < span) ? (ir * Ho * Wo + x / PW) * cout : -1;
         }
+    }
+    if constexpr (ROWS != 0) {
+        const int col = n0 + wave_e * 32 + l31_e;
+#pragma unroll
+        for (int j = 0; j < 4; j++) {
+            if (PH == 2 && (j & 1)) continue;
+#pragma unroll
+            for (int r = 0; r < 16; r++) {
+                if (PW == 2 && (r & 1)) continue;
+                const int x = x0 + (r & 3) + 8 * (r >> 2) + 4 * half_e;
+                if (FLAT ? xo_off[r] < 0 : x + (PW - 1) >= W) continue;
+                const f32x16& a0 = acc[j >> 1][j & 1];
+                const f32x16& a1 = acc[(j ^ 1) >> 1][(j ^ 1) & 1];
+                float m = act(a0[r]);
+                if (PW == 2) { const float v = act(a0[(r + 1) & 15]); m = v > m ? v : m; }
+                if (PH == 2) {
+                    { const float v = act(a1[r]); m = v > m ? v : m; }
+                    if (PW == 2) { const float v = act(a1[(r + 1) & 15]); m = v > m ? v : m; }
+                }
+                const int yo = (y0 + j) / PH;
+                if (FLAT) C[xo_off[r] + yo * Wo * cout + col] = m;
+                else C[((int64_t)yo * Wo + x / PW) * cout + col] = m;
+            }
+        }
+        return;
     }
 #pragma unroll
     for (int t = 0; t < NTW; t++) {
@@ -916,11 +1029,23 @@
         }
 }
 
-bool conv3x3_ragged(const float* x, const RaggedView& rv, int cin, const float* wt, const float* bias, int cout, int relu,
-                    int ph, int pw, float* y, const RaggedView& out, hipStream_t s, const uint16_t* wsplit) {
+bool conv3x3_ragged(const float* x, const RaggedView& rv_in, int cin, const float* wt, const float* bias, int cout, int relu,
+                    int ph, int pw, float* y, const RaggedView& out, hipStream_t s, const uint16_t* wsplit, bool skip_exact) {
     if ((cin % (2 * RG_BK)) != 0 || (cout % 4) != 0 || cout < 64) return false;
     if (!((ph == 1 && pw == 1) || (ph == 2 && (pw == 1 || pw == 2)))) return false;
     if ((ph == 2 || pw == 2) && !relu) return false;
+    const int rows_opt = conv_rows_setting();
+    const bool exact = !(wsplit && (cin % 64) == 0 && option(OPT_NUMERICS) != 0);
+    const bool rows = rows_opt != 0 && exact && (cout % 128) == 0 && rv_in.H % 4 == 0;
+    const int skip = rows && rows_opt == 2 && skip_exact ? 1 : 0;
+    RaggedView rv = rv_in;
+    if (rows) {
+        rv.tw = 32;
+        rv.toff2d = rv_in.toff2d_32; rv.ntiles2d = rv_in.ntiles2d_32;
+        rv.toff2d_flat = rv_in.toff2d_flat_32; rv.ntiles2d_flat = rv_in.ntiles2d_flat_32;
+        rv.toff2d_flat2 = rv_in.toff2d_flat2_32; rv.ntiles2d_flat2 = rv_in.ntiles2d_flat2_32;
+        rv.max_tile_px_ = rv_in.max_tile_px32_;
+    }
     if (rv.tw != 32 && rv.tw != 16) return false;
     if (rv.H % (RG_BM / rv.tw) != 0) return false;
     const bool flat = option(OPT_CONV_FLAT) != 0 && rv.min_w >= 11 &&
@@ -936,9 +1061,9 @@
     const dim3 grid(ntiles, (cout + (n64 ? 63 : 127)) / (n64 ? 64 : 128));
 #define OCRS_LAUNCH_SPLIT(TW_, PH_, PW_, FLAT_, NP_, SLOT_)                                                              \
     if (flat == FLAT_ && (numerics == 2 ? 2 : 3) == NP_) {                                                              \
-        allow_dynamic_lds(reinterpret_cast<const void*>(&conv3x3_ragged_kernel<128, TW_, PH_, PW_, FLAT_, NP_>), ok_[SLOT_]);   \
-        hipLaunchKernelGGL((conv3x3_ragged_kernel<128, TW_, PH_, PW_, FLAT_, NP_>), grid, dim3(256), lds, s, x, rv, cin, ws_, bias, \
-                           cout, relu, y, out.poff);                                                                    \
+        allow_dynamic_lds(reinterpret_cast<const void*>(&conv3x3_ragged_kernel<128, TW_, PH_, PW_, 0, FLAT_, NP_>), ok_[SLOT_]);   \
+        hipLaunchKernelGGL((conv3x3_ragged_kernel<128, TW_, PH_, PW_, 0, FLAT_, NP_>), grid, dim3(256), lds, s, x, rv, cin, ws_, bias, \
+                           cout, relu, y, out.poff, 0);                                                                 \
     }
 #define OCRS_LAUNCH_CONV(BN_, TW_, PH_, PW_)                                                                            \
     do {                                                                                                                \
@@ -947,10 +1072,17 @@
             static std::atomic<uint64_t> ok_[4] = {};                                                                    \
             OCRS_LAUNCH_SPLIT(TW_, PH_, PW_, true, 3, 0) OCRS_LAUNCH_SPLIT(TW_, PH_, PW_, false, 3, 1)                     \
             OCRS_LAUNCH_SPLIT(TW_, PH_, PW_, true, 2, 2) OCRS_LAUNCH_SPLIT(TW_, PH_, PW_, false, 2, 3)                     \
-        } else if (flat) hipLaunchKernelGGL((conv3x3_ragged_kernel<BN_, TW_, PH_, PW_, true>), grid, dim3(256), lds, s, x, rv, \
-                                     cin, wt, bias, cout, relu, y, out.poff);                                           \
-        else hipLaunchKernelGGL((conv3x3_ragged_kernel<BN_, TW_, PH_, PW_, false>), grid, dim3(256), lds, s, x, rv,     \
-                                cin, wt, bias, cout, relu, y, out.poff);                                                \
+        } else if (flat) hipLaunchKernelGGL((conv3x3_ragged_kernel<BN_, TW_, PH_, PW_, 0, true>), grid, dim3(256), lds, s, x, rv, \
+                                     cin, wt, bias, cout, relu, y, out.poff, 0);                                        \
+        else hipLaunchKernelGGL((conv3x3_ragged_kernel<BN_, TW_, PH_, PW_, 0, false>), grid, dim3(256), lds, s, x, rv,  \
+                                cin, wt, bias, cout, relu, y, out.poff, 0);                                             \
+    } while (0)
+#define OCRS_LAUNCH_ROWS(PH_, PW_)                                                                                      \
+    do {                                                                                                                \
+        if (flat) hipLaunchKernelGGL((conv3x3_ragged_kernel<128, 32, PH_, PW_, 1, true>), grid, dim3(256), lds, s, x, rv, cin, wt, \
+                                     bias, cout, relu, y, out.poff, skip);                                              \
+        else hipLaunchKernelGGL((conv3x3_ragged_kernel<128, 32, PH_, PW_, 1, false>), grid, dim3(256), lds, s, x, rv, cin, wt, \
+                                bias, cout, relu, y, out.poff, skip);                                                   \
     } while (0)
 #define OCRS_DISPATCH_POOL(BN_, TW_)                              \
     do {                                                          \
@@ -958,12 +1090,17 @@
         else if (pw == 1) OCRS_LAUNCH_CONV(BN_, TW_, 2, 1);       \
         else OCRS_LAUNCH_CONV(BN_, TW_, 2, 2);                    \
     } while (0)
-    if (n64) {
+    if (rows) {
+        if (ph == 1) OCRS_LAUNCH_ROWS(1, 1);
+        else if (pw == 1) OCRS_LAUNCH_ROWS(2, 1);
+        else OCRS_LAUNCH_ROWS(2, 2);
+    } else if (n64) {
         if (rv.tw == 32) OCRS_DISPATCH_POOL(64, 32); else OCRS_DISPATCH_POOL(64, 16);
     } else {
         if (rv.tw == 32) OCRS_DISPATCH_POOL(128, 32); else OCRS_DISPATCH_POOL(128, 16);
     }
 #undef OCRS_DISPATCH_POOL
+#undef OCRS_LAUNCH_ROWS
 #undef OCRS_LAUNCH_CONV
 #undef OCRS_LAUNCH_SPLIT
     return true;
diff --git a/ocrs_amd/csrc/model.hpp b/ocrs_amd/csrc/model.hpp
--- a/ocrs_amd/csrc/model.hpp
+++ b/ocrs_amd/csrc/model.hpp
@@ -23,6 +23,7 @@
     const float* aux1 = nullptr;
     const float* aux2 = nullptr;
     const float* aux3 = nullptr;
+    bool skip_exact = false;
     const uint16_t* wsplit = nullptr;
     bool fused_into_prev = false;
     bool fuse_next_pw = false;
diff --git a/ocrs_amd/csrc/model_load.cpp b/ocrs_amd/csrc/model_load.cpp
--- a/ocrs_amd/csrc/model_load.cpp
+++ b/ocrs_amd/csrc/model_load.cpp
@@ -1,3 +1,4 @@
+#include "conv_rows.hpp"
 #include "model_exec.hpp"
 
 namespace ocrs {
@@ -205,6 +206,15 @@
     }
 }
 
+void mark_skip_exact(HipModel& m, const ParsedFile& pf) {
+    for (size_t i = 0; i < m.ops.size(); i++) {
+        GraphOp& op = m.ops[i];
+        if (op.type != OP_CONV || op.kh != 3 || op.kw != 3) continue;
+        const FileOp& f = pf.fops[i];
+        op.skip_exact = conv_rows_skip_exact(pf.blob + f.w[0].off, f.w[0].cnt, pf.blob + f.w[1].off, f.w[1].cnt, op.relu != 0);
+    }
+}
+
 void mark_fusions(HipModel& m) {
     std::vector<GraphOp>& ops = m.ops;
     auto only_reader_is_next = [&](size_t i) {
@@ -330,6 +340,7 @@
     m->device = ctx().device;
     upload_slab(*m, pf, fixes);
     upload_split_images(*m, pf, fixes);
+    mark_skip_exact(*m, pf);
     mark_fusions(*m);
     find_double_conv_blocks(*m, pf);
     return m;
diff --git a/ocrs_amd/csrc/model_packed.cpp b/ocrs_amd/csrc/model_packed.cpp
--- a/ocrs_amd/csrc/model_packed.cpp
+++ b/ocrs_amd/csrc/model_packed.cpp
@@ -127,7 +127,7 @@
                 bool ok = false;
                 timed(KC_GEMM_CONV3X3, 2.0 * vin.pixels * 9.0 * op.cin * op.cout,
                       4.0 * (vin.pixels * op.cin + vout.pixels * op.cout) + 4.0 * op.wcount[0],
-                      [&] { ok = k::conv3x3_ragged(cur, vin, op.cin, op.w[0], op.w[1], op.cout, op.relu, ph, pw, y, vout, st, op.wsplit); });
+                      [&] { ok = k::conv3x3_ragged(cur, vin, op.cin, op.w[0], op.w[1], op.cout, op.relu, ph, pw, y, vout, st, op.wsplit, op.skip_exact); });
                 if (!ok) fail(OCRS_ERR_RUN_FAILED, "model run failed: ragged conv %d->%d at height %d not supported", op.cin, op.cout, vin.H);
                 produced(y, vout, op.cout);
             }
diff --git a/ocrs_amd/csrc/ragged_plan.hpp b/ocrs_amd/csrc/ragged_plan.hpp
--- a/ocrs_amd/csrc/ragged_plan.hpp
+++ b/ocrs_amd/csrc/ragged_plan.hpp
@@ -59,14 +59,20 @@
         v.toff2d = d32 + t2d.off; v.ntiles2d = t2d.total;
         v.toff2d_flat = d32 + flat[0].off; v.ntiles2d_flat = flat[0].total;
         v.toff2d_flat2 = d32 + flat[1].off; v.ntiles2d_flat2 = flat[1].total;
+        const bool has32 = l.H % 4 == 0;
+        v.toff2d_32 = d32 + l.t32.off; v.ntiles2d_32 = has32 ? l.t32.total : 0;
+        v.toff2d_flat_32 = d32 + l.f32[0].off; v.ntiles2d_flat_32 = has32 ? l.f32[0].total : 0;
+        v.toff2d_flat2_32 = d32 + l.f32[1].off; v.ntiles2d_flat2_32 = has32 ? l.f32[1].total : 0;
         v.toff2d_gap = d32 + l.gap.off;
         v.ntiles2d_gap = l.H % 8 == 0 ? l.gap.total : 0;
         v.max_w = 0;
         v.max_tile_px_ = 0;
+        v.max_tile_px32_ = 0;
         v.min_w = INT32_MAX;
         for (int g = 0; g < G; g++) {
             const int64_t w = l.W[g], span = std::min<int64_t>(n[g], (v.tw - 1 + w - 1) / w + 1);
             v.max_tile_px_ = std::max(v.max_tile_px_, span * l.H * w);
+            v.max_tile_px32_ = std::max(v.max_tile_px32_, std::min<int64_t>(n[g], (32 - 1 + w - 1) / w + 1) * l.H * w);
             v.min_w = std::min(v.min_w, (int)w);
             v.max_w = std::max(v.max_w, (int)w);
         }
```

New measurement: 285.0 (median of 6 runs). 1.03x the previous value.
